# chemprop/chemprop

Measured on AMD Instinct MI355X. Metric: million directed-edge-updates/sec (depth=3, hidden=300), higher is better.
Workload: dtype f32 (exact 3-term f16 split of fp32 operands, fp32 accumulate); 1 GPU; qm9-shaped synthetic molecules, 512 mols/GPU/step, BondMessagePassing depth=3 hidden=300, forward (plan K0 + K1..K5); mols_per_gpu=512, directed_edges_per_gpu=9120, parallelism=dp1 (molecule shards, no data-path collective), launch=eager

## Files before the change

### chemprop_amd/_lib.py

```python
from __future__ import annotations

import ctypes as C
import os
import shutil
import subprocess
from typing import Optional

_HERE = os.path.dirname(os.path.abspath(__file__))
_ROOT = os.path.dirname(_HERE)
CSRC = os.path.join(_HERE, "csrc")
INCLUDE = os.path.join(_ROOT, "include")
LIB_PATH = os.environ.get("DMPNN_LIB") or os.path.join(_HERE, "libdmpnn_gfx950.so")
SOURCES = ["dmpnn_abi.hip", "dmpnn_prepare.hip", "dmpnn_segment.hip", "dmpnn_gemm.hip", "dmpnn_gemm_p1.hip",
           "dmpnn_gemm_p2.hip", "dmpnn_gemm_p3.hip", "dmpnn_gemm_p4.hip", "dmpnn_gemm_s1.hip", "dmpnn_rows16_drop.hip", "dmpnn_mega.hip", "dmpnn_mega16.hip", "dmpnn_mega16_lp.hip", "dmpnn_mega16_bwd.hip", "dmpnn_rows16.hip", "dmpnn_step16.hip", "dmpnn_bstep16.hip", "dmpnn_backward.hip", "dmpnn_molagg.hip", "dmpnn_collate.hip", "dmpnn_tiles_large.hip", "dmpnn_optim.hip", "dmpnn_wgrad16.hip", "dmpnn_head.hip", "dmpnn_vd.hip", "dmpnn_attn.hip", "dmpnn_inputgrad.hip", "dmpnn_predict.hip"]
HEADERS = ["dmpnn_common.hpp", "dmpnn_spill_impl.hpp", "dmpnn_gemm_impl.hpp", "dmpnn_mega_impl.hpp", "dmpnn_mega16_impl.hpp", "dmpnn_mega16_bwd_impl.hpp", "dmpnn_rows16_impl.hpp", "dmpnn_seg16.hpp", "dmpnn_step16_impl.hpp", "dmpnn_head_kernels.hpp"]
ABI_VERSION = 15
PLAN_NOFFSETS = 15

EXPORTS = [
    "dmpnn_version", "dmpnn_debug_timestamps", "dmpnn_last_error_string", "dmpnn_last_launch_count", "dmpnn_plan_bytes",
    "dmpnn_plan_layout", "dmpnn_prepare", "dmpnn_prepare_light", "dmpnn_prepare_tiles", "dmpnn_message_fwd", "dmpnn_aggregate_fwd",
    "dmpnn_linear_fwd", "dmpnn_linear16_wsplit_bytes", "dmpnn_linear16_ok", "dmpnn_linear16_fwd", "dmpnn_update_fwd", "dmpnn_forward", "dmpnn_forward_can_fuse", "dmpnn_forward_wsplit_bytes", "dmpnn_forward_keep_bits_bytes", "dmpnn_forward_spill_bytes", "dmpnn_backward_ws_bytes", "dmpnn_backward", "dmpnn_message_bwd", "dmpnn_atom_message_bwd",
    "dmpnn_aggregate_bwd", "dmpnn_linear_wgrad_ws_bytes", "dmpnn_linear_wgrad",
    "dmpnn_molagg_ws_bytes", "dmpnn_molagg_bounds", "dmpnn_molagg_fwd", "dmpnn_molagg_bwd", "dmpnn_gather_rows", "dmpnn_collate", "dmpnn_pack_tiles", "dmpnn_pack_tiles_blocked", "dmpnn_max_tiles",
    "dmpnn_prepare_tiles_from_table", "dmpnn_prepare_with_batch", "dmpnn_tile_plan_any_size", "dmpnn_split_row_floats", "dmpnn_forward_can_fuse16", "dmpnn_adam_step",
    "dmpnn_full_plan_keeps_tiles", "dmpnn_head_ws_bytes", "dmpnn_head", "dmpnn_train_step", "dmpnn_forward_tiles", "dmpnn_forward_route", "dmpnn_dropout_keep",
    "dmpnn_clip_grad", "dmpnn_clip_grad_ws_bytes", "dmpnn_train_route", "dmpnn_forward_h0_bytes", "dmpnn_tile_waves", "dmpnn_debug_lds_poison",
    "dmpnn_vd_ws_bytes", "dmpnn_vd_forward", "dmpnn_vd_backward", "dmpnn_linear16_dropout_fwd",
    "dmpnn_molagg_attn_ws_bytes", "dmpnn_molagg_attn_fwd", "dmpnn_molagg_attn_bwd",
    "dmpnn_backward_inputs", "dmpnn_backward_inputs_ws_bytes", "dmpnn_src_sum",
    "dmpnn_predict_head_ws_bytes", "dmpnn_predict_head_wsplit_bytes", "dmpnn_predict_head",
]

ACT = {"none": 0, "relu": 1, "leakyrelu": 2, "prelu": 3, "tanh": 4, "elu": 5, "selu": 6}
F_UNDIRECTED = 1
F_FUSED = 2
F_MEGA = 4
F_KEEP = 8
F_SPLIT16 = 16
F_WSPLIT_READY = 32
F_LOADER_TILES = 64
F_STORE16 = 128
F_ATOM = 1024
F_TILE_PLAN = 2048
F_UNDIRECTED_MASK = 4096
F_H0_RESIDUAL = 256
F_ROW_FINALIZE = 512
ROUTES = ("general", "general16", "fused", "fused16", "mega", "mega16")
PLAN_NOMEGA_MASK = 15
PLAN_NOFUSE_MASK = 7


class GemmArgs(C.Structure):
    _fields_ = [
        ("M", C.c_int64), ("N", C.c_int64), ("K1", C.c_int64), ("K2", C.c_int64),
        ("A1", C.c_void_p), ("lda1", C.c_int64), ("gather1", C.c_void_p), ("gather1_rows", C.c_int64),
        ("A2", C.c_void_p), ("lda2", C.c_int64),
        ("W", C.c_void_p), ("ldw", C.c_int64),
        ("bias", C.c_void_p),
        ("Cadd", C.c_void_p), ("ldcadd", C.c_int64),
        ("C", C.c_void_p), ("ldc", C.c_int64),
        ("Zpre", C.c_void_p), ("ldz", C.c_int64),
        ("act", C.c_int), ("act_slope", C.c_float), ("act_slope_ptr", C.c_void_p),
    ]


class FwdArgs(C.Structure):
    _fields_ = [
        ("plan", C.c_void_p), ("n_atoms", C.c_int64), ("n_edges", C.c_int64),
        ("d_v", C.c_int64), ("d_e", C.c_int64), ("d_h", C.c_int64), ("d_vd", C.c_int64),
        ("depth", C.c_int32), ("flags", C.c_uint32),
        ("act", C.c_int32), ("act_slope", C.c_float), ("act_slope_ptr", C.c_void_p),
        ("V", C.c_void_p), ("ldv", C.c_int64),
        ("E", C.c_void_p), ("lde", C.c_int64),
        ("V_d", C.c_void_p), ("ldvd", C.c_int64),
        ("W_i", C.c_void_p), ("b_i", C.c_void_p),
        ("W_h", C.c_void_p), ("b_h", C.c_void_p),
        ("W_o", C.c_void_p), ("b_o", C.c_void_p),
        ("W_d", C.c_void_p), ("b_d", C.c_void_p),
        ("ldh", C.c_int64), ("H0", C.c_void_p), ("Hs", C.c_void_p), ("n_hslots", C.c_int32),
        ("Ms", C.c_void_p), ("n_mslots", C.c_int32),
        ("Mv", C.c_void_p), ("Hv", C.c_void_p),
        ("out", C.c_void_p), ("ldout", C.c_int64),
        ("wsplit", C.c_void_p), ("wsplit_bytes", C.c_size_t),
        ("edge_index", C.c_void_p), ("rev_edge_index", C.c_void_p),
        ("n_tiles_launch", C.c_int64),
        ("spill_ws", C.c_void_p), ("spill_bytes", C.c_size_t),
        ("msplit", C.c_void_p), ("msplit_bytes", C.c_size_t),
        ("dropout_p", C.c_float), ("dropout_seed", C.c_uint64),
        ("keep_bits", C.c_void_p), ("keep_bits_bytes", C.c_size_t),
        ("h0_bytes", C.c_size_t),
    ]


class BwdArgs(C.Structure):
    _fields_ = [
        ("f", FwdArgs), ("gout", C.c_void_p), ("ldgout", C.c_int64),
        ("gW_i", C.c_void_p), ("gb_i", C.c_void_p), ("gW_h", C.c_void_p), ("gb_h", C.c_void_p),
        ("gW_o", C.c_void_p), ("gb_o", C.c_void_p), ("gW_d", C.c_void_p), ("gb_d", C.c_void_p),
        ("ws", C.c_void_p), ("ws_bytes", C.c_size_t),
        ("g_edge", C.c_void_p), ("ld_gedge", C.c_int64),
    ]


class BwdInputsArgs(C.Structure):
    _fields_ = [
        ("b", BwdArgs),
        ("gV", C.c_void_p), ("ldgv", C.c_int64),
        ("gE", C.c_void_p), ("ldge", C.c_int64),
        ("gV_d", C.c_void_p), ("ldgvd", C.c_int64),
    ]


MAX_FFN_LAYERS = 8
MAX_COMPONENTS = 8
DROP_SITE_VD = 0x8000
DROP_SITE_FFN = 0x10000
LOSS = {"mse": 0, "mae": 1, "bce": 2, "ce": 3, "mve": 4, "evidential": 5, "quantile": 6, "dirichlet": 7, "sid": 8, "wasserstein": 9, "mcc": 11}
SPECTRAL_ACT = {"softplus": 0, "exp": 1}
STEP_FORWARD, STEP_BACKWARD, STEP_UPDATE = 1, 2, 4


class HeadArgs(C.Structure):
    _fields_ = [
        ("n_atoms", C.c_int64), ("n_mols", C.c_int64), ("d_h", C.c_int64),
        ("batch", C.c_void_p),
        ("agg_mode", C.c_int32), ("agg_norm", C.c_float),
# ... 28 lines not shown
        ("keep_s", C.c_void_p), ("keep_Z", C.c_void_p),
        ("gout", C.c_void_p), ("ldgo", C.c_int64),
        ("gH", C.c_void_p), ("ldgh", C.c_int64),
        ("gW", C.c_void_p), ("gb", C.c_void_p),
        ("ws", C.c_void_p), ("ws_bytes", C.c_size_t),
    ]


MOLAGG_ATTENTIVE = 3
PREDICT_TRANSFORM = {"none": 0, "unscale": 1, "sigmoid": 2, "softmax": 3, "mve": 4, "evidential": 5, "quantile": 6}
PT_SPECTRAL = 8
PT_DIRICHLET_BINARY, PT_DIRICHLET_MULTICLASS = 10, 11
PREDICT_MAX_OUT = 64


class PredictArgs(C.Structure):
    _fields_ = [
        ("head", HeadArgs),
        ("transform", C.c_int32),
        ("out_mean", C.c_void_p), ("out_scale", C.c_void_p),
        ("preds", C.c_void_p),
        ("fingerprint", C.c_void_p), ("ld_fp", C.c_int64),
        ("wsplit", C.c_void_p), ("wsplit_bytes", C.c_size_t), ("wsplit_ready", C.c_int32),
    ]


class TrainRouteInfo(C.Structure):
    _fields_ = [("plan_kind", C.c_int32), ("route", C.c_int32), ("keep_rows", C.c_int32), ("keep_bits", C.c_int32), ("lean", C.c_int32)]


class StepComponent(C.Structure):
    _fields_ = [
        ("edge_index", C.c_void_p), ("rev_edge_index", C.c_void_p), ("batch", C.c_void_p), ("plan_bytes", C.c_size_t), ("plan_ready", C.c_int32),
        ("bwd", BwdArgs),
    ]


class VdArgs(C.Structure):
    _fields_ = [
        ("n_atoms", C.c_int64), ("d_h", C.c_int64), ("d_vd", C.c_int64),
        ("Hv", C.c_void_p), ("ldhv", C.c_int64),
        ("V_d", C.c_void_p), ("ldvd", C.c_int64),
        ("W_d", C.c_void_p), ("b_d", C.c_void_p),
        ("out", C.c_void_p), ("ldout", C.c_int64),
        ("gout", C.c_void_p), ("ldgout", C.c_int64),
        ("gHv", C.c_void_p), ("ldghv", C.c_int64),
        ("gW_d", C.c_void_p), ("gb_d", C.c_void_p),
        ("ws", C.c_void_p), ("ws_bytes", C.c_size_t),
        ("dropout_p", C.c_float), ("dropout_seed", C.c_uint64),
    ]


VD_MAX_WIDTH = 544


class StepArgs(C.Structure):
    _fields_ = [
        ("edge_index", C.c_void_p), ("rev_edge_index", C.c_void_p), ("batch", C.c_void_p), ("plan_bytes", C.c_size_t), ("plan_ready", C.c_int32),
        ("stages", C.c_int32),
        ("bwd", BwdArgs), ("head", HeadArgs),
        ("p", C.c_void_p), ("g", C.c_void_p), ("m", C.c_void_p), ("v", C.c_void_p), ("n_params", C.c_int64),
        ("lr", C.c_float), ("beta1", C.c_float), ("beta2", C.c_float), ("eps", C.c_float), ("weight_decay", C.c_float),
        ("bias_corr1", C.c_float), ("sqrt_bias_corr2", C.c_float), ("grad_scale", C.c_float), ("dev_scalars", C.c_void_p),
        ("clip_val", C.c_float), ("clip_mode", C.c_int32), ("clip_ws", C.c_void_p),
        ("n_extra", C.c_int32), ("extra", C.POINTER(StepComponent)),
        ("vd", C.POINTER(VdArgs)),
    ]


def sources() -> list[str]:
    return [os.path.join(CSRC, s) for s in SOURCES if os.path.isfile(os.path.join(CSRC, s))]


def _stale() -> bool:
    if os.environ.get("DMPNN_LIB"):
        return False
    if not os.path.isfile(LIB_PATH):
        return True
    t = os.path.getmtime(LIB_PATH)
    deps = sources() + [os.path.join(CSRC, h) for h in HEADERS] + [os.path.join(INCLUDE, "dmpnn.h")]
    return any(os.path.getmtime(d) > t for d in deps if os.path.isfile(d))


NO_SCRATCH = ("dmpnn_predict.hip",)


def _check_no_scratch(src: str, remarks: str, verbose: bool) -> None:
    import re

    fields = ("Function Name", "VGPRs", "LDS Size [bytes/block]", "ScratchSize [bytes/lane]")
    found = [dict()]
    for key, val in re.findall(r"remark:\s+(%s): (\S+)" % "|".join(re.escape(f) for f in fields), remarks):
        if key == "Function Name":
            found.append({})
        found[-1][key] = val
    kernels = [k for k in found if "Function Name" in k]
    if not kernels:
        raise RuntimeError(f"{src}: the compiler reported no kernel resource usage")
    for k in kernels:
        if verbose:
            print(f"{os.path.basename(src)}: {k['Function Name']} VGPRs {k.get('VGPRs')} LDS {k.get(fields[2])} B scratch {k.get(fields[3])} B/lane")
        if int(k.get(fields[3], "0")) != 0:
            raise RuntimeError(f"{src}: kernel {k['Function Name']} spills ({k[fields[3]]} bytes of scratch per lane)")


def build(force: bool = False, verbose: bool = False, defines=(), out: Optional[str] = None) -> str:
    lib_path = out or LIB_PATH
    if not force and not _stale() and out is None:
        return LIB_PATH
    hipcc = shutil.which("hipcc") or "/opt/rocm/bin/hipcc"
    if not os.path.isfile(hipcc):
        raise RuntimeError("hipcc not found: cannot build libdmpnn_gfx950.so")
    import concurrent.futures as cf
    import tempfile

    flags = ["--offload-arch=gfx950", "-O3", "-std=c++17", "-fPIC", f"-I{INCLUDE}", f"-I{CSRC}", *[f"-D{d}" for d in defines]]
    with tempfile.TemporaryDirectory(prefix="dmpnn_build_") as tmp:
        def cc(src):
            obj = os.path.join(tmp, os.path.basename(src) + ".o")
            no_scratch = os.path.basename(src) in NO_SCRATCH
            cmd = [hipcc, *flags, *(["-Rpass-analysis=kernel-resource-usage"] if no_scratch else []), "-c", src, "-o", obj]
            if verbose:
                print(" ".join(cmd))
            r = subprocess.run(cmd, capture_output=True, text=True)
            if r.returncode != 0:
                raise RuntimeError(f"hipcc failed on {src} ({r.returncode}):\n{r.stdout}\n{r.stderr}")
            if no_scratch:
                _check_no_scratch(src, r.stderr, verbose)
            return obj

        with cf.ThreadPoolExecutor(max_workers=8) as ex:
            objs = list(ex.map(cc, sources()))
        linked = os.path.join(os.path.dirname(objs[0]), "libdmpnn.so")
        cmd = [hipcc, "--offload-arch=gfx950", "-shared", "-fPIC", *objs, "-o", linked]
        if verbose:
            print(" ".join(cmd))
        r = subprocess.run(cmd, capture_output=True, text=True)
        if r.returncode != 0:
            raise RuntimeError(f"hipcc link failed ({r.returncode}):\n{r.stdout}\n{r.stderr}")
        shutil.copyfile(linked, lib_path + ".tmp")
        os.chmod(lib_path + ".tmp", 0o755)
    os.replace(lib_path + ".tmp", lib_path)
    _clean_unbundle_temporaries(lib_path)
    return lib_path


def _clean_unbundle_temporaries(lib_path: str) -> int:
    import glob

    n = 0
    for f in glob.glob(glob.escape(lib_path) + ".*"):
        tail = f[len(lib_path) + 1:]
        if tail.split(".", 1)[0].isdigit() and ("hipv4-" in tail or "host-" in tail):
            try:
                os.remove(f)
                n += 1
            except OSError:
                pass
    return n


_lib: Optional[C.CDLL] = None


def load() -> C.CDLL:
    global _lib
    if _lib is not None:
        return _lib
    import torch

    if _stale() and (shutil.which("hipcc") or os.path.isfile("/opt/rocm/bin/hipcc")):
        build()
    if not os.path.isfile(LIB_PATH):
        raise RuntimeError(
            f"{LIB_PATH} is missing: run `python -c 'import __graft_entry__ as g; g.build()'` "
            "(the MI355X engine has no CPU / eager fallback)")
    lib = C.CDLL(LIB_PATH)
    lib.dmpnn_version.restype = C.c_int
    lib.dmpnn_last_error_string.restype = C.c_char_p
    lib.dmpnn_last_launch_count.restype = C.c_int
    lib.dmpnn_plan_bytes.restype = C.c_size_t
    lib.dmpnn_plan_bytes.argtypes = [C.c_int64, C.c_int64]
    lib.dmpnn_plan_layout.argtypes = [C.c_int64, C.c_int64, C.POINTER(C.c_int64)]
    lib.dmpnn_forward_can_fuse.argtypes = [C.POINTER(FwdArgs)]
    lib.dmpnn_prepare.argtypes = [C.c_void_p, C.c_void_p, C.c_int64, C.c_int64, C.c_void_p, C.c_size_t, C.c_void_p]
    lib.dmpnn_prepare_light.argtypes = lib.dmpnn_prepare.argtypes
    lib.dmpnn_prepare_tiles.argtypes = [C.c_void_p, C.c_void_p, C.c_void_p, C.c_int64, C.c_int64, C.c_void_p, C.c_size_t, C.c_void_p]
    lib.dmpnn_message_fwd.argtypes = [C.c_void_p, C.c_int64, C.c_int64, C.c_int64, C.c_void_p, C.c_int64,
                                      C.c_void_p, C.c_int64, C.c_int, C.c_float, C.c_void_p, C.c_uint, C.c_void_p]
    lib.dmpnn_aggregate_fwd.argtypes = [C.c_void_p, C.c_int64, C.c_int64, C.c_int64, C.c_void_p, C.c_int64,
                                        C.c_void_p, C.c_int64, C.c_int, C.c_float, C.c_void_p, C.c_void_p]
    lib.dmpnn_linear_fwd.argtypes = [C.POINTER(GemmArgs), C.c_void_p]
    lib.dmpnn_update_fwd.argtypes = [C.c_void_p, C.c_int64, C.c_int64, C.c_int64, C.c_void_p, C.c_int64, C.c_void_p, C.c_int64,
                                     C.c_void_p, C.c_void_p, C.c_void_p, C.c_int64, C.c_void_p, C.c_int64, C.c_void_p,
                                     C.c_int64, C.c_int, C.c_float, C.c_void_p, C.c_void_p]
    lib.dmpnn_forward.argtypes = [C.POINTER(FwdArgs), C.c_void_p]
    lib.dmpnn_backward_ws_bytes.argtypes = [C.POINTER(FwdArgs)]
    lib.dmpnn_backward.argtypes = [C.POINTER(BwdArgs), C.c_void_p]
    lib.dmpnn_backward_inputs_ws_bytes.argtypes = [C.POINTER(FwdArgs)]
    lib.dmpnn_backward_inputs.argtypes = [C.POINTER(BwdInputsArgs), C.c_void_p]
    lib.dmpnn_src_sum.argtypes = [C.c_void_p, C.c_int64, C.c_int64, C.c_int64, C.c_void_p, C.c_int64, C.c_void_p, C.c_int64, C.c_void_p]
    lib.dmpnn_message_bwd.argtypes = [C.c_void_p, C.c_int64, C.c_int64, C.c_int64, C.c_void_p, C.c_int64,
                                      C.c_void_p, C.c_int64, C.c_void_p]
    lib.dmpnn_aggregate_bwd.argtypes = lib.dmpnn_message_bwd.argtypes
    lib.dmpnn_atom_message_bwd.argtypes = lib.dmpnn_message_bwd.argtypes
    lib.dmpnn_linear_wgrad_ws_bytes.argtypes = [C.c_int64, C.c_int64, C.c_int64, C.c_int]
    lib.dmpnn_linear_wgrad.argtypes = [C.POINTER(GemmArgs), C.c_void_p, C.c_int64, C.c_void_p, C.c_int64,
                                       C.c_void_p, C.c_void_p, C.c_size_t, C.c_void_p]
    size_t_fns = ("dmpnn_plan_bytes", "dmpnn_backward_ws_bytes", "dmpnn_linear_wgrad_ws_bytes", "dmpnn_forward_wsplit_bytes", "dmpnn_forward_spill_bytes",
                  "dmpnn_forward_keep_bits_bytes",
                  "dmpnn_molagg_ws_bytes", "dmpnn_linear16_wsplit_bytes", "dmpnn_head_ws_bytes", "dmpnn_clip_grad_ws_bytes", "dmpnn_forward_h0_bytes", "dmpnn_vd_ws_bytes",
                  "dmpnn_molagg_attn_ws_bytes", "dmpnn_backward_inputs_ws_bytes", "dmpnn_predict_head_ws_bytes", "dmpnn_predict_head_wsplit_bytes")
    lib.dmpnn_linear16_wsplit_bytes.argtypes = [C.c_int64, C.c_int64]
    lib.dmpnn_linear16_ok.argtypes = [C.POINTER(GemmArgs)]
    lib.dmpnn_linear16_fwd.argtypes = [C.POINTER(GemmArgs), C.c_void_p, C.c_size_t, C.c_int, C.c_void_p]
    lib.dmpnn_linear16_dropout_fwd.argtypes = [C.POINTER(GemmArgs), C.c_void_p, C.c_size_t, C.c_int, C.c_float, C.c_uint64, C.c_int32, C.c_void_p]
    lib.dmpnn_gather_rows.argtypes = [C.c_void_p, C.c_int64, C.c_int64, C.c_void_p, C.c_int64, C.c_int64, C.c_void_p, C.c_int64,
                                      C.c_void_p]
    lib.dmpnn_pack_tiles.argtypes = [C.c_void_p, C.c_void_p, C.c_int64, C.c_void_p, C.c_void_p, C.c_int64]
    lib.dmpnn_pack_tiles.restype = C.c_int64
    lib.dmpnn_pack_tiles_blocked.argtypes = [C.c_void_p, C.c_void_p, C.c_int64, C.c_void_p, C.c_void_p, C.c_int64]
    lib.dmpnn_pack_tiles_blocked.restype = C.c_int64
    lib.dmpnn_max_tiles.argtypes = [C.c_int64, C.c_int64]
    lib.dmpnn_prepare_with_batch.argtypes = [C.c_void_p, C.c_void_p, C.c_void_p, C.c_int64, C.c_int64, C.c_void_p, C.c_size_t, C.c_void_p]
    lib.dmpnn_prepare_with_batch.restype = C.c_int
    lib.dmpnn_tile_plan_any_size.argtypes = [C.c_int64, C.c_int64]
    lib.dmpnn_max_tiles.restype = C.c_int64
    lib.dmpnn_prepare_tiles_from_table.argtypes = [C.c_void_p, C.c_void_p, C.c_int64, C.c_int64, C.c_int64, C.c_void_p, C.c_size_t,
                                                   C.c_void_p]
    lib.dmpnn_collate.argtypes = [C.c_void_p, C.c_void_p, C.c_int64, C.c_void_p, C.c_void_p, C.c_void_p, C.c_int64, C.c_int64,
                                  C.c_void_p, C.c_void_p, C.c_void_p, C.c_void_p]
    lib.dmpnn_molagg_ws_bytes.argtypes = [C.c_int64]
    lib.dmpnn_molagg_bounds.argtypes = [C.c_void_p, C.c_int64, C.c_int64, C.c_void_p, C.c_size_t, C.c_void_p]
    lib.dmpnn_molagg_fwd.argtypes = [C.c_void_p, C.c_int64, C.c_int64, C.c_int64, C.c_int64, C.c_void_p, C.c_int, C.c_float,
                                     C.c_void_p, C.c_int64, C.c_void_p]
    lib.dmpnn_molagg_bwd.argtypes = [C.c_void_p, C.c_int64, C.c_void_p, C.c_int64, C.c_int64, C.c_int64, C.c_void_p, C.c_int,
                                     C.c_float, C.c_void_p, C.c_int64, C.c_void_p]
    lib.dmpnn_forward_wsplit_bytes.argtypes = [C.POINTER(FwdArgs)]
    lib.dmpnn_forward_keep_bits_bytes.argtypes = [C.POINTER(FwdArgs)]
    lib.dmpnn_forward_spill_bytes.argtypes = [C.POINTER(FwdArgs)]
    lib.dmpnn_forward_h0_bytes.argtypes = [C.POINTER(FwdArgs)]
    lib.dmpnn_forward_can_fuse16.argtypes = [C.POINTER(FwdArgs)]
    lib.dmpnn_adam_step.argtypes = [C.c_void_p, C.c_void_p, C.c_void_p, C.c_void_p, C.c_int64, C.c_float, C.c_float, C.c_float, C.c_float,
                                    C.c_float, C.c_float, C.c_float, C.c_float, C.c_void_p, C.c_void_p]
    lib.dmpnn_train_route.argtypes = [C.POINTER(FwdArgs), C.c_int64, C.c_int32, C.c_int32, C.c_int32, C.c_int32, C.c_int32, C.POINTER(TrainRouteInfo)]
    lib.dmpnn_clip_grad.argtypes = [C.c_void_p, C.c_int64, C.c_float, C.c_int32, C.c_float, C.c_void_p, C.c_void_p]
    lib.dmpnn_dropout_keep.argtypes = [C.c_uint64, C.c_int32, C.c_int64, C.c_int64, C.c_float]
    lib.dmpnn_forward_route.argtypes = [C.POINTER(FwdArgs), C.c_int, C.c_int, C.c_int, C.c_int]
    lib.dmpnn_tile_waves.restype = C.c_int
    lib.dmpnn_tile_waves.argtypes = [C.c_int64, C.c_int64, C.c_int64, C.c_int64]
    lib.dmpnn_forward_tiles.argtypes = [C.POINTER(FwdArgs), C.c_void_p, C.c_void_p, C.c_void_p, C.c_int64, C.c_size_t, C.c_void_p]
    lib.dmpnn_full_plan_keeps_tiles.argtypes = [C.c_int64, C.c_int64]
    lib.dmpnn_head_ws_bytes.argtypes = [C.POINTER(HeadArgs)]
    lib.dmpnn_head.argtypes = [C.POINTER(HeadArgs), C.c_void_p, C.c_int64, C.c_void_p]
    lib.dmpnn_train_step.argtypes = [C.POINTER(StepArgs), C.c_void_p]
    lib.dmpnn_vd_ws_bytes.argtypes = [C.POINTER(VdArgs)]
    lib.dmpnn_vd_forward.argtypes = [C.POINTER(VdArgs), C.c_void_p]
    lib.dmpnn_vd_backward.argtypes = [C.POINTER(VdArgs), C.c_void_p]
    lib.dmpnn_molagg_attn_ws_bytes.argtypes = [C.POINTER(MolAggAttnArgs)]
    lib.dmpnn_molagg_attn_fwd.argtypes = [C.POINTER(MolAggAttnArgs), C.c_void_p]
    lib.dmpnn_molagg_attn_bwd.argtypes = [C.POINTER(MolAggAttnArgs), C.c_void_p]
    lib.dmpnn_predict_head_ws_bytes.argtypes = [C.POINTER(PredictArgs)]
    lib.dmpnn_predict_head_wsplit_bytes.argtypes = [C.POINTER(PredictArgs)]
    lib.dmpnn_predict_head.argtypes = [C.POINTER(PredictArgs), C.c_void_p, C.c_int64, C.c_void_p]
    lib.dmpnn_split_row_floats.argtypes = [C.c_int64]
    lib.dmpnn_split_row_floats.restype = C.c_int64
    lib.dmpnn_debug_timestamps.argtypes = [C.c_void_p]
    for name in size_t_fns:
        getattr(lib, name).restype = C.c_size_t
    for name in EXPORTS:
        if name != "dmpnn_last_error_string" and name not in size_t_fns and name not in ("dmpnn_pack_tiles", "dmpnn_pack_tiles_blocked", "dmpnn_max_tiles", "dmpnn_split_row_floats"):
            getattr(lib, name).restype = C.c_int
    if lib.dmpnn_version() != ABI_VERSION:
        raise RuntimeError(f"libdmpnn ABI version {lib.dmpnn_version()} != {ABI_VERSION} (stale build?)")
    _lib = lib
    return lib


_ENV_DATA = getattr(os.environ, "_data", None)
_ENV_KEYS: dict = {}


def opt(name: str, default: str) -> str:
    if _ENV_DATA is None or os.name != "posix":
        return os.environ.get(name, default)
    k = _ENV_KEYS.get(name)
    if k is None:
        k = _ENV_KEYS[name] = name.encode()
    v = _ENV_DATA.get(k)
    return default if v is None else v.decode()


class DmpnnError(RuntimeError):
    pass


def check(rc: int, what: str) -> None:
    if rc != 0:
        msg = load().dmpnn_last_error_string().decode(errors="replace")
        raise DmpnnError(f"{what} failed (code {rc}): {msg}")
```

### chemprop_amd/csrc/dmpnn_abi.hip

```cpp
#include <stdarg.h>
#include <stdlib.h>
#include <string.h>

#include "dmpnn_common.hpp"
#include "dmpnn_mega16_impl.hpp"

namespace dmpnn {

static thread_local char g_err[512] = "";
static thread_local int g_launches = 0;

void set_error(const char* fmt, ...) {
    va_list ap;
    va_start(ap, fmt);
    vsnprintf(g_err, sizeof(g_err), fmt, ap);
    va_end(ap);
}
void reset_launch_count() { g_launches = 0; }
static __global__ __launch_bounds__(1024) void k_debug_lds_poison(unsigned pat, unsigned* sink) {
    extern __shared__ unsigned lds_words[];
    constexpr int n = (160 * 1024 - 64) / 4;
    for (int i = threadIdx.x; i < n; i += 1024) lds_words[i] = pat;
    __syncthreads();
    if (sink && lds_words[(threadIdx.x * 7) % n] == 0x12345u) sink[0] = 1;
// ... 211 lines not shown
        if (Mv && n_atoms > 0) {
            for (int64_t v = 0; v < n_atoms; ++v)
                if (hipMemsetAsync(Mv + v * ld_mv, 0, (size_t)d_h * sizeof(float), static_cast<hipStream_t>(stream)) != hipSuccess) {
                    set_error("update_fwd: memset failed");
                    return DMPNN_EHIP;
                }
        }
        return DMPNN_OK;
    }
    const int* plan_i = static_cast<const int*>(plan);
    const PlanLayout L = plan_layout(n_atoms, n_edges);
    dmpnn_gemm_args g;
    memset(&g, 0, sizeof(g));
    g.M = n_edges; g.N = d_h; g.K1 = d_h;
    g.A1 = M; g.lda1 = ld_m;
    g.W = W_h; g.ldw = d_h; g.bias = b_h;
    g.Cadd = H0; g.ldcadd = ld_h0;
    g.C = H_out; g.ldc = ld_hout;
    g.act = act; g.act_slope = act_slope; g.act_slope_ptr = act_slope_ptr;
    GemmExtra x;
    memset(&x, 0, sizeof(x));
    x.seg = true;
    x.tile_row = plan_i + L.tile_row; x.tile_atom = plan_i + L.tile_atom; x.n_tiles = (int)L.max_tiles;
    x.row_ptr = plan_i + L.row_ptr; x.revp = plan_i + L.revp;
    x.Mout = M_next; x.ldm = ld_mnext; x.Sout = Mv; x.lds = ld_mv;
    return launch_linear_ex(g, x, static_cast<hipStream_t>(stream));
}

static size_t steps16_wsplit_bytes(const dmpnn_fwd_args& a) {
    const int64_t h = a.d_h;
    const int64_t de_i = (a.flags & DMPNN_F_ATOM) ? 0 : a.d_e, de_h = (a.flags & DMPNN_F_ATOM) ? a.d_e : 0;
    size_t n = linear16_wsplit_bytes(h, a.d_v + de_i) + linear16_wsplit_bytes(h, h + de_h) + linear16_wsplit_bytes(h, a.d_v + h);
    n += linear16_wsplit_bytes(h + a.d_vd, h + a.d_vd) * ((a.W_d && a.d_vd > 0) ? 1 : 0);
    n += linear16_wsplit_bytes(h, h) + linear16_wsplit_bytes(h, a.d_v);
    return n;
}

size_t dmpnn_forward_wsplit_bytes(const dmpnn_fwd_args* a) {
    if (!a || a->d_h <= 0 || a->d_v <= 0 || a->d_e < 0) return 0;
    return (a->flags & DMPNN_F_MEGA) ? mega16_wsplit_bytes(*a) : steps16_wsplit_bytes(*a);
}

static bool keep_bits_apply(const dmpnn_fwd_args& a) {
    const unsigned need = DMPNN_F_TILE_PLAN | DMPNN_F_KEEP | DMPNN_F_MEGA | DMPNN_F_SPLIT16 | DMPNN_F_FUSED;
    return (a.flags & need) == need && (a.act == DMPNN_ACT_NONE || act_is_relu_class(a.act)) &&
           !(a.dropout_p > 0.f) && !a.W_d && a.n_atoms > 0 && a.n_edges > 0;
}
size_t dmpnn_forward_keep_bits_bytes(const dmpnn_fwd_args* a) {
    if (!a) return 0;
    if ((a->flags & (DMPNN_F_FUSED | DMPNN_F_SPLIT16)) == (DMPNN_F_FUSED | DMPNN_F_SPLIT16) && !(a->flags & DMPNN_F_MEGA)) return fused16_lean_bits_bytes(*a);
    if (!keep_bits_apply(*a)) return 0;
    return (size_t)a->depth * (size_t)plan_layout(a->n_atoms, a->n_edges).max_mtiles * 256u * 8u;
}

size_t dmpnn_forward_h0_bytes(const dmpnn_fwd_args* a) { return a ? fused16_h0q_bytes(*a) : 0; }

size_t dmpnn_forward_spill_bytes(const dmpnn_fwd_args* a) {
    if (!a || a->n_atoms < 0 || a->n_edges < 0 || a->ldh <= 0) return 0;
    return (size_t)(3 * a->n_edges + a->n_atoms) * (size_t)a->ldh * sizeof(float);
}

static bool al_ptr(const void* p, int bytes) { return (reinterpret_cast<uintptr_t>(p) & (uintptr_t)(bytes - 1)) == 0; }

int dmpnn_forward_can_fuse(const dmpnn_fwd_args* a) {
    if (!a) return 0;
    const int64_t h = a->d_h, dv = a->d_v, de = a->d_e;
    if (a->flags & DMPNN_F_UNDIRECTED) return 0;
    if (h <= 0 || h % 4 != 0 || h > 320 || a->ldh % 4 != 0) return 0;
    if (dv % 2 != 0 || de % 2 != 0 || a->ldv % 2 != 0 || a->lde % 2 != 0) return 0;
    if (!al_ptr(a->V, 8) || !al_ptr(a->E, 8) || !al_ptr(a->W_i, 8) || !al_ptr(a->W_h, 16)) return 0;
    if (!al_ptr(a->H0, 16) || !al_ptr(a->Ms, 16) || !al_ptr(a->Mv, 16) || (a->Hs && !al_ptr(a->Hs, 16))) return 0;
    if (a->n_atoms * a->ldv * 4 > 0x7FFFFFFF || a->n_edges * a->lde * 4 > 0x7FFFFFFF) return 0;
    return mega_shapes_ok(*a) ? 2 : 1;
}

static const int64_t kSteps16MinEdges = 20000, kFused16MinEdges = 2048;

int dmpnn_tile_waves(int64_t n_atoms, int64_t n_edges, int64_t d_h, int64_t n_tiles) {
    dmpnn_fwd_args t;
    memset(&t, 0, sizeof(t));
    t.n_atoms = n_atoms; t.n_edges = n_edges; t.d_h = d_h;
    return tile_waves(t, n_tiles > 0 ? (int)n_tiles : (int)plan_layout(n_atoms, n_edges).max_mtiles);
}

int dmpnn_forward_route(const dmpnn_fwd_args* a, int keep, int max_level, int plan_kind, int arith) {
    if (!a || max_level < 0 || plan_kind < 0 || plan_kind > 2 || arith < 0 || arith > 1) return -1;
    const bool undirected = (a->flags & DMPNN_F_UNDIRECTED) != 0;
    int level = undirected ? 0 : dmpnn_forward_can_fuse(a);
    if (level > max_level) level = max_level;
    if (plan_kind == 2) return (level == 2 && arith == 0 && !(keep && a->W_d)) ? DMPNN_ROUTE_MEGA16 : -1;
    if (plan_kind == 1 && keep) return -1;
    const int64_t nE = a->n_edges, h = a->d_h;
    if (!keep && !undirected && arith == 0 && nE >= kFused16MinEdges && (level == 1 || (level == 0 && h > 320 && max_level >= 1))) {
        dmpnn_fwd_args t = *a;
        t.flags &= ~(unsigned)(DMPNN_F_KEEP | DMPNN_F_STORE16);
        if (fused16_shapes_ok(t)) return DMPNN_ROUTE_FUSED16;
    }
    if (keep && level == 1 && arith == 0 && nE >= kSteps16MinEdges && plan_kind == 0) {
        dmpnn_fwd_args t = *a;
        t.flags = (t.flags | DMPNN_F_FUSED | DMPNN_F_SPLIT16) & ~(unsigned)(DMPNN_F_MEGA | DMPNN_F_STORE16);
        if (fused16_lean_shapes(t)) return DMPNN_ROUTE_FUSED16;
    }
    if (level == 1 && arith == 0 && nE >= kSteps16MinEdges && plan_kind != 1) level = 0;
    if (level == 2) return arith == 0 ? DMPNN_ROUTE_MEGA16 : DMPNN_ROUTE_MEGA;
    if (level == 1) return DMPNN_ROUTE_FUSED;
    if (plan_kind == 1) return -1;
    return (arith == 0 && (h > 320 || nE >= kSteps16MinEdges)) ? DMPNN_ROUTE_GENERAL16 : DMPNN_ROUTE_GENERAL;
}

int dmpnn_train_route(const dmpnn_fwd_args* a, int64_t n_mols, int32_t have, int32_t oversize, int32_t max_level, int32_t arith,
                      int32_t keep_rows, dmpnn_train_route_info* out) {
    DMPNN_CHECK_ARG(a && out && max_level >= 0 && (arith == 0 || arith == 1) && keep_rows >= -1 && keep_rows <= 1, "train_route: bad arguments");
    memset(out, 0, sizeof(*out));
    const int64_t nV = a->n_atoms, nE = a->n_edges, h = a->d_h;
    const bool undirected = (a->flags & DMPNN_F_UNDIRECTED) != 0, atom = (a->flags & DMPNN_F_ATOM) != 0;
    const bool relu_class = act_is_relu_class(a->act);
    const bool builtin = a->act == DMPNN_ACT_NONE || relu_class || act_is_smooth(a->act);
    bool tiles = !undirected && !a->W_d && builtin && max_level >= 2 && arith == 0 && nE > 0 && nV > 0 && oversize != 1;
    if (a->dropout_p > 0.f && !relu_class) tiles = false;
    if (!(h > 0 && h % 4 == 0 && h <= 320 && a->d_v % 2 == 0 && a->d_e % 2 == 0)) tiles = false;
    if (atom && !(a->d_e >= 2 && a->d_e <= 16) ) tiles = false;
    const bool small = small_plan_fits(nV, nE), table = (have & 2) != 0, large = (have & 1) != 0 && tiles_large_fits(nV, nE);
    if (!(small || table || large)) tiles = false;
    if (!(n_mols > 0 && nE <= 30 * n_mols && (table || large || small))) tiles = false;
    out->plan_kind = tiles ? 2 : 0;
    int cap = max_level;
    if (oversize == 1 && cap > 1) cap = 1;
    dmpnn_fwd_args t = *a;
    if (table || large) t.flags |= DMPNN_F_LOADER_TILES;
    out->route = dmpnn_forward_route(&t, 1, cap, out->plan_kind, arith);
    if (out->route < 0 && out->plan_kind == 2) {
        out->plan_kind = 0;
        out->route = dmpnn_forward_route(&t, 1, cap, 0, arith);
    }
    const int64_t n_steps = a->depth > 1 ? a->depth - 1 : 0;
    const bool rows = keep_rows == 1 || (keep_rows < 0 && nE * n_steps >= DMPNN_KEEP_ROWS_MIN);
    out->keep_rows = (!atom && n_steps > 0 && mega16_rows_width_ok(h) && rows) ? 1 : 0;
    if (out->route == DMPNN_ROUTE_MEGA16) {
        out->keep_bits = (out->plan_kind == 2 && (relu_class || a->act == DMPNN_ACT_NONE) && !(a->dropout_p > 0.f)) ? 1 : 0;
    } else if (out->route == DMPNN_ROUTE_FUSED16) {
        dmpnn_fwd_args l = *a;
        l.flags = (l.flags | DMPNN_F_FUSED | DMPNN_F_SPLIT16) & ~(unsigned)(DMPNN_F_MEGA | DMPNN_F_STORE16);
        out->lean = fused16_lean_shapes(l) ? 1 : 0;
        out->keep_bits = out->lean;
    }
    return DMPNN_OK;
}

int dmpnn_forward_tiles(const dmpnn_fwd_args* a, const int64_t* batch, const int* tile_row, const int* tile_atom, int64_t n_tiles,
                        size_t plan_bytes, void* stream) {
    DMPNN_CHECK_ARG(a != nullptr && a->plan != nullptr, "forward_tiles: null args / plan");
    void* plan = const_cast<void*>(a->plan);
    bool did_split = false;
    if (batch && tile_row && tile_atom && n_tiles > 0) {
        const dmpnn::PlanLayout L = dmpnn::plan_layout(a->n_atoms, a->n_edges);
        const bool ok = a->n_atoms > 0 && a->n_edges > 0 && a->n_atoms < (1ll << 31) && a->n_edges < (1ll << 31) &&
                        plan_bytes >= (size_t)L.words * sizeof(int) && n_tiles <= L.max_mtiles;
        if (ok) DMPNN_TRY(launch_tiles_checked_split(a->edge_index, batch, tile_row, tile_atom, n_tiles, a->n_atoms, a->n_edges, static_cast<int*>(plan),
                                                     static_cast<hipStream_t>(stream), a, &did_split));
        if (!did_split)
            DMPNN_TRY(prepare_tiles_and_bounds(a->edge_index, a->rev_edge_index, batch, a->n_atoms, a->n_edges, plan, plan_bytes, nullptr, 0, stream, nullptr, a, &did_split));
    } else if (tile_row && tile_atom && n_tiles > 0) {
        const dmpnn::PlanLayout L = dmpnn::plan_layout(a->n_atoms, a->n_edges);
        const bool ok = a->n_atoms >= 0 && a->n_edges >= 0 && a->n_atoms < (1ll << 31) && a->n_edges < (1ll << 31) &&
                        plan_bytes >= (size_t)L.words * sizeof(int) && n_tiles <= L.max_mtiles;
        if (ok) DMPNN_TRY(launch_tiles_from_table_split(tile_row, tile_atom, n_tiles, a->n_atoms, a->n_edges, static_cast<int*>(plan),
// ... 338 lines not shown
```

### chemprop_amd/csrc/dmpnn_common.hpp

```cpp
#pragma once

#include <hip/hip_runtime.h>
#include <stdint.h>
#include <stdio.h>
#include <string.h>

#include "dmpnn.h"

namespace dmpnn {

namespace mega16 { struct SplitArgs; }

void set_error(const char* fmt, ...);
void count_launch(const char* name);
void reset_launch_count();

#define DMPNN_CHECK_ARG(cond, ...)                 \
    do {                                           \
        if (!(cond)) {                             \
            ::dmpnn::set_error(__VA_ARGS__);       \
            return DMPNN_EINVAL;                   \
        }                                          \
    } while (0)

// ... 171 lines not shown
        matom[t] = a;
    }
    if (n_tiles == 0 && (nE > 0 || nV > 0)) bad = 1;
    if (bad) atomicOr(&bad_s, 1);
    __syncthreads();
    if (threadIdx.x < DMPNN_HDR_WORDS) {
        int v = 0;
        const int h = threadIdx.x;
        if (h == DMPNN_HDR_FLAGS) v = (bad_s ? PLAN_NO_PIECE_TILES : 0) | PLAN_TILES_ONLY | extra_flags;
        if (h == DMPNN_HDR_NMTILES) v = bad_s ? 0 : n_tiles;
        if (h == DMPNN_HDR_NSPILL) v = bad_s ? 0 : spill_s;
        if (h == DMPNN_HDR_LIGHT) v = 2;
        if (h == DMPNN_HDR_NATOMS) v = nV;
        if (h == DMPNN_HDR_NEDGES) v = nE;
        if (h == DMPNN_HDR_TILE_STRIDE) v = kFusedBM;
        plan[h] = v;
    }
}

int launch_tiles_from_table_split(const int* tile_row, const int* tile_atom, int64_t n_tiles, int64_t nV, int64_t nE, int* plan, hipStream_t s,
                                  const dmpnn_fwd_args* split_for, bool* did_split);
int launch_tiles_checked_split(const int64_t* edge_index, const int64_t* batch, const int* tile_row, const int* tile_atom, int64_t n_tiles,
                               int64_t nV, int64_t nE, int* plan, hipStream_t s, const dmpnn_fwd_args* split_for, bool* did_split);
int launch_prepare_tiles_batch(const int64_t* edge_index, const int64_t* batch, int64_t nV, int64_t nE, int* plan, hipStream_t s,
                               int* mol_bounds = nullptr, int64_t n_mols = 0, const dmpnn_fwd_args* split_for = nullptr, bool* did_split = nullptr);
bool mega16_split_args(const dmpnn_fwd_args& a, mega16::SplitArgs* sp);
size_t fused16_h0q_bytes(const dmpnn_fwd_args& a);
bool mega16_keeps_rows(const dmpnn_fwd_args& a);
bool mega16_rows_width_ok(int64_t d_h);
int prepare_tiles_and_bounds(const int64_t* edge_index, const int64_t* rev, const int64_t* batch, int64_t nV, int64_t nE, void* plan,
                             size_t plan_bytes, int* mol_bounds, int64_t n_mols, void* stream, bool* wrote_bounds,
                             const dmpnn_fwd_args* split_for = nullptr, bool* did_split = nullptr);
int molagg_fwd_rows(const float* H, int64_t ldh, int64_t n_atoms, int64_t d_h, int64_t n_mols, const void* ws, int mode,
                    float norm, float* out, int64_t ldo, int64_t rows, void* stream);
int molagg_bwd_rows(const float* gout, int64_t ldg, const int64_t* batch, int64_t n_atoms, int64_t d_h, int64_t n_mols,
                    const void* ws, int mode, float norm, float* gH, int64_t ldgh, int64_t rows, void* stream);
int attn_fwd_impl(const dmpnn_molagg_attn_args* a, int* id_bounds, int64_t* id_batch, void* stream);
int attn_bwd_impl(const dmpnn_molagg_attn_args* a, void* stream);
bool tiles_large_fits(int64_t nV, int64_t nE);
int launch_prepare_tiles_large(const int64_t* edge_index, const int64_t* batch, int64_t nV, int64_t nE, int* plan, hipStream_t s);
constexpr int kSmallPlanMaxAtoms = 6144, kSmallPlanMaxEdges = 10240;
inline size_t small_plan_lds_bytes(int64_t nV, int64_t nE) {
    return ((size_t)(3 * (nV + 2)) * 4 + (size_t)(5 * nE + 2) * 2 + 31) & ~size_t(15);
}
inline bool small_plan_fits(int64_t nV, int64_t nE) {
    return nV <= kSmallPlanMaxAtoms && nE <= kSmallPlanMaxEdges && small_plan_lds_bytes(nV, nE) <= 160 * 1024 - 2048;
}
int launch_message(const PlanView& pv, int64_t nV, int64_t nE, int64_t h, const float* Hin,
                   int64_t ld_in, float* M, int64_t ld_m, int act, float slope,
                   const float* slope_ptr, unsigned flags, hipStream_t s);
int launch_aggregate(const PlanView& pv, int64_t nV, int64_t nE, int64_t h, const float* Hin,
                     int64_t ld_in, float* Mv, int64_t ld_mv, int act, float slope,
                     const float* slope_ptr, hipStream_t s);
int launch_linear(const dmpnn_gemm_args& a, hipStream_t s);

struct GemmExtra {
    const int* gather2; int64_t gather2_rows;
    const int* tile_row; int n_tiles;
    bool seg;
    const int* tile_atom; const int* row_ptr; const int* revp;
    float* Mout; int64_t ldm;
    float* Sout; int64_t lds;
    const int* poison_flags; int poison_mask;
};
int launch_linear_ex(const dmpnn_gemm_args& a, const GemmExtra& x, hipStream_t s);
bool mega_shapes_ok(const dmpnn_fwd_args& a);
int launch_mega_forward(const dmpnn_fwd_args& a, float* out, int64_t ldout, hipStream_t s);
size_t mega16_wsplit_bytes(const dmpnn_fwd_args& a);
size_t mega16_fwd_wsplit_bytes(const dmpnn_fwd_args& a);
struct SplitWView { const unsigned char* p; const float* inv_scale; int nc; };
size_t linear16_wsplit_bytes(int64_t N, int64_t K);
int split_weights_view(const float* W, int64_t ldw, int64_t N, int64_t K, int tr, void* ws, SplitWView* out, hipStream_t s);
SplitWView split_weights_view_of(void* ws, int64_t N, int64_t K);
struct SplitWJob { const float* W; int64_t ldw, N, K; int tr; void* ws; };
int split_weights_views(const SplitWJob* jobs, int n, SplitWView* out, hipStream_t s);
bool split_weights_args(const SplitWJob* jobs, int n, SplitWView* out, mega16::SplitArgs* sp);
int launch_split_args(const mega16::SplitArgs& sp, hipStream_t s);
bool linear16_ok(const dmpnn_gemm_args& a);
struct RowsDrop { float p; uint64_t seed; int site; };
int launch_linear16_view(const dmpnn_gemm_args& a, const SplitWView& W, const int* poison_flags, int poison_mask, hipStream_t s,
                         const RowsDrop* drop = nullptr);
int launch_mega16_forward(const dmpnn_fwd_args& a, float* out, int64_t ldout, hipStream_t s);
int tile_waves(const dmpnn_fwd_args& a, int n_tiles);
bool fused16_shapes_ok(const dmpnn_fwd_args& a);
bool fused16_lean_shapes(const dmpnn_fwd_args& a, bool on_demand = false);
size_t fused16_lean_bits_bytes(const dmpnn_fwd_args& a);
bool fused16_lean(const dmpnn_fwd_args& a);
int64_t split_row_floats(int64_t d_h);

struct WSplitJob {
    int64_t M; int C;
    const float* A1; int64_t lda1; const int* g1; int K1;
    const float* A2; int64_t lda2; const int* g2; int K2;
    int ones;
    unsigned char* out; float* scales;
    int n_ct, n_chunks, wg0;
    const long long* g1_64; int64_t g1_rows;
};
struct WSplitArgs { WSplitJob job[8]; int n_jobs; };
struct WProdArgs {
    const unsigned char* Z; const float* sZ; const unsigned char* A; const float* sA;
    int n_nt, n_kt, n_chunks, chunks_per_split, splits;
    int N, Kt; float* slab; int ldk; int64_t slab_stride;
};
struct WProdPlan { int n_nt, n_kt, n_chunks, chunks_per_split, splits, ldk; int64_t slab_stride; };
constexpr int kWProdMaxJobs = 8;
struct WProdJobs { WProdArgs job[4]; int wg0[5]; int n_jobs; };
struct WProdRPlan { int n_kg, splits, rows_per_split, ldk; int64_t slab_stride; };
WProdRPlan plan_wgrad16r(int64_t M, int N, int K, int rows_per_split = 0);
void wgrad16r_plan_launch(const int64_t* M, const int* K, int n, int reserve, int* rows_out);
constexpr int kWProdRMaxJobs = 16;
struct WProdRJob { const unsigned char* Z; int tsz; const unsigned char* A; int tsa; int64_t M; int N, K; float* slab; WProdRPlan plan; float* slab_b; };
int launch_wgrad16r(const WProdRJob* jobs, int n, hipStream_t s);
struct SRJob { const float* A1; int64_t lda1; int K1; const int* g1; const long long* g1_64; int64_t g1_rows;
               const float* A2; int64_t lda2; int K2; const int* g2; int64_t M; unsigned char* out; int ts; };
int launch_rows2sr(const SRJob* jobs, int n, hipStream_t s);
size_t wsplit16_bytes(int64_t M, int64_t C);
struct AggRide {
    float* Hm; int ld; const int64_t* batch; int* table; int n_mols; int mode; float norm;
    bool taken;
};
extern thread_local AggRide g_agg_ride;
struct ExtraWgrad {
    const float* Z; int64_t ldz; const float* A; int64_t lda; int64_t M; int N, K, ones;
    float* gW; int64_t ldgw; float* gb; float* ws;
};
size_t extra_wgrad_ws_floats(int64_t M, int N, int Kt);
struct InputGrads { float* gV; int64_t ldgv; float* gE; int64_t ldge; float* gV_d; int64_t ldgvd; float* ws; };
size_t input_grads_ws_floats(const dmpnn_fwd_args& f);
int launch_src_sum(const PlanView& pv, int64_t nV, int64_t nE, int64_t h, const float* G, int64_t ldg, float* S, int64_t lds, hipStream_t s);
int input_grads(const dmpnn_fwd_args& f, const InputGrads& ig, const float* gout, int64_t ldgout, const float* GO, const float* G0, float* S,
                bool use16, hipStream_t s);
int backward_impl(const dmpnn_bwd_args* b, void* stream, const ExtraWgrad* extra, bool* extra_done, const InputGrads* ig = nullptr);
void wsplit16_job(WSplitJob* j, int64_t M, int C, const float* A1, int64_t lda1, const int* g1, int K1, const float* A2, int64_t lda2,
                  const int* g2, int K2, int ones, void* ws);
int launch_wsplit16(WSplitArgs& a, hipStream_t s);
bool wgrad16_operand_ok(const float* A1, int64_t lda1, int K1, const float* A2, int64_t lda2, int K2);
WProdPlan plan_wgrad16(int64_t M, int N, int Kt);
void wgrad16_add(WProdJobs* jobs, const WSplitJob& Z, const WSplitJob& A, const WProdPlan& p, int N, int Kt, float* slab);
int launch_wgrad16(const WProdJobs& jobs, hipStream_t s);
int launch_fused16_forward(const dmpnn_fwd_args& a, const SplitWView* w16, float* out, int64_t ldout, hipStream_t s,
                           const mega16::SplitArgs* pending = nullptr);
int launch_bstep16(const dmpnn_fwd_args& f, int site, const float* Tin, const float* gMv, const SplitWView* W, float* Tout,
                   unsigned char* Zrows, hipStream_t s);
size_t mega16_bwd_wsplit_bytes(int64_t h);
struct Mega16BwdRows { unsigned char* gZ; unsigned char* gH0; unsigned char* gZO; int tsr; };
int launch_mega16_backward(const dmpnn_fwd_args& f, const float* gHO, int64_t ldg, const float* HO, int64_t ldho, float* gZO,
                           float* gZs, float* gH0, void* wsplit, float* sp_gM, float* sp_Ta, hipStream_t s, const float* g_edge = nullptr, int64_t ld_gedge = 0,
                           const Mega16BwdRows* rows = nullptr);

int vd_check_args(const dmpnn_vd_args* a, bool bwd);
int vd_forward_impl(const dmpnn_vd_args* a, void* stream);
int vd_backward_impl(const dmpnn_vd_args* a, void* stream, bool split_ready);

struct PredictTail {
    const float* A; int64_t lda; int K;
    const float* W; const float* b; int n_out;
    int64_t B;
    float* raw;
    float* preds; int transform, t, nc; const float* mean; const float* scale;
    float* fp; int64_t ld_fp; const float* Z; int64_t ldz; int fp_w;
    int spectral_act;
};
int launch_predict_tail(const PredictTail& q, hipStream_t s);

inline bool aligned16(const void* p) { return (reinterpret_cast<uintptr_t>(p) & 15u) == 0; }
// ... 13 lines not shown
```

### chemprop_amd/csrc/dmpnn_mega16.hip

```cpp
#include <algorithm>
#include <cstdlib>

#include "dmpnn_mega16_impl.hpp"

namespace dmpnn {
namespace mega16 {
DMPNN_DEFINE_MEGA16(1, true, true)
DMPNN_DEFINE_MEGA16(1, true, false)
DMPNN_DEFINE_MEGA16(1, false, true)
DMPNN_DEFINE_MEGA16(1, false, false)
DMPNN_DEFINE_MEGA16(2, true, true)
DMPNN_DEFINE_MEGA16(2, true, false)
DMPNN_DEFINE_MEGA16(2, false, true)
DMPNN_DEFINE_MEGA16(2, false, false)
DMPNN_DEFINE_MEGA16(5, true, true)
DMPNN_DEFINE_MEGA16(5, true, false)
DMPNN_DEFINE_MEGA16(5, false, true)
DMPNN_DEFINE_MEGA16(5, false, false)
DMPNN_DEFINE_MEGA16_NW(5, true, true, 8)
DMPNN_DEFINE_MEGA16_NW(5, true, false, 8)
DMPNN_DEFINE_MEGA16_NW(5, false, true, 8)
DMPNN_DEFINE_MEGA16_NW(5, false, false, 8)
#define DMPNN_DECLARE_MEGA16_LP(WN, SA, NW) template <> int launch_mega16<WN, SA, false, NW, true>(const Mega16K& g, int n_tiles, hipStream_t s);
DMPNN_DECLARE_MEGA16_LP(1, true, 4) DMPNN_DECLARE_MEGA16_LP(1, false, 4) DMPNN_DECLARE_MEGA16_LP(2, true, 4) DMPNN_DECLARE_MEGA16_LP(2, false, 4)
DMPNN_DECLARE_MEGA16_LP(5, true, 4) DMPNN_DECLARE_MEGA16_LP(5, false, 4) DMPNN_DECLARE_MEGA16_LP(5, true, 8) DMPNN_DECLARE_MEGA16_LP(5, false, 8)
#undef DMPNN_DECLARE_MEGA16_LP
}

thread_local long long* g_debug_stamps = nullptr;
thread_local AggRide g_agg_ride = {nullptr, 0, nullptr, nullptr, 0, 0, 0.f, false};

namespace {
inline size_t al256(size_t x) { return (x + 255) & ~size_t(255); }
struct WsLayout {
    size_t wi, wh, wom, wov, sc_i, sc_h, sc_o, whe, sc_e, total;
    int nc_i, nc_h, nc_v;
};
WsLayout ws_layout(const dmpnn_fwd_args& a) {
    WsLayout L;
    const size_t N = (size_t)a.d_h;
    const bool atom = (a.flags & DMPNN_F_ATOM) != 0;
    L.nc_i = (int)((a.d_v + (atom ? 0 : a.d_e) + 31) / 32); L.nc_h = (int)((a.d_h + 31) / 32); L.nc_v = (int)((a.d_v + 31) / 32);
    size_t o = 0;
    const size_t NT = (N + 15) / 16;
    L.wi = o; o += al256(NT * L.nc_i * 2048);
    L.wh = o; o += al256(NT * L.nc_h * 2048);
    L.wom = o; o += al256(NT * L.nc_h * 2048);
    L.wov = o; o += al256(NT * L.nc_v * 2048);
    L.sc_i = o; o += al256(N * 4);
    L.sc_h = o; o += al256(N * 4);
    L.sc_o = o; o += al256(N * 4);
    L.whe = o; o += atom ? al256(NT * 1 * 2048) : 0;
    L.sc_e = o; o += atom ? al256(N * 4) : 0;
    L.total = o;
    return L;
}
}

size_t mega16_wsplit_bytes(const dmpnn_fwd_args& a) {
    return ws_layout(a).total + ((a.flags & DMPNN_F_KEEP) ? mega16_bwd_wsplit_bytes(a.d_h) : 0);
}
size_t mega16_fwd_wsplit_bytes(const dmpnn_fwd_args& a) { return ws_layout(a).total; }

bool mega16_split_args(const dmpnn_fwd_args& a, mega16::SplitArgs* spp) {
    const WsLayout W = ws_layout(a);
    if (!a.wsplit || a.wsplit_bytes < W.total) return false;
    unsigned char* ws = static_cast<unsigned char*>(a.wsplit);
    const int N = (int)a.d_h, dv = (int)a.d_v, de = (int)a.d_e;
    mega16::SplitArgs& sp = *spp;
    memset(&sp, 0, sizeof(sp));
    sp.N = N; sp.n_jobs = 4;
    const bool atom = (a.flags & DMPNN_F_ATOM) != 0;
    const int ki = atom ? dv : dv + de, ldwh = atom ? N + de : N;
    sp.job[0] = mega16::SplitJob{a.W_i, ki, 0, ki, 0, ki, ws + W.wi, W.nc_i, reinterpret_cast<float*>(ws + W.sc_i)};
    sp.job[1] = mega16::SplitJob{a.W_h, ldwh, 0, N, 0, N, ws + W.wh, W.nc_h, reinterpret_cast<float*>(ws + W.sc_h)};
    sp.job[2] = mega16::SplitJob{a.W_o, dv + N, dv, N, 0, dv + N, ws + W.wom, W.nc_h, reinterpret_cast<float*>(ws + W.sc_o)};
    sp.job[3] = mega16::SplitJob{a.W_o, dv + N, 0, dv, 0, dv + N, ws + W.wov, W.nc_v, nullptr};
    if ((a.flags & DMPNN_F_KEEP) && a.wsplit_bytes >= W.total + mega16_bwd_wsplit_bytes(N)) {
        const size_t NT = (size_t)(N + 15) / 16, nch = (size_t)(N + 31) / 32;
        const size_t one = al256(NT * nch * 2048) + al256((size_t)N * 4);
        unsigned char* wb = ws + W.total;
        sp.job[4] = mega16::SplitJob{a.W_o + dv, dv + N, 0, N, 0, N, wb, (int)nch, reinterpret_cast<float*>(wb + al256(NT * nch * 2048)), 1};
        sp.job[5] = mega16::SplitJob{a.W_h, ldwh, 0, N, 0, N, wb + one, (int)nch, reinterpret_cast<float*>(wb + one + al256(NT * nch * 2048)), 1};
        sp.n_jobs = 6;
    }
    if (atom) {
        sp.job[sp.n_jobs] = mega16::SplitJob{a.W_h, ldwh, N, de, N, de, ws + W.whe, 1, reinterpret_cast<float*>(ws + W.sc_e)};
        ++sp.n_jobs;
    }
    return true;
}

bool mega16_rows_width_ok(int64_t d_h) {
    const int64_t bn = d_h <= 64 ? 64 : (d_h <= 128 ? 128 : 320);
    return d_h > 0 && d_h <= 320 && split_row_floats(d_h) * 4 == bn * 4 + 16;
}
bool mega16_keeps_rows(const dmpnn_fwd_args& a) {
    const unsigned need = DMPNN_F_FUSED | DMPNN_F_MEGA | DMPNN_F_SPLIT16 | DMPNN_F_KEEP;
    if ((a.flags & need) != need || (a.flags & DMPNN_F_ATOM) || a.depth < 2 || a.n_edges <= 0 || !mega16_rows_width_ok(a.d_h)) return false;
    const size_t bytes = (size_t)(a.depth - 1) * (size_t)a.n_edges * (size_t)(split_row_floats(a.d_h) * 4);
    return a.msplit && aligned16(a.msplit) && a.msplit_bytes >= bytes;
}

int tile_waves(const dmpnn_fwd_args& a, int n_tiles) {
    static const int forced = [] { const char* e = getenv("DMPNN_TILE_WAVES"); return e ? atoi(e) : 0; }();
    if (forced == 4 || forced == 8) return forced;
    if (a.d_h <= 128 || a.d_h > 320) return 4;
    static const int n_cu = [] {
        int dev = 0, n = 0;
        if (hipGetDevice(&dev) != hipSuccess || hipDeviceGetAttribute(&n, hipDeviceAttributeMultiprocessorCount, dev) != hipSuccess || n <= 0) n = 256;
        return n;
    }();
    if (n_tiles <= n_cu) return 8;
    const int64_t est = std::max<int64_t>((a.n_edges + 39) / 40, (a.n_atoms + 19) / 20);
    return est + est / 16 <= n_cu ? 8 : 4;
}

int launch_mega16_forward(const dmpnn_fwd_args& a, float* out, int64_t ldout, hipStream_t s) {
    const int64_t nV = a.n_atoms, nE = a.n_edges;
    const WsLayout W = ws_layout(a);
    if (!a.wsplit || a.wsplit_bytes < W.total) {
        set_error("forward(split16): wsplit workspace missing or too small (%zu < %zu bytes)", a.wsplit_bytes, W.total);
        return DMPNN_ENOSPC;
    }
    unsigned char* ws = static_cast<unsigned char*>(a.wsplit);
    const int N = (int)a.d_h, dv = (int)a.d_v, de = (int)a.d_e;
    if (!(a.flags & DMPNN_F_WSPLIT_READY)) {
        mega16::SplitArgs sp;
        if (!mega16_split_args(a, &sp)) { set_error("forward(split16): wsplit workspace missing or too small"); return DMPNN_ENOSPC; }
        hipLaunchKernelGGL(mega16::k_split_weights, dim3((unsigned)(((N + 15) / 16) * 4 * sp.n_jobs)), dim3(256), 0, s, sp);
        DMPNN_CHECK_LAUNCH("k_split_weights");
    }

    const PlanLayout L = plan_layout(nV, nE);
    const int* plan_i = static_cast<const int*>(a.plan);
    mega16::Mega16K G;
    memset(&G, 0, sizeof(G));
    mega::MegaK& g = G.m;
    g.mtile_row = plan_i + L.mtile_row; g.mtile_atom = plan_i + L.mtile_atom; g.row_ptr = plan_i + L.row_ptr;
    g.srcp = plan_i + L.srcp; g.perm = plan_i + L.perm; g.revp = plan_i + L.revp;
    g.flags = plan_i + DMPNN_HDR_FLAGS; g.poison_mask = kPlanNoMega;
    g.nV = (int)nV; g.nE = (int)nE; g.d_v = dv; g.d_e = (a.flags & DMPNN_F_ATOM) ? 0 : de; g.h = N; g.depth = a.depth;
    g.V = a.V; g.ldv = (int)a.ldv; g.E = a.E ? a.E : a.V; g.lde = (int)a.lde;
    g.v_bytes = (unsigned)(nV * a.ldv * 4); g.e_bytes = a.E ? (unsigned)(nE * a.lde * 4) : 0u;
    g.W_i = a.W_i; g.b_i = a.b_i; g.W_h = a.W_h; g.b_h = a.b_h; g.W_o = a.W_o; g.b_o = a.b_o;
    g.act = a.act; g.slope = a.act_slope; g.slope_ptr = a.act_slope_ptr;
    g.out = out; g.ldout = (int)ldout;
    g.ldh = (int)a.ldh; g.slot = (long long)nE * a.ldh;
    if (a.flags & DMPNN_F_KEEP) { g.H0 = a.H0; g.Hs = a.Hs; g.Ms = a.Ms; g.Mv = a.Mv; }
    if ((a.flags & DMPNN_F_KEEP) && a.keep_bits) {
        G.keep_bits = static_cast<unsigned long long*>(a.keep_bits);
        G.bits_slot = (long long)L.max_mtiles * 256;
    }
    g.spill = (a.spill_ws && a.spill_bytes >= dmpnn_forward_spill_bytes(&a) && aligned16(a.spill_ws)) ? a.spill_ws : nullptr;
    G.Wi = mega16::SplitW{ws + W.wi, reinterpret_cast<const float*>(ws + W.sc_i), W.nc_i};
    G.Wh = mega16::SplitW{ws + W.wh, reinterpret_cast<const float*>(ws + W.sc_h), W.nc_h};
    G.WoM = mega16::SplitW{ws + W.wom, reinterpret_cast<const float*>(ws + W.sc_o), W.nc_h};
    G.WoV = mega16::SplitW{ws + W.wov, reinterpret_cast<const float*>(ws + W.sc_o), W.nc_v};
    if (a.flags & DMPNN_F_ATOM) {
        G.WhE = mega16::SplitW{ws + W.whe, reinterpret_cast<const float*>(ws + W.sc_e), 1};
        G.atom_de = de;
        if ((a.flags & DMPNN_F_KEEP) && a.depth > 1 && nE > 0) {
            G.atom_me = static_cast<float*>(a.msplit);
            G.me_slot = (long long)nE * mega16::kAtomK;
        }
    }
    if (mega16_keeps_rows(a)) {
        G.Mrows = static_cast<unsigned char*>(a.msplit);
        G.tsr = (int)(split_row_floats(a.d_h) * 4);
        G.mrow_slot = (long long)nE * G.tsr;
    }
    g.dbg = g_debug_stamps;
    if ((a.flags & DMPNN_F_KEEP) && g_agg_ride.Hm && g_agg_ride.n_mols > 0 && out == a.out && N % 4 == 0) {
        G.agg_Hm = g_agg_ride.Hm; G.agg_ld = g_agg_ride.ld; G.agg_batch = reinterpret_cast<const long long*>(g_agg_ride.batch);
        G.agg_bounds = g_agg_ride.table; G.agg_done = g_agg_ride.table + 2 * g_agg_ride.n_mols + 4; G.agg_n_mols = g_agg_ride.n_mols;
        G.agg_mode = g_agg_ride.mode; G.agg_norm = g_agg_ride.norm;
        g_agg_ride.taken = true;
    }
    if (a.dropout_p > 0.f && a.dropout_p < 1.f) {
        g.drop_thr = drop_threshold(a.dropout_p); g.drop_scale = 1.f / (1.f - a.dropout_p);
        g.seed_lo = (unsigned)(a.dropout_seed & 0xFFFFFFFFull); g.seed_hi = (unsigned)(a.dropout_seed >> 32);
    }
    g.edge_index = reinterpret_cast<const long long*>(a.edge_index);
    g.rev64 = reinterpret_cast<const long long*>(a.rev_edge_index);
    const int n_tiles = (a.n_tiles_launch > 0 && a.n_tiles_launch < L.max_mtiles) ? (int)a.n_tiles_launch : (int)L.max_mtiles;
    const bool sa = !act_is_smooth(a.act), kp = (a.flags & DMPNN_F_KEEP) != 0;
    const int wn = a.d_h <= 64 ? 1 : (a.d_h <= 128 ? 2 : 5);
    if (a.flags & DMPNN_F_STORE16) {
        if (wn == 1) return sa ? mega16::launch_mega16<1, true, false, 4, true>(G, n_tiles, s) : mega16::launch_mega16<1, false, false, 4, true>(G, n_tiles, s);
        if (wn == 2) return sa ? mega16::launch_mega16<2, true, false, 4, true>(G, n_tiles, s) : mega16::launch_mega16<2, false, false, 4, true>(G, n_tiles, s);
        if (tile_waves(a, n_tiles) == 8)
            return sa ? mega16::launch_mega16<5, true, false, 8, true>(G, n_tiles, s) : mega16::launch_mega16<5, false, false, 8, true>(G, n_tiles, s);
        return sa ? mega16::launch_mega16<5, true, false, 4, true>(G, n_tiles, s) : mega16::launch_mega16<5, false, false, 4, true>(G, n_tiles, s);
    }
#define DMPNN_PICK(WN) (sa ? (kp ? mega16::launch_mega16<WN, true, true>(G, n_tiles, s) : mega16::launch_mega16<WN, true, false>(G, n_tiles, s)) \
                           : (kp ? mega16::launch_mega16<WN, false, true>(G, n_tiles, s) : mega16::launch_mega16<WN, false, false>(G, n_tiles, s)))
    if (wn == 1) return DMPNN_PICK(1);
    if (wn == 2) return DMPNN_PICK(2);
    if (tile_waves(a, n_tiles) == 8)
        return sa ? (kp ? mega16::launch_mega16<5, true, true, 8>(G, n_tiles, s) : mega16::launch_mega16<5, true, false, 8>(G, n_tiles, s))
                  : (kp ? mega16::launch_mega16<5, false, true, 8>(G, n_tiles, s) : mega16::launch_mega16<5, false, false, 8>(G, n_tiles, s));
    return DMPNN_PICK(5);
#undef DMPNN_PICK
}

}
```

### chemprop_amd/csrc/dmpnn_mega16_impl.hpp

```cpp
#pragma once

#include <type_traits>

#include "dmpnn_mega_impl.hpp"

namespace dmpnn {
namespace mega16 {

using gemm::BK;
using gemm::f32x4;
using gemm::kOOB;
using gemm::kThreads;
using gemm::rsrc_t;
using gemm::u32x4;
using gemm::u32x2;
using mega::RT_A;
using mega::RT_E;

typedef _Float16 h8 __attribute__((ext_vector_type(8)));
typedef _Float16 h4 __attribute__((ext_vector_type(4)));
typedef _Float16 h2 __attribute__((ext_vector_type(2)));


struct SplitW {
// ... 87 lines not shown
        const float s = live ? scale_for(mx) : 0.f;
        if (lane == 0 && J.inv_scale && live) J.inv_scale[n] = 1.f / s;
        if (k0 < J.nc * 32) {
            h8 hv, lv;
#pragma unroll
            for (int q = 0; q < 8; ++q) {
                const float x = (k0 + q < J.K && live) ? v[q] * s : 0.f;
                const _Float16 hi = (_Float16)x;
                const _Float16 lo = (_Float16)(x - (float)hi);
                hv[q] = hi; lv[q] = lo;
            }
            const int c = k0 >> 5, lg = (k0 & 31) >> 3;
            const long long base = (((long long)T * J.nc + c) * 2) * 512 + (lg * 16 + li) * 8;
            *reinterpret_cast<h8*>(out + base) = hv;
            *reinterpret_cast<h8*>(out + base + 512) = lv;
        }
        return;
    }
    float mx = 0.f;
    for (int k = lane; k < J.scale_K; k += 64) mx = fmaxf(mx, fabsf(row[(J.scale_col0 + k) * ks]));
    for (int off = 32; off > 0; off >>= 1) mx = fmaxf(mx, __shfl_xor(mx, off));
    const float s = live ? scale_for(mx) : 0.f;
    if (lane == 0 && J.inv_scale && live) J.inv_scale[n] = 1.f / s;
    for (int k = lane; k < J.nc * 32; k += 64) {
        const float x = (k < J.K && live) ? row[(J.col0 + k) * ks] * s : 0.f;
        const _Float16 hi = (_Float16)x;
        const _Float16 lo = (_Float16)(x - (float)hi);
        const int c = k >> 5, kk = k & 31, lg = kk >> 3, j = kk & 7;
        const long long base = (((long long)T * J.nc + c) * 2) * 512 + (lg * 16 + li) * 8 + j;
        out[base] = hi;
        out[base + 512] = lo;
    }
}
static __global__ __launch_bounds__(256) void k_split_weights(SplitArgs a) {
    split_weights_wave(a, blockIdx.x * 4 + (threadIdx.x >> 6), threadIdx.x & 63);
}

__device__ __forceinline__ void rows_to_sr(const float* src, long long ld, long long row0, int nrows, int N, unsigned char* dst, int ts,
                                           int wave, int lane, int n_waves) {
    for (int r = wave; r < nrows; r += n_waves) {
        const float* x = src + (row0 + r) * ld;
        float v[8];
        float mx = 0.f;
#pragma unroll
        for (int j = 0; j < 8; ++j) {
            const int c = lane + 64 * j;
            v[j] = c < N ? x[c] : 0.f;
            mx = fmaxf(mx, fabsf(v[j]));
        }
        for (int off = 32; off > 0; off >>= 1) mx = fmaxf(mx, __shfl_xor(mx, off));
        const float sc = scale_for(mx);
        unsigned char* o = dst + (row0 + r) * ts;
#pragma unroll
        for (int j = 0; j < 8; ++j) {
            const int c = lane + 64 * j;
            if (c < N) {
                const float y = v[j] * sc;
                const _Float16 hi = (_Float16)y;
                *reinterpret_cast<_Float16*>(o + (c >> 5) * 128 + (c & 31) * 2) = hi;
                *reinterpret_cast<_Float16*>(o + (c >> 5) * 128 + 64 + (c & 31) * 2) = (_Float16)(y - (float)hi);
            }
        }
        if (lane == 0) *reinterpret_cast<float4*>(o + (ts - 16)) = make_float4(sc, mx > 0.f ? 0.f : 1.f, 0.f, 0.f);
    }
}

#if !defined(DMPNN_TILE8_BRING)
#define DMPNN_TILE8_BRING 1
#endif
template <int WN>
constexpr size_t tile_region_bytes() {
    constexpr size_t ts = 64 * WN * 4 + 16, tsg = 4 * 128 + 16;
    return (size_t)kMegaBM * (ts > tsg ? ts : tsg);
}
constexpr int kAtomK = 16;
constexpr size_t kAtomLds = (size_t)(kMegaBM + kMegaBA) * kAtomK * sizeof(float);
template <int WN>
constexpr size_t lds_bytes() {
    return tile_region_bytes<WN>() + (size_t)(3 * kMegaBM + kMegaBA + 24) * sizeof(int) + 10 * 64 * 16;
}
template <int WN>
constexpr size_t lds_bytes_atom() { return lds_bytes<WN>() + kAtomLds; }

template <int WN, bool SA, bool KEEP, int NW = 4, bool LP = false>
__global__ __launch_bounds__(64 * NW, 2) void k_mpnn_tile16(Mega16K G) {
    static_assert(!(LP && KEEP), "the hi-halves-alone form is inference only");
    static_assert(NW == 4 || (NW == 8 && WN == 5), "the 8-wave form splits 20 column tiles 3+3+3+3+2+2+2+2");
    const mega::MegaK& g = G.m;
    constexpr int KT = 64 * NW;
    constexpr int JR = 16 / NW;
    constexpr int BM = kMegaBM, BA = kMegaBA, BN = 64 * WN, LDC = BN + 4, QN = BN / 4;
    constexpr int TS = BN * 4 + 16;
    constexpr int ITEMS = (BM * QN + KT - 1) / KT;
    extern __shared__ __attribute__((aligned(16))) unsigned char lds[];
    unsigned char* T16 = lds;
    static_assert(LDC * 4 == TS, "the fp32 tile and the split A tile have the same footprint");
    constexpr int META_OFF = (int)tile_region_bytes<WN>();
    float* T = reinterpret_cast<float*>(lds);
    int* revl = reinterpret_cast<int*>(lds + META_OFF);
    int* aor = revl + BM;
    int* asrc = aor + BM;
    int* rp = asrc + BM;
    unsigned* maxbits = reinterpret_cast<unsigned*>(rp + BA + 1);
    h8* cfrag = reinterpret_cast<h8*>(lds + META_OFF + (((3 * BM + BA + 1 + 8) * 4 + 15) / 16) * 16);

    using T_ = std::true_type;
    using F_ = std::false_type;
    int tid = threadIdx.x, lane = tid & 63, wave = tid >> 6;
    int li = lane & 15, lg = lane >> 4;
    int kq = tid & 7;
    auto launder = [&]() {
        asm volatile("" : "+v"(tid));
        lane = tid & 63; wave = tid >> 6; li = lane & 15; lg = lane >> 4; kq = tid & 7;
    };
#if !defined(DMPNN_NO_KERNARG_WARM)
    warm_kernargs<(int)sizeof(Mega16K)>();
#endif
    int n_stamp = 0;
    auto stamp = [&]() {
        if (g.dbg && blockIdx.x == 0 && threadIdx.x == 0 && n_stamp < 32) g.dbg[n_stamp] = (long long)__builtin_readcyclecounter();
        ++n_stamp;
    };
    stamp();
    const int t = blockIdx.x;
    int rs = g.mtile_row[t], re = g.mtile_row[t + 1];
    int va = g.mtile_atom[t], vb = g.mtile_atom[t + 1];
    int hdr_light = g.flags[DMPNN_HDR_LIGHT], hdr_flags = g.flags[0], hdr_tiles = g.flags[DMPNN_HDR_NMTILES];
    int chk = g.flags[DMPNN_HDR_WORDS + (lane & (kPlanCheckWords - 1))];
    asm volatile("" : "+v"(rs), "+v"(re), "+v"(va), "+v"(vb), "+v"(hdr_light), "+v"(hdr_flags), "+v"(hdr_tiles), "+v"(chk));
    rs = __builtin_amdgcn_readfirstlane(rs); re = __builtin_amdgcn_readfirstlane(re);
    va = __builtin_amdgcn_readfirstlane(va); vb = __builtin_amdgcn_readfirstlane(vb);
    hdr_light = __builtin_amdgcn_readfirstlane(hdr_light); hdr_flags = __builtin_amdgcn_readfirstlane(hdr_flags);
    hdr_tiles = __builtin_amdgcn_readfirstlane(hdr_tiles);
    const int nrows = re - rs, na = vb - va;
    const int N = g.h, qn = N >> 2;
    const bool lean = hdr_light == 2;
    const bool poison = (hdr_flags & (lean ? kPlanNoMegaLean : g.poison_mask)) != 0 || (lean && g.nE > 0 && (!g.edge_index || !g.rev64)) ||
                        hdr_tiles > (int)gridDim.x || ((hdr_flags & PLAN_CHECK_WORDS) != 0 && __ballot(chk != 0) != 0ull);
    if (poison) {
        const float nanv = __int_as_float(0x7fc00000);
        const long long total = (long long)g.nV * N;
        for (long long i = (long long)blockIdx.x * KT + tid; i < total; i += (long long)gridDim.x * KT)
            g.out[(i / N) * g.ldout + (i % N)] = nanv;
        return;
    }
    if (na <= 0 || nrows < 0 || va < 0 || vb > g.nV || rs < 0 || re > g.nE) return;
    if (nrows > BM || na > BA) {
        if (NW > 4 && threadIdx.x >= kThreads) return;
        const mega::MegaK& gs = spill::fresh_kernargs<Mega16K>()->m;
        if ((KEEP && gs.drop_thr) || G.atom_de) {
            const float nanv = __int_as_float(0x7fc00000);
            for (int i = tid; i < na * N; i += kThreads) gs.out[(long long)(va + i / N) * gs.ldout + (i % N)] = nanv;
            if constexpr (KEEP) {
                if (gs.Hs)
                    for (int i = tid; i < nrows * N; i += kThreads)
                        for (int sl = 0; sl < gs.depth - 1; ++sl) gs.Hs[(long long)sl * gs.slot + (long long)(rs + i / N) * gs.ldh + (i % N)] = nanv;
            }
            return;
        }
        spill::forward(mega::spill_view(gs, gs.flags[DMPNN_HDR_LIGHT] == 2, rs, nrows, va, na, gs.slope_ptr ? *gs.slope_ptr : gs.slope),
                       reinterpret_cast<float*>(lds));
        if constexpr (KEEP) {
            const Mega16K& Gs = *spill::fresh_kernargs<Mega16K>();
            if (Gs.Mrows && gs.Ms) {
                __threadfence_block();
                __syncthreads();
                for (int sl = 0; sl < gs.depth - 1; ++sl)
                    rows_to_sr(gs.Ms + (long long)sl * gs.slot, gs.ldh, rs, nrows, gs.h, Gs.Mrows + (long long)sl * Gs.mrow_slot, Gs.tsr,
                               (int)(threadIdx.x >> 6), (int)(threadIdx.x & 63), kThreads / 64);
            }
        }
        return;
    }
    const float slope = g.slope_ptr ? *g.slope_ptr : g.slope;
    const float neg_slope = g.act == DMPNN_ACT_NONE ? 1.f : (g.act == DMPNN_ACT_RELU ? 0.f : slope);
    constexpr bool simple_act = SA;

    int revl_v = 0, rp_v = 0, aor_v = 0, asrc_v = 0;
    bool row_bad = false;
    unsigned ro1[JR * RT_E], ro2[JR * RT_E];
    {
        int i1[JR * RT_E], i2[JR * RT_E];
        if (lean && nrows > 0) {
            const int e = rs + (tid < nrows ? tid : 0);
            const long long es = g.edge_index[e], ed = g.edge_index[(long long)g.nE + e], er = g.rev64[e];
            const long long r_l = er - rs, d_l = ed - va, s_l = es - va;
            row_bad = tid < nrows && (r_l < 0 || r_l >= nrows || d_l < 0 || d_l >= na || s_l < 0 || s_l >= na);
            revl_v = (tid < nrows && !row_bad) ? (int)r_l : 0;
            aor_v = (tid < nrows && !row_bad) ? (int)d_l : 0;
            asrc_v = (tid < nrows && !row_bad) ? (int)s_l : 0;
#pragma unroll
            for (int j = 0; j < JR * RT_E; ++j) {
                const int r = wave + NW * j;
                const long long sj = g.edge_index[r < nrows ? rs + r : rs];
                i1[j] = (sj >= 0 && sj < g.nV) ? (int)sj : 0;
                i2[j] = rs + r;
            }
        } else if (lean) {
#pragma unroll
            for (int j = 0; j < JR * RT_E; ++j) { i1[j] = 0; i2[j] = 0; }
        } else {
            revl_v = tid < nrows ? g.revp[rs + tid] - rs : 0;
            rp_v = g.row_ptr[va + (tid <= na ? tid : na)] - rs;
#pragma unroll
            for (int j = 0; j < JR * RT_E; ++j) {
                const int r = wave + NW * j;
                i1[j] = g.srcp[r < nrows ? rs + r : 0];
                i2[j] = g.perm[r < nrows ? rs + r : 0];
            }
        }
#pragma unroll
        for (int j = 0; j < JR * RT_E; ++j) {
            const bool ok = wave + NW * j < nrows;
            ro1[j] = ok ? (unsigned)i1[j] * (unsigned)g.ldv * 4u : kOOB;
            ro2[j] = ok ? (unsigned)i2[j] * (unsigned)g.lde * 4u : kOOB;
        }
    }
    const rsrc_t rVg = gemm::make_rsrc(g.V, g.v_bytes), rEg = gemm::make_rsrc(g.E, g.e_bytes);
    u32x2 a_grp[JR * RT_E];
    {
        const int k = lane * 2;
        const unsigned k1o = k < g.d_v ? (unsigned)k * 4u : kOOB;
        const unsigned k2o = (k >= g.d_v && k < g.d_v + g.d_e) ? (unsigned)(k - g.d_v) * 4u : kOOB;
#pragma unroll
        for (int j = 0; j < JR * RT_E; ++j)
            a_grp[j] = __builtin_amdgcn_raw_buffer_load_b64(rVg, gemm::join_off(ro1[j], k1o), 0, 0) |
                       __builtin_amdgcn_raw_buffer_load_b64(rEg, gemm::join_off(ro2[j], k2o), 0, 0);
    }
    unsigned pf_word[4] = {0u, 0u, 0u, 0u};
#if defined(DMPNN_META_STAMPS)
    stamp();
#endif
    if (tid < BM) { revl[tid] = revl_v; asrc[tid] = asrc_v; if (lean) aor[tid] = aor_v; }
    if (tid <= BA) rp[tid] = rp_v;
    if (tid < 8) maxbits[tid] = 0u;
    __syncthreads();
#if defined(DMPNN_META_STAMPS)
    stamp();
#endif
    if (row_bad) atomicOr(&maxbits[5], 1u);
    if (!lean && tid < na)
        for (int r = rp[tid]; r < rp[tid + 1]; ++r) aor[r] = tid;
    __syncthreads();
#if defined(DMPNN_META_STAMPS)
    stamp();
#endif
    int ar[12];
    {
        const int4 q0 = *reinterpret_cast<const int4*>(aor + lg * 4), q1 = *reinterpret_cast<const int4*>(aor + 16 + lg * 4),
                   q2 = *reinterpret_cast<const int4*>(aor + 32 + lg * 4);
        const int qa[12] = {q0.x, q0.y, q0.z, q0.w, q1.x, q1.y, q1.z, q1.w, q2.x, q2.y, q2.z, q2.w};
#pragma unroll
        for (int i = 0; i < 12; ++i) ar[i] = ((i >> 2) * 16 + lg * 4 + (i & 3)) < nrows ? qa[i] : -2;
    }
    for (int f = wave; f < 10; f += NW) {
        const bool agg = f >= 6;
        const int ff = agg ? f - 6 : f, jt = ff >> 1, ks = ff & 1;
        const int j = jt * 16 + li;
        int a_t = -1, rv = -1;
        if (agg) {
            a_t = j < na ? j : -1;
        } else if (j < nrows) {
            rv = revl[j];
            a_t = lean ? asrc[j] : aor[rv];
        }
        if (G.atom_de) rv = -1;
        unsigned hb[8];
#pragma unroll
        for (int sl = 0; sl < 8; ++sl) {
            const int row = ks == 0 ? (sl < 4 ? lg * 4 + sl : 16 + lg * 4 + (sl - 4)) : (sl < 4 ? 32 + lg * 4 + sl : -2);
            const int av = ks == 0 ? ar[sl] : (sl < 4 ? ar[8 + sl] : -2);
            const bool in = av == a_t, isrev = row == rv;
            hb[sl] = in ? (isrev ? 0u : 0x3C00u) : (isrev ? 0xBC00u : 0u);
        }
        const u32x4 pk = {hb[0] | (hb[1] << 16), hb[2] | (hb[3] << 16), hb[4] | (hb[5] << 16), hb[6] | (hb[7] << 16)};
        cfrag[f * 64 + lane] = __builtin_bit_cast(h8, pk);
    }
    __syncthreads();

    auto wave_max = [&](float v) -> float {
        int u = (int)__float_as_uint(v);
        u = max(u, __builtin_amdgcn_update_dpp(0, u, 0xB1, 0xf, 0xf, true));
        u = max(u, __builtin_amdgcn_update_dpp(0, u, 0x4E, 0xf, 0xf, true));
        u = max(u, __builtin_amdgcn_update_dpp(0, u, 0x141, 0xf, 0xf, true));
        u = max(u, __builtin_amdgcn_update_dpp(0, u, 0x140, 0xf, 0xf, true));
        const int m = max(max(__builtin_amdgcn_readlane(u, 0), __builtin_amdgcn_readlane(u, 16)),
                          max(__builtin_amdgcn_readlane(u, 32), __builtin_amdgcn_readlane(u, 48)));
        return __uint_as_float((unsigned)m);
    };
    int scale_phase = 0;
    float tile_mx = 0.f;
    auto tile_scale = [&](float local_max) -> float {
        const int slot = scale_phase & 3;
        local_max = wave_max(local_max);
        if (lane == 0) atomicMax(&maxbits[slot], __float_as_uint(local_max));
        __syncthreads();
        const float mx = __uint_as_float(maxbits[slot]);
        tile_mx = mx;
        if (tid == 0) maxbits[(slot + 2) & 3] = 0u;
        ++scale_phase;
        return scale_for(mx);
    };

    auto body = [&](auto wl_c) __attribute__((always_inline)) {
    constexpr int WL = decltype(wl_c)::value;
    auto ct0 = [&]() -> int { return (NW == 8 && WL == 2) ? 2 * wave + 4 : WL * wave; };
    auto load_bfrags = [&](rsrc_t rW, const unsigned (&offB)[WL], int c, h8 (&bh)[WL], h8 (&bl)[WL]) {
#pragma unroll
        for (int ct = 0; ct < WL; ++ct) {
            const u32x4 vh = __builtin_amdgcn_raw_buffer_load_b128(rW, offB[ct] + (unsigned)c * 2048u, 0, 0);
            bh[ct] = __builtin_bit_cast(h8, vh);
            if constexpr (!LP) {
                const u32x4 vl = __builtin_amdgcn_raw_buffer_load_b128(rW, offB[ct] + (unsigned)c * 2048u + 1024u, 0, 0);
                bl[ct] = __builtin_bit_cast(h8, vl);
            }
        }
    };
    auto bfrag_offsets = [&](const SplitW& W, unsigned (&offB)[WL]) {
        launder();
#pragma unroll
        for (int ct = 0; ct < WL; ++ct)
            offB[ct] = (unsigned)(ct0() + ct) * (unsigned)(W.nc * 2048) + (unsigned)lane * 16u;
    };
    unsigned char* rows_pending = nullptr;
    int rows_pending_n = 0;
    auto flush_rows = [&]() {
        if constexpr (KEEP) {
            if (rows_pending) {
                constexpr int PPR = TS / 16;
                for (int it = tid; it < rows_pending_n * PPR; it += KT) {
                    const int r = it / PPR, pc = it - r * PPR;
                    *reinterpret_cast<u32x4*>(rows_pending + (long long)r * TS + pc * 16) = *reinterpret_cast<const u32x4*>(T16 + r * TS + pc * 16);
                }
                rows_pending = nullptr;
            }
        }
    };
    auto contract = [&](auto rt_c, f32x4 (&acc)[decltype(rt_c)::value][WL], const unsigned char* Ab, int astride, int n_chunks,
                        int wc0, const SplitW& W) {
        constexpr int RT = decltype(rt_c)::value;
        const rsrc_t rW = gemm::make_rsrc(W.p, (unsigned)(((N + 15) / 16) * W.nc * 2048));
        unsigned offB[WL];
        bfrag_offsets(W, offB);
#pragma unroll
        for (int ct = 0; ct < WL; ++ct) offB[ct] += (unsigned)wc0 * 2048u;
        auto read_afrags = [&](int c, h8 (&ah)[RT], h8 (&al)[RT]) {
#pragma unroll
            for (int rt = 0; rt < RT; ++rt) {
                const unsigned char* p = Ab + (rt * 16 + li) * astride + c * 128 + lg * 16;
                ah[rt] = *reinterpret_cast<const h8*>(p);
                if constexpr (!LP) al[rt] = *reinterpret_cast<const h8*>(p + 64);
            }
        };
        h8 a0h[RT], a0l[RT], a1h[RT], a1l[RT];
        if constexpr (NW == 8 && DMPNN_TILE8_BRING == 2) {
            h8 b0h[WL], b0l[WL], b1h[WL], b1l[WL];
            load_bfrags(rW, offB, 0, b0h, b0l);
            {
                const bool two = n_chunks > 1;
#pragma unroll
                for (int ct = 0; ct < WL; ++ct) {
                    b1h[ct] = __builtin_bit_cast(h8, __builtin_amdgcn_raw_buffer_load_b128(rW, two ? offB[ct] + 2048u : kOOB, 0, 0));
                    if constexpr (!LP) b1l[ct] = __builtin_bit_cast(h8, __builtin_amdgcn_raw_buffer_load_b128(rW, two ? offB[ct] + 3072u : kOOB, 0, 0));
                }
            }
            __syncthreads();
            flush_rows();
            launder();
            read_afrags(0, a0h, a0l);
            auto chunk2 = [&](int c, h8 (&ah)[RT], h8 (&al)[RT], h8 (&nah)[RT], h8 (&nal)[RT], h8 (&bh)[WL], h8 (&bl)[WL]) {
                const bool more2 = c + 2 < n_chunks;
#pragma unroll
                for (int ct = 0; ct < WL; ++ct) {
#pragma unroll
                    for (int rt = 0; rt < RT; ++rt) acc[rt][ct] = __builtin_amdgcn_mfma_f32_16x16x32_f16(ah[rt], bh[ct], acc[rt][ct], 0, 0, 0);
                    if constexpr (!LP) {
#pragma unroll
                        for (int rt = 0; rt < RT; ++rt) acc[rt][ct] = __builtin_amdgcn_mfma_f32_16x16x32_f16(ah[rt], bl[ct], acc[rt][ct], 0, 0, 0);
#pragma unroll
                        for (int rt = 0; rt < RT; ++rt) acc[rt][ct] = __builtin_amdgcn_mfma_f32_16x16x32_f16(al[rt], bh[ct], acc[rt][ct], 0, 0, 0);
                    }
                    __builtin_amdgcn_sched_barrier(0);
                    const unsigned o = more2 ? offB[ct] + (unsigned)(c + 2) * 2048u : kOOB;
                    bh[ct] = __builtin_bit_cast(h8, __builtin_amdgcn_raw_buffer_load_b128(rW, o, 0, 0));
                    if constexpr (!LP) bl[ct] = __builtin_bit_cast(h8, __builtin_amdgcn_raw_buffer_load_b128(rW, more2 ? o + 1024u : kOOB, 0, 0));
                    if (ct == (WL > 1 ? WL - 2 : 0)) read_afrags(c + 1 < n_chunks ? c + 1 : c, nah, nal);
                    __builtin_amdgcn_sched_barrier(0);
                }
            };
            int c = 0;
#pragma nounroll
            for (; c + 1 < n_chunks; c += 2) {
                chunk2(c, a0h, a0l, a1h, a1l, b0h, b0l);
                chunk2(c + 1, a1h, a1l, a0h, a0l, b1h, b1l);
            }
            if (c < n_chunks) chunk2(c, a0h, a0l, a1h, a1l, b0h, b0l);
            return;
        }
        h8 bh[WL], bl[WL];
        load_bfrags(rW, offB, 0, bh, bl);
        __syncthreads();
        flush_rows();
        launder();
        read_afrags(0, a0h, a0l);
        auto chunk = [&](int c, h8 (&ah)[RT], h8 (&al)[RT], h8 (&nah)[RT], h8 (&nal)[RT]) {
            const bool more = c + 1 < n_chunks;
#pragma unroll
            for (int ct = 0; ct < WL; ++ct) {
#pragma unroll
                for (int rt = 0; rt < RT; ++rt) acc[rt][ct] = __builtin_amdgcn_mfma_f32_16x16x32_f16(ah[rt], bh[ct], acc[rt][ct], 0, 0, 0);
                if constexpr (!LP) {
#pragma unroll
                    for (int rt = 0; rt < RT; ++rt) acc[rt][ct] = __builtin_amdgcn_mfma_f32_16x16x32_f16(ah[rt], bl[ct], acc[rt][ct], 0, 0, 0);
#pragma unroll
                    for (int rt = 0; rt < RT; ++rt) acc[rt][ct] = __builtin_amdgcn_mfma_f32_16x16x32_f16(al[rt], bh[ct], acc[rt][ct], 0, 0, 0);
                }
                __builtin_amdgcn_sched_barrier(0);
                const unsigned o = more ? offB[ct] + (unsigned)(c + 1) * 2048u : kOOB;
                bh[ct] = __builtin_bit_cast(h8, __builtin_amdgcn_raw_buffer_load_b128(rW, o, 0, 0));
                if constexpr (!LP) bl[ct] = __builtin_bit_cast(h8, __builtin_amdgcn_raw_buffer_load_b128(rW, more ? o + 1024u : kOOB, 0, 0));
                if (ct == (WL > 1 ? WL - 2 : 0)) read_afrags(more ? c + 1 : c, nah, nal);
                __builtin_amdgcn_sched_barrier(0);
            }
        };
#pragma nounroll
        for (int c = 0; c < n_chunks; c += 2) {
            chunk(c, a0h, a0l, a1h, a1l);
            if (c + 1 < n_chunks) chunk(c + 1, a1h, a1l, a0h, a0l);
        }
    };

    constexpr int TSG = 4 * 128 + 16;
    unsigned char* Ag = lds;
    auto ga_load = [&](auto rt_c, auto has_a2_c, int grp, int K1, int K2, rsrc_t rA1, rsrc_t rA2,
                       const unsigned (&ro1)[JR * decltype(rt_c)::value], const unsigned (&ro2)[JR * decltype(rt_c)::value],
                       u32x2 (&v)[JR * decltype(rt_c)::value]) {
        constexpr int J = JR * decltype(rt_c)::value;
        constexpr bool HAS_A2 = decltype(has_a2_c)::value;
        const int k = grp * 128 + lane * 2;
        const unsigned k1o = k < K1 ? (unsigned)k * 4u : kOOB;
        const unsigned k2o = (k >= K1 && k < K1 + K2) ? (unsigned)(k - K1) * 4u : kOOB;
#pragma unroll
        for (int j = 0; j < J; ++j) {
            v[j] = __builtin_amdgcn_raw_buffer_load_b64(rA1, gemm::join_off(ro1[j], k1o), 0, 0);
            if constexpr (HAS_A2) v[j] = v[j] | __builtin_amdgcn_raw_buffer_load_b64(rA2, gemm::join_off(ro2[j], k2o), 0, 0);
        }
    };
    auto ga_stage = [&](auto rt_c, f32x4 (&acc)[decltype(rt_c)::value][WL], const u32x2 (&v)[JR * decltype(rt_c)::value], float s_prev) -> float {
        constexpr int RT = decltype(rt_c)::value, J = JR * RT;
        float mx = 0.f;
#pragma unroll
        for (int j = 0; j < J; ++j) mx = fmaxf(mx, fmaxf(fabsf(__uint_as_float(v[j].x)), fabsf(__uint_as_float(v[j].y))));
        const float s = tile_scale(mx);
        if (s_prev != 0.f && s_prev != s) {
            const float f = s / s_prev;
#pragma unroll
            for (int rt = 0; rt < RT; ++rt)
#pragma unroll
                for (int ct = 0; ct < WL; ++ct)
#pragma unroll
                    for (int r = 0; r < 4; ++r) acc[rt][ct][r] *= f;
        }
        launder();
#pragma unroll
        for (int j = 0; j < J; ++j) {
            unsigned hi, lo;
            split2(__uint_as_float(v[j].x), __uint_as_float(v[j].y), s, hi, lo);
            unsigned char* p = Ag + (wave + NW * j) * TSG + (lane >> 4) * 128 + (lane & 15) * 4;
            *reinterpret_cast<unsigned*>(p) = hi;
            if constexpr (!LP) *reinterpret_cast<unsigned*>(p + 64) = lo;
        }
        return s;
    };
    auto zero_acc = [&](auto rt_c, f32x4 (&acc)[decltype(rt_c)::value][WL]) {
        constexpr int RT = decltype(rt_c)::value;
#pragma unroll
        for (int rt = 0; rt < RT; ++rt)
#pragma unroll
            for (int ct = 0; ct < WL; ++ct) acc[rt][ct] = f32x4{0.f, 0.f, 0.f, 0.f};
    };
    struct ColConst { float isw[WL], bv[WL]; };
    auto col_consts = [&](const float* inv_sW, const float* bias) -> ColConst {
        ColConst cc;
        launder();
        const float* bp = bias ? bias : inv_sW;
#pragma unroll
        for (int ct = 0; ct < WL; ++ct) {
            const int col = (ct0() + ct) * 16 + li;
            const bool okc = col < N;
            cc.isw[ct] = inv_sW[okc ? col : 0];
            const float braw = bp[okc ? col : 0];
            cc.bv[ct] = (okc && bias) ? braw : 0.f;
        }
        return cc;
    };
    auto unscale = [&](auto rt_c, f32x4 (&acc)[decltype(rt_c)::value][WL], float inv_sA, const ColConst& cc) {
        constexpr int RT = decltype(rt_c)::value;
#pragma unroll
        for (int ct = 0; ct < WL; ++ct) {
            const float isw = cc.isw[ct] * inv_sA;
#pragma unroll
            for (int rt = 0; rt < RT; ++rt)
#pragma unroll
                for (int r = 0; r < 4; ++r) acc[rt][ct][r] = acc[rt][ct][r] * isw + cc.bv[ct];
        }
    };
    auto act_frags = [&](auto rt_c, auto use_res_c, f32x4 (&z)[decltype(rt_c)::value][WL], const f32x4 (&res)[decltype(rt_c)::value][WL]) {
        constexpr int RT = decltype(rt_c)::value;
        constexpr bool USE_RES = decltype(use_res_c)::value;
        if constexpr (simple_act) {
#if !defined(DMPNN_RELU_SELECT)
            if (neg_slope == 0.f) {
#pragma unroll
                for (int rt = 0; rt < RT; ++rt)
#pragma unroll
                    for (int ct = 0; ct < WL; ++ct)
#pragma unroll
                        for (int r = 0; r < 4; ++r) {
                            const float v = USE_RES ? res[rt][ct][r] + z[rt][ct][r] : z[rt][ct][r];
                            z[rt][ct][r] = __builtin_elementwise_maximum(v, 0.f);
                        }
                return;
            }
#endif
#pragma unroll
            for (int rt = 0; rt < RT; ++rt)
#pragma unroll
                for (int ct = 0; ct < WL; ++ct)
#pragma unroll
                    for (int r = 0; r < 4; ++r) {
                        const float v = USE_RES ? res[rt][ct][r] + z[rt][ct][r] : z[rt][ct][r];
                        z[rt][ct][r] = (v > 0.f ? v : neg_slope * v) + 0.f;
// ... 260 lines not shown
        __syncthreads();
        launder();
        if constexpr (KEEP) {
            if (G.atom_me) {
                for (int i = tid; i < nrows * kAtomK; i += KT) {
                    const int r = i / kAtomK, k = i - r * kAtomK;
                    const float v = SE[(lean ? asrc[r] : aor[revl[r]]) * kAtomK + k];
                    for (int sl = 0; sl < T_steps - 1; ++sl) G.atom_me[(long long)sl * G.me_slot + (long long)(rs + r) * kAtomK + k] = v;
                }
            }
        }
        float xv[RT_E][8];
        float mx = 0.f;
#pragma unroll
        for (int rt = 0; rt < RT_E; ++rt) {
            const int row = rt * 16 + li;
            const int a_s = row < nrows ? (lean ? asrc[row] : aor[revl[row]]) : -1;
#pragma unroll
            for (int j = 0; j < 8; ++j) {
                const int k = lg * 8 + j;
                xv[rt][j] = (a_s >= 0 && k < kAtomK) ? SE[a_s * kAtomK + (k < kAtomK ? k : 0)] : 0.f;
                mx = fmaxf(mx, fabsf(xv[rt][j]));
            }
        }
        const float sE = tile_scale(mx);
        h8 eh[RT_E], el[RT_E];
#pragma unroll
        for (int rt = 0; rt < RT_E; ++rt)
#pragma unroll
            for (int j = 0; j < 8; ++j) {
                const float x = xv[rt][j] * sE;
                const _Float16 hi = (_Float16)x;
                eh[rt][j] = hi; el[rt][j] = (_Float16)(x - (float)hi);
            }
        unsigned offE[WL];
        bfrag_offsets(G.WhE, offE);
        h8 wh[WL], wl[WL];
        load_bfrags(gemm::make_rsrc(G.WhE.p, (unsigned)(((N + 15) / 16) * G.WhE.nc * 2048)), offE, 0, wh, wl);
        const ColConst ce = col_consts(G.WhE.inv_scale, nullptr);
#pragma unroll
        for (int ct = 0; ct < WL; ++ct)
#pragma unroll
            for (int rt = 0; rt < RT_E; ++rt) {
                f32x4 z = f32x4{0.f, 0.f, 0.f, 0.f};
                z = __builtin_amdgcn_mfma_f32_16x16x32_f16(eh[rt], wh[ct], z, 0, 0, 0);
                z = __builtin_amdgcn_mfma_f32_16x16x32_f16(eh[rt], wl[ct], z, 0, 0, 0);
                z = __builtin_amdgcn_mfma_f32_16x16x32_f16(el[rt], wh[ct], z, 0, 0, 0);
                const float isw = ce.isw[ct] / sE;
#pragma unroll
                for (int r = 0; r < 4; ++r) h0[rt][ct][r] += z[r] * isw;
            }
    }

    for (int step = 1; step < T_steps; ++step) {
        f32x4 acc[RT_E][WL];
        zero_acc(RE{}, acc);
        const ColConst cc = col_consts(G.Wh.inv_scale, g.b_h);
        contract(RE{}, acc, T16, TS, (N + BK - 1) / BK, 0, G.Wh);
        stamp();
        unscale(RE{}, acc, rcp_pow2_exact(sA), cc);
        act_frags(RE{}, T_{}, acc, h0);
        dropout_frags(RE{}, acc, (unsigned)(step - 1), rs, true);
        stamp();
        if (KEEP && G.keep_bits) {
            store_bits(RE{}, acc, step);
        } else if (KEEP && g.Hs) {
            __syncthreads();
            frag_to_tile(RE{}, acc);
            __syncthreads();
            tile_to_global(g.Hs + (long long)(step - 1) * g.slot, rs, g.ldh, nrows);
        }
        const bool last = step == T_steps - 1;
        sA = segment_mfma(acc, last, last ? g.Mv : ((g.Ms && !G.Mrows) ? g.Ms + (long long)step * g.slot : nullptr), g.ldh,
                          (last || !G.Mrows) ? nullptr : G.Mrows + (long long)step * G.mrow_slot);
        stamp();
    }

    {
        f32x4 acc[RT_A][WL];
        zero_acc(RA{}, acc);
        const ColConst cc = col_consts(G.WoM.inv_scale, g.b_o);
        const rsrc_t rV = gemm::make_rsrc(g.V + (long long)va * g.ldv, (unsigned)(na * g.ldv) * 4u);
        const rsrc_t rnull = gemm::make_rsrc(g.W_o, 0);
        unsigned rov[JR * RT_A];
#pragma unroll
        for (int j = 0; j < JR * RT_A; ++j) rov[j] = wave + NW * j < na ? (unsigned)(wave + NW * j) * (unsigned)g.ldv * 4u : kOOB;
        u32x2 v_grp[JR * RT_A];
        ga_load(RA{}, F_{}, 0, g.d_v, 0, rV, rnull, rov, rov, v_grp);
        contract(RA{}, acc, T16, TS, (N + BK - 1) / BK, 0, G.WoM);
        stamp();
        float sV = sA;
        for (int grp = 0; grp * 4 < G.WoV.nc; ++grp) {
            if (grp > 0) ga_load(RA{}, F_{}, grp, g.d_v, 0, rV, rnull, rov, rov, v_grp);
            sV = ga_stage(RA{}, acc, v_grp, sV);
            if (grp == 0) stamp();
            const int ncg = G.WoV.nc - grp * 4 < 4 ? G.WoV.nc - grp * 4 : 4;
            contract(RA{}, acc, Ag, TSG, ncg, grp * 4, G.WoV);
        }
        stamp();
        unscale(RA{}, acc, rcp_pow2_exact(sV), cc);
        act_frags(RA{}, F_{}, acc, acc);
        dropout_frags(RA{}, acc, (unsigned)(T_steps - 1), va, false);
        if (maxbits[5]) {
#pragma unroll
            for (int rt = 0; rt < RT_A; ++rt)
#pragma unroll
                for (int ct = 0; ct < WL; ++ct) acc[rt][ct] = f32x4{__int_as_float(0x7fc00000), __int_as_float(0x7fc00000), __int_as_float(0x7fc00000), __int_as_float(0x7fc00000)};
        }
        if ((pf_word[0] ^ pf_word[1] ^ pf_word[2] ^ pf_word[3]) == 0x7fdead01u) maxbits[7] = 1u;
        __syncthreads();
        frag_to_tile(RA{}, acc);
        __syncthreads();
        tile_to_global(g.out, va, g.ldout, na);
        stamp();
        if constexpr (KEEP) {
            if (G.agg_Hm) {
                const long long m0 = G.agg_batch[va], m1 = G.agg_batch[vb - 1];
                if (m0 >= 0 && m1 < G.agg_n_mols && m1 - m0 < BA) {
                    const int nm = (int)(m1 - m0) + 1;
                    for (int it = tid; it < nm * QN; it += KT) {
                        const int ml = it / QN, q = it - ml * QN;
                        if (q >= qn) continue;
                        const long long m = m0 + ml;
                        const int f = G.agg_bounds[m] - va, e = G.agg_bounds[G.agg_n_mols + m] - va;
                        if (f < 0 || e > na || e <= f) continue;
                        float4 sacc = *reinterpret_cast<const float4*>(T + f * LDC + 4 * q);
                        for (int a = f + 1; a < e; ++a) {
                            const float4 x = *reinterpret_cast<const float4*>(T + a * LDC + 4 * q);
                            sacc.x += x.x; sacc.y += x.y; sacc.z += x.z; sacc.w += x.w;
                        }
                        if (G.agg_mode == DMPNN_MOLAGG_MEAN) { const float n = (float)(e - f); sacc.x /= n; sacc.y /= n; sacc.z /= n; sacc.w /= n; }
                        if (G.agg_mode == DMPNN_MOLAGG_NORM) { sacc.x /= G.agg_norm; sacc.y /= G.agg_norm; sacc.z /= G.agg_norm; sacc.w /= G.agg_norm; }
                        *reinterpret_cast<float4*>(G.agg_Hm + m * G.agg_ld + 4 * q) = sacc;
                        if (q == 0) G.agg_done[m] = 1;
                    }
                }
            }
        }
    }
    };
    if constexpr (NW == 4) {
        body(std::integral_constant<int, WN>{});
    } else {
        if (__builtin_amdgcn_readfirstlane((int)(threadIdx.x >> 6)) < 4) body(std::integral_constant<int, 3>{});
        else body(std::integral_constant<int, 2>{});
    }
}

template <int WN, bool SA, bool KEEP, int NW = 4, bool LP = false>
int launch_mega16(const Mega16K& g, int n_tiles, hipStream_t s);

#define DMPNN_DEFINE_MEGA16(WN, SA, KEEP) DMPNN_DEFINE_MEGA16_NW(WN, SA, KEEP, 4)
#define DMPNN_DEFINE_MEGA16_NW(WN, SA, KEEP, NW) DMPNN_DEFINE_MEGA16_LP(WN, SA, KEEP, NW, false)
#define DMPNN_DEFINE_MEGA16_LP(WN, SA, KEEP, NW, LP)                                                       \
    template <>                                                                                            \
    int launch_mega16<WN, SA, KEEP, NW, LP>(const Mega16K& g, int n_tiles, hipStream_t s) {                \
        const size_t lds = g.atom_de ? lds_bytes_atom<WN>() : lds_bytes<WN>();                             \
        static bool attr_set = false;                                                                      \
        if (!attr_set) {                                                                                   \
            hipError_t e = hipFuncSetAttribute(reinterpret_cast<const void*>(&k_mpnn_tile16<WN, SA, KEEP, NW, LP>),      \
                                               hipFuncAttributeMaxDynamicSharedMemorySize, (int)lds_bytes_atom<WN>()); \
            if (e != hipSuccess) {                                                                         \
                set_error("hipFuncSetAttribute(k_mpnn_tile16<%d>, %zu B LDS): %s", WN, lds, hipGetErrorString(e)); \
                return DMPNN_EHIP;                                                                         \
            }                                                                                              \
            attr_set = true;                                                                               \
        }                                                                                                  \
        hipLaunchKernelGGL((k_mpnn_tile16<WN, SA, KEEP, NW, LP>), dim3((unsigned)n_tiles), dim3(64 * NW), lds, s, g);   \
        DMPNN_CHECK_LAUNCH("k_mpnn_tile16");                                                               \
        return DMPNN_OK;                                                                                   \
    }

}
}
```

### chemprop_amd/engine.py

```python
from __future__ import annotations

import ctypes as C
import os
from typing import NamedTuple, Optional

import torch
from torch import Tensor

from . import _lib
from ._lib import (ACT, F_FUSED, F_H0_RESIDUAL, F_KEEP, F_LOADER_TILES, F_MEGA, F_ROW_FINALIZE, F_SPLIT16, F_STORE16, F_TILE_PLAN, F_UNDIRECTED, F_WSPLIT_READY,
                   PLAN_NOFUSE_MASK, PLAN_NOMEGA_MASK, FwdArgs, GemmArgs)


STEPS16_MIN_EDGES = 20000
FUSED16_MIN_EDGES = 2048


def small_plan_fits(n_atoms: int, n_edges: int) -> bool:
    lds = ((3 * (n_atoms + 2)) * 4 + (5 * n_edges + 2) * 2 + 31) & ~15
    return n_atoms <= 6144 and n_edges <= 10240 and lds <= 160 * 1024 - 2048


_raw_stream = getattr(torch._C, "_cuda_getCurrentRawStream", None)


_plan_bytes_cache: dict = {}


def plan_bytes(n_atoms: int, n_edges: int) -> int:
    k = (n_atoms, n_edges)
    v = _plan_bytes_cache.get(k)
    if v is None:
        if len(_plan_bytes_cache) > 4096:
            _plan_bytes_cache.clear()
        v = _plan_bytes_cache[k] = int(_lib.load().dmpnn_plan_bytes(n_atoms, n_edges))
    return v


def _stream_ptr(device) -> int:
    if _raw_stream is not None:
        idx = device.index
        return _raw_stream(torch.cuda.current_device() if idx is None else idx)
    return torch.cuda.current_stream(device).cuda_stream


class _OnDevice:

    __slots__ = ("ctx",)

    def __init__(self, dev):
        idx = dev.index
        self.ctx = None if (idx is None or idx == torch.cuda.current_device()) else torch.cuda.device(dev)

    def __enter__(self):
        if self.ctx is not None:
            self.ctx.__enter__()

    def __exit__(self, *a):
        if self.ctx is not None:
            self.ctx.__exit__(*a)


def _require_device(t: Tensor, name: str) -> None:
    if t.device.type != "cuda":
        raise RuntimeError(
            f"chemprop_amd: `{name}` lives on {t.device}; the MI355X engine runs HIP kernels only "
            "(no CPU fallback) — move the batch and the module to a GPU device first")


def _f32c(t: Tensor, name: str) -> Tensor:
    _require_device(t, name)
    if t.dtype != torch.float32:
        t = t.float()
    if t.dim() == 2 and t.stride(1) == 1 and t.stride(0) >= t.shape[1]:
        return t
    if t.dim() == 2 and t.shape[0] <= 1:
        return torch.empty(t.shape, dtype=t.dtype, device=t.device).copy_(t)
    return t.contiguous()


def _dense32(t: Optional[Tensor], name: str) -> Optional[Tensor]:
    if t is None:
        return None
    _require_device(t, name)
    return (t if t.dtype == torch.float32 else t.float()).contiguous()


def _ptr(t: Optional[Tensor]) -> Optional[int]:
    return None if t is None else t.data_ptr()


class GraphPlan:

    __slots__ = ("buf", "n_atoms", "n_edges", "device", "light", "tiles_only", "edge_index", "rev_edge_index", "loader_tiles",
                 "any_size", "oversize", "pending", "_job", "host_tiles")

    def __init__(self, edge_index: Tensor, rev_edge_index: Tensor, n_atoms: int, light=False, batch: Optional[Tensor] = None,
                 tiles: Optional[tuple] = None, launch: bool = True):
        _require_device(edge_index, "edge_index")
        lib = _lib.load()
        dev = edge_index.device
        n_edges = int(edge_index.shape[1])
        ei = edge_index if edge_index.dtype == torch.int64 else edge_index.long()
        ei = ei.contiguous()
        rev = rev_edge_index if rev_edge_index.dtype == torch.int64 else rev_edge_index.long()
        rev = rev.contiguous()
        nbytes = plan_bytes(n_atoms, n_edges)
        self.buf = torch.empty(nbytes // 4, dtype=torch.int32, device=dev)
        self.n_atoms, self.n_edges, self.device = int(n_atoms), n_edges, dev
        self.oversize = None
        small = small_plan_fits(n_atoms, n_edges)
        self.loader_tiles = 0
        if light == "tiles" and tiles is not None:
            tr, ta, nt = tiles
            if (tr.dtype == torch.int32 and ta.dtype == torch.int32 and tr.device == dev and ta.device == dev
                    and tr.is_contiguous() and ta.is_contiguous() and tr.numel() > nt and ta.numel() > nt and nt > 0):
                self.loader_tiles = int(nt)
        bt = batch if (batch is not None and batch.dtype == torch.int64 and batch.device == dev
                       and batch.numel() == n_atoms and batch.is_contiguous()) else None
        big = (light == "tiles" and not small and not self.loader_tiles and bt is not None and n_atoms > 0
               and bool(lib.dmpnn_tile_plan_any_size(n_atoms, n_edges)))
        self.tiles_only = light == "tiles" and (small or self.loader_tiles > 0 or big)
        self.light = bool(light) and (small or self.loader_tiles > 0 or big)
        full_tiles = (not light and not small and bt is not None and n_atoms > 0 and n_edges > 0
                      and bool(lib.dmpnn_full_plan_keeps_tiles(n_atoms, n_edges)))
        self.any_size = (self.tiles_only and not small) or full_tiles
        self.edge_index, self.rev_edge_index = ei, rev
        self.pending, self._job = None, None
        self.host_tiles = None
        if launch == "defer":
            if self.tiles_only and small and not self.loader_tiles and bt is not None:
                self.pending = bt
                self._job = (tiles, bt, full_tiles, nbytes)
                return
            launch = True
        if not launch:
            if light and not self.tiles_only:
                raise RuntimeError("GraphPlan(launch=False) is the plan of a training step: full, or the tile plan (light='tiles')")
            self.loader_tiles = 0
            return
        self._job = (tiles, bt, full_tiles, nbytes)
        self._launch()

    def ensure_launched(self) -> None:
        if self.pending is not None:
            self.pending = None
            self._launch()

    def _launch(self) -> None:
        lib = _lib.load()
        tiles, bt, full_tiles, nbytes = self._job
        self._job = None
        dev, ei, rev, n_atoms, n_edges = self.device, self.edge_index, self.rev_edge_index, self.n_atoms, self.n_edges
        with _OnDevice(dev):
            if self.loader_tiles:
                _lib.check(lib.dmpnn_prepare_tiles_from_table(tiles[0].data_ptr(), tiles[1].data_ptr(), self.loader_tiles, n_atoms,
                                                              n_edges, self.buf.data_ptr(), nbytes, _stream_ptr(dev)),
                           "dmpnn_prepare_tiles_from_table")
            elif self.tiles_only:
                _lib.check(lib.dmpnn_prepare_tiles(ei.data_ptr(), rev.data_ptr(), bt.data_ptr() if bt is not None else None,
                                                   n_atoms, n_edges, self.buf.data_ptr(), nbytes, _stream_ptr(dev)),
                           "dmpnn_prepare_tiles")
            elif full_tiles:
                _lib.check(lib.dmpnn_prepare_with_batch(ei.data_ptr(), rev.data_ptr(), bt.data_ptr(), n_atoms, n_edges,
                                                        self.buf.data_ptr(), nbytes, _stream_ptr(dev)), "dmpnn_prepare_with_batch")
            else:
                prep = lib.dmpnn_prepare_light if self.light else lib.dmpnn_prepare
                _lib.check(prep(ei.data_ptr(), rev.data_ptr(), n_atoms, n_edges,
                                self.buf.data_ptr(), nbytes, _stream_ptr(dev)), "dmpnn_prepare")

    @classmethod
    def from_bmg(cls, bmg, light=False, use_batch: bool = True, launch=True) -> "GraphPlan":
        return cls(bmg.edge_index, bmg.rev_edge_index, int(bmg.V.shape[0]), light=light,
                   batch=getattr(bmg, "batch", None) if use_batch else None,
                   tiles=getattr(bmg, "tiles", None) if light == "tiles" else None, launch=launch)

    def arrays(self) -> dict:
        self.ensure_launched()
        off = self._offsets()
        b = self.buf.cpu()
        E, V, T = self.n_edges, self.n_atoms, int(off[11])
        cut = lambda o, n: b[o:o + n]
        return dict(hdr=b[:16], src=cut(off[0], E), dst=cut(off[1], E), rev=cut(off[2], E),
                    row_ptr=cut(off[3], V + 1), perm=cut(off[4], E), inv=cut(off[5], E), srcp=cut(off[6], E),
                    dstp=cut(off[7], E), revp=cut(off[8], E), tile_row=cut(off[9], T + 2),
                    tile_atom=cut(off[10], T + 2), mtile_row=cut(off[12], int(off[14]) + 2),
                    mtile_atom=cut(off[13], int(off[14]) + 2))

    def header(self) -> list:
        self.ensure_launched()
        return self.buf[:16].tolist()

    def flags(self) -> int:
# ... 227 lines not shown
    g.act, g.act_slope, g.act_slope_ptr = act_code(act), float(slope), _ptr(slope_t)
    lib = _lib.load()
    with _OnDevice(A1.device):
        if mfma == "split16":
            if not lib.dmpnn_linear16_ok(C.byref(g)):
                raise RuntimeError("linear(split16): shapes / alignments not taken by the split kernel")
            nb = int(lib.dmpnn_linear16_wsplit_bytes(N, K1 + K2))
            ws = torch.empty(nb, dtype=torch.uint8, device=A1.device)
            _lib.check(lib.dmpnn_linear16_fwd(C.byref(g), ws.data_ptr(), nb, 0, _stream_ptr(A1.device)), "dmpnn_linear16_fwd")
        else:
            _lib.check(lib.dmpnn_linear_fwd(C.byref(g), _stream_ptr(A1.device)), "dmpnn_linear_fwd")
    return C_


def update_fused(plan: GraphPlan, M: Tensor, H0: Tensor, W_h: Tensor, b_h: Optional[Tensor] = None,
                 act: str = "relu", slope: float = 0.0, slope_t: Optional[Tensor] = None, want_H: bool = False,
                 want_M: bool = True, want_Mv: bool = False, H_out: Optional[Tensor] = None,
                 M_next: Optional[Tensor] = None, Mv: Optional[Tensor] = None):
    M, H0, W_h = _f32c(M, "M"), _f32c(H0, "H0"), _f32c(W_h, "W_h").contiguous()
    dev, (nE, h) = M.device, M.shape
    if want_H and H_out is None:
        H_out = torch.empty_like(M)
    if want_M and M_next is None:
        M_next = torch.empty_like(M)
    if want_Mv and Mv is None:
        Mv = torch.empty(plan.n_atoms, h, dtype=torch.float32, device=dev)
    ld = lambda t: t.stride(0) if t is not None else 0
    with _OnDevice(dev):
        _lib.check(_lib.load().dmpnn_update_fwd(
            plan.buf.data_ptr(), plan.n_atoms, plan.n_edges, h, M.data_ptr(), M.stride(0), H0.data_ptr(), H0.stride(0),
            W_h.data_ptr(), _ptr(b_h), _ptr(H_out), ld(H_out), _ptr(M_next), ld(M_next), _ptr(Mv), ld(Mv),
            act_code(act), float(slope), _ptr(slope_t), _stream_ptr(dev)), "dmpnn_update_fwd")
    return H_out, M_next, Mv


class ForwardState:

    __slots__ = ("plan", "H0", "Hs", "Ms", "Mv", "Hv", "ldh", "n_hslots", "n_mslots", "out", "args", "refs", "dims",
                 "fused", "route")


class _Route(NamedTuple):
    demand: Optional[str]
    use_mega: bool
    use_fused: bool
    use_fused16: bool
    want16: bool
    asked_general: bool
    mf: str


class _Workspace(NamedTuple):
    edge_ws: Optional[Tensor]
    atom_ws: Optional[Tensor]
    split_ms: Optional[Tensor] = None
    bits: Optional[Tensor] = None
    n_hslots: int = 0
    n_mslots: int = 0
    h0_bytes: int = 0
    spill: Optional[Tensor] = None


def _forward_args(plan: GraphPlan, V, E, W_i, W_h, W_o, b_o, b_i, b_h, W_d, b_d, V_d, depth: int, act: str, slope: float, slope_t,
                  undirected: bool, form: int, atom: bool, out: Optional[Tensor]) -> tuple:
    V = _f32c(V, "V")
    E = _f32c(E, "E")
    dev = V.device
    nV, nE = plan.n_atoms, plan.n_edges
    if V.shape[0] != nV or E.shape[0] != nE:
        raise RuntimeError(f"forward: plan is for V={nV}, E={nE} but got V={V.shape[0]}, E={E.shape[0]}")
    d_v, d_e, d_h = int(V.shape[1]), int(E.shape[1]), int(W_h.shape[0])
    if atom and (int(W_i.shape[1]) != d_v or int(W_h.shape[1]) != d_h + d_e):
        raise RuntimeError("forward(atom): W_i must be [d_h, d_v] and W_h [d_h, d_h + d_e] (base.py:278-289)")
    d_vd = int(V_d.shape[1]) if (W_d is not None and V_d is not None) else 0

    a = FwdArgs()
    a.plan, a.n_atoms, a.n_edges = plan.buf.data_ptr(), nV, nE
    a.edge_index, a.rev_edge_index = plan.edge_index.data_ptr(), plan.rev_edge_index.data_ptr()
    a.d_v, a.d_e, a.d_h, a.d_vd = d_v, d_e, d_h, d_vd
    a.depth, a.flags = int(depth), (F_UNDIRECTED if undirected else 0) | (int(form) & (F_H0_RESIDUAL | F_ROW_FINALIZE))
    if getattr(plan, "loader_tiles", 0) or getattr(plan, "any_size", False):
        a.flags |= F_LOADER_TILES
        a.n_tiles_launch = plan.loader_tiles
    a.act, a.act_slope, a.act_slope_ptr = act_code(act), float(slope), _ptr(slope_t)
    a.V, a.ldv = V.data_ptr(), V.stride(0)
    a.E, a.lde = E.data_ptr(), E.stride(0)
    if d_vd:
        V_d = _f32c(V_d, "V_d")
        a.V_d, a.ldvd = V_d.data_ptr(), V_d.stride(0)
    W_i, W_h, W_o, b_o = _dense32(W_i, "W_i"), _dense32(W_h, "W_h"), _dense32(W_o, "W_o"), _dense32(b_o, "b_o")
    b_i, b_h = _dense32(b_i, "b_i"), _dense32(b_h, "b_h")
    a.W_i, a.b_i, a.W_h, a.b_h, a.W_o, a.b_o = W_i.data_ptr(), _ptr(b_i), W_h.data_ptr(), _ptr(b_h), W_o.data_ptr(), b_o.data_ptr()
    if d_vd:
        W_d, b_d = _dense32(W_d, "W_d"), _dense32(b_d, "b_d")
        a.W_d, a.b_d = _ptr(W_d), _ptr(b_d)
    a.ldh = (d_h + 3) // 4 * 4
    if out is None:
        out = torch.empty(nV, d_h + d_vd, dtype=torch.float32, device=dev)
    elif (out.dtype != torch.float32 or out.device != dev or tuple(out.shape) != (nV, d_h + d_vd) or out.stride(1) != 1
          or out.stride(0) % 4 or out.data_ptr() % 16):
        raise ValueError(f"forward: out must be fp32 [{nV}, {d_h + d_vd}] on {dev}, unit column stride, 16-byte aligned rows")
    a.out, a.ldout = out.data_ptr(), out.stride(0)
    a.H0 = a.Ms = a.Mv = plan.buf.data_ptr()
    dims = dict(d_v=d_v, d_e=d_e, d_h=d_h, d_vd=d_vd, has_bi=b_i is not None, has_bh=b_h is not None, atom=bool(atom))
    return a, out, (V, E, V_d, W_i, W_h, W_o, b_o, b_i, b_h, W_d, b_d), dims


def _forward_route(lib, a, plan: GraphPlan, keep: bool, fused: Optional[bool], route: Optional[str], max_level: int, mfma: Optional[str],
                   undirected: bool) -> _Route:
    if fused is False:
        route = "general"
    asked_general = route == "general"
    if _lib.opt("DMPNN_GENERAL", "0") == "1":
        route = "general"
    mf = mfma or _lib.opt("DMPNN_MFMA", "split16")
    light, tiles_only = bool(getattr(plan, "light", False)), bool(getattr(plan, "tiles_only", False))
    if route is None and fused is None and mfma is None:
        cap = min(int(max_level), 1) if _lib.opt("DMPNN_MEGA", "1") == "0" else int(max_level)
        rc = int(lib.dmpnn_forward_route(C.byref(a), 1 if keep else 0, cap, 2 if tiles_only else (1 if light else 0), 1 if mf == "f32" else 0))
        if rc < 0:
            raise RuntimeError("forward: " + ("a tile plan (light='tiles') only serves the whole-forward tile kernel on the f16 pipe" if tiles_only else
                                              "a light GraphPlan only serves inference forwards of the fused routes (build the plan with "
                                              "light=False for the general route or for training)"))
        name = _lib.ROUTES[rc]
        use_mega, use_fused16 = name.startswith("mega"), name == "fused16"
        return _Route(route, use_mega, use_mega or use_fused16 or name == "fused", use_fused16, name.endswith("16"), asked_general, mf)
    level = 0 if (route == "general" or undirected) else int(lib.dmpnn_forward_can_fuse(C.byref(a)))
    if route == "fused" or _lib.opt("DMPNN_MEGA", "1") == "0":
        level = min(level, 1)
    if route is None:
        level = min(level, int(max_level))
    if (fused is True or route in ("fused", "mega")) and level < (2 if route == "mega" else 1):
        raise RuntimeError(f"forward: route {route or 'fused'!r} requested but the shapes do not allow it "
                           "(fused: d_h % 4 == 0, d_h <= 320, even d_v / d_e, directed; mega: additionally a batch within the "
                           "single-workgroup plan, or a plan with molecule tiles)")
    use_fused16 = (route == "fused16" and not undirected and not tiles_only and mf == "split16" and not (keep and light) and fuse16_shapes(a))
    if route == "fused16" and not use_fused16:
        raise RuntimeError("forward: route 'fused16' requested but not available (directed, d_h % 4 == 0, d_h <= 640, "
                           "even d_v / d_e, a full or light plan — training: a full plan)")
    if use_fused16:
        level = 1
    use_fused, use_mega = level >= 1, level >= 2
    if light and (not use_fused or (keep and not (tiles_only and use_mega and not a.d_vd))):
        raise RuntimeError("forward: a light GraphPlan only serves inference forwards of the fused routes "
                           "(build the plan with light=False for the general route or for training; the tile plan also "
                           "serves a training forward of the tile kernel without W_d)")
    if tiles_only and (not use_mega or mf == "f32"):
        raise RuntimeError("forward: a tile plan (light='tiles') only serves the whole-forward tile kernel on the f16 pipe")
    want16 = mf != "f32" and (use_mega or use_fused16 or (not use_fused and (mfma == "split16" or (mfma is None and mf == "split16" and (
        a.d_h > 320 or a.n_edges >= STEPS16_MIN_EDGES)))))
    return _Route(route, use_mega, use_fused, use_fused16, want16, asked_general, mf)


def _forward_homes(lib, a, r: _Route, V: Tensor, act: str, mfma: Optional[str], keep: bool, keep_bits: bool, atom: bool,
                   dropout: Optional[tuple], undirected: bool, undirected_dropout: bool) -> None:
    d_v, d_e, d_h, d_vd = a.d_v, a.d_e, a.d_h, a.d_vd
    if atom:
        tile_home = r.use_mega and r.want16 and (not keep or (d_e % 2 == 0 and d_v % 2 == 0 and d_h % 2 == 0))
        rows_home = r.asked_general and not r.use_fused and not undirected
        if not ((tile_home or rows_home) and not d_vd and 1 <= d_e <= 16):
            raise RouteUnavailable("atom messages inside the kernels: the tile kernel, 1 <= d_e <= 16, no W_d (training: even d_v / d_e / d_h) "
                                   "— or, on demand (route='general'), the per-step general route: directed, 1 <= d_e <= 16, no W_d")
        a.flags |= _lib.F_ATOM
    if dropout is None or not float(dropout[0]) > 0.0:
        return
    relu_class = act in ("relu", "leakyrelu")
# ... 331 lines not shown
```

### chemprop_amd/nn.py

```python
from __future__ import annotations

import copy
import ctypes as _ctypes
import os
from typing import Optional

import torch
from torch import Tensor, nn

from . import _lib, engine
from .autograd import input_grad_plan, input_grad_wanted, mp_forward
from .data import BatchMolGraph as _OwnBatch

DEFAULT_ATOM_FDIM, DEFAULT_BOND_FDIM = 72, 14
DEFAULT_HIDDEN_DIM = 300


class InvalidShapeError(ValueError):

    def __init__(self, var_name, received, expected):
        super().__init__(f"arg '{var_name}' has incorrect shape! got: `{tuple(received)}`. "
                         f"expected: `{tuple(expected)}`")


# ... 61 lines not shown
                 d_h: int = DEFAULT_HIDDEN_DIM, bias: bool = False, depth: int = 3, dropout: float = 0.0,
                 activation="relu", undirected: bool = False, d_vd: Optional[int] = None,
                 V_d_transform: Optional[nn.Module] = None, graph_transform: Optional[nn.Module] = None):
        super().__init__()
        self.hparams = _HParams(d_v=d_v, d_e=d_e, d_h=d_h, bias=bias, depth=depth, dropout=dropout,
                                activation=activation, undirected=undirected, d_vd=d_vd,
                                V_d_transform=V_d_transform, graph_transform=graph_transform,
                                cls=self.__class__)
        self.W_i = nn.Linear(d_v + d_e, d_h, bias)
        self.W_h = nn.Linear(d_h, d_h, bias)
        self.W_o = nn.Linear(d_v + d_h, d_h)
        self.W_d = nn.Linear(d_h + d_vd, d_h + d_vd) if d_vd else None
        self.depth = depth
        self.undirected = undirected
        self.dropout = nn.Dropout(dropout)
        self.tau = get_activation_function(activation)
        self.V_d_transform = V_d_transform if V_d_transform is not None else nn.Identity()
        self.graph_transform = graph_transform if graph_transform is not None else nn.Identity()

    @property
    def output_dim(self) -> int:
        return self.W_d.out_features if self.W_d is not None else self.W_o.out_features

    def forward(self, bmg, V_d: Optional[Tensor] = None) -> Tensor:
        return bond_message_passing_forward(self, bmg, V_d)


def _training_plan_kind(mp, bmg, atom: bool = False, vd_outside: bool = False):
    if _lib.opt("DMPNN_GENERAL", "0") == "1" or _lib.opt("DMPNN_TRAIN_PLAN", "tiles") == "full":
        return False
    act = classify_activation(mp.tau)[0]
    if act == "custom" or (mp.training and mp.dropout.p > 0 and type(mp.dropout) is not nn.Dropout):
        return False
    mode = _lib.opt("DMPNN_VALIDATE", "first")
    if mode == "always" or (mode != "never" and getattr(mp, "_dmpnn_batches_checked", 0) < _VALIDATE_FIRST_N):
        return False
    if not (mp.W_i.weight.requires_grad or mp.W_h.weight.requires_grad):
        return False
    d_h, d_in = mp.W_h.weight.shape[0], mp.W_i.weight.shape[1]
    d_v = mp.W_o.weight.shape[1] - d_h
    d_e = int(bmg.E.shape[1]) if atom else d_in - d_v
    batch = getattr(bmg, "batch", None)
    info = engine.train_route(int(bmg.V.shape[0]), int(bmg.E.shape[0]), d_v, d_e, d_h, mp.depth, act,
                              len(bmg) if hasattr(bmg, "__len__") else 0, undirected=bool(mp.undirected), has_vd=mp.W_d is not None and not vd_outside,
                              dropout_p=float(mp.dropout.p) if mp.training else 0.0, atom=atom,
                              have_batch=batch is not None and batch.dtype == torch.int64 and batch.is_contiguous(),
                              have_table=getattr(bmg, "tiles", None) is not None, oversize=getattr(bmg, "oversize", None),
                              max_level=1 if getattr(mp, "_dmpnn_no_mega", False) else 2)
    return "tiles" if info.plan_kind == 2 else False


_ENV_KEYS = ("DMPNN_GENERAL", "DMPNN_MEGA", "DMPNN_MFMA", "DMPNN_VALIDATE", "DMPNN_STORE")


class _Replay:

    __slots__ = ("args", "tensors", "ptrs", "tau", "training", "env", "dev", "d_v", "d_e", "d_h", "wsplit", "depth", "block", "flags",
                 "ldh", "spill")


def _param(mp, lin: str, name: str):
    m = mp._modules.get(lin)
    return None if m is None else m._parameters.get(name)


def _make_replay(mp, plan, st) -> None:
    mp.__dict__.pop("_dmpnn_replay", None)
    if st is None or st.route not in ("mega16", "mega16/f16-operands") or not plan.tiles_only or mp.W_d is not None:
        return
    r = _Replay()
    r.args = bytes(st.args)
    r.tensors = tuple(_param(mp, l, n) for l, n in (("W_i", "weight"), ("W_h", "weight"), ("W_o", "weight"), ("W_i", "bias"),
                                                      ("W_h", "bias"), ("W_o", "bias")))
    r.ptrs = tuple(0 if t is None else t.data_ptr() for t in r.tensors)
    r.tau, r.training, r.depth = mp._modules.get("tau"), mp.training, mp.depth
    r.env = tuple(_lib.opt(k, "") for k in _ENV_KEYS)
    r.dev = plan.device
    r.d_v, r.d_e, r.d_h = st.dims["d_v"], st.dims["d_e"], st.dims["d_h"]
    r.wsplit = st.refs[-1]
    if r.wsplit is None or any(t is not None and (t.dtype != torch.float32 or not t.is_contiguous()) for t in r.tensors):
        return
    blk = r.block = _lib.FwdArgs.from_buffer_copy(r.args)
    blk.ldv, blk.lde, blk.ldout = r.d_v, r.d_e, r.d_h
    r.flags = int(blk.flags) & ~_lib.F_WSPLIT_READY & ~_lib.F_LOADER_TILES
    r.ldh, r.spill = int(blk.ldh), None
    mp.__dict__["_dmpnn_replay"] = r


def _replay_forward(mp, r: "_Replay", bmg):
    mods = mp._modules
    if (mp.training != r.training or mods.get("tau") is not r.tau or mp.depth != r.depth or mp.undirected
            or type(mods.get("graph_transform")) is not nn.Identity or mods.get("W_d") is not None):
        return None
    ts = r.tensors
    if (_param(mp, "W_i", "weight") is not ts[0] or _param(mp, "W_h", "weight") is not ts[1] or _param(mp, "W_o", "weight") is not ts[2]
            or _param(mp, "W_i", "bias") is not ts[3] or _param(mp, "W_h", "bias") is not ts[4] or _param(mp, "W_o", "bias") is not ts[5]):
        return None
    for t, ptr in zip(ts, r.ptrs):
        if t is not None and (t.data_ptr() != ptr or t.device != r.dev):
            return None
    if tuple(_lib.opt(k, "") for k in _ENV_KEYS) != r.env:
        return None
    V, E, ei, rev, batch = bmg.V, bmg.E, bmg.edge_index, bmg.rev_edge_index, getattr(bmg, "batch", None)
    dev = r.dev
    if V.device != dev or batch is None or V.dim() != 2 or E.dim() != 2 or V.shape[1] != r.d_v or E.shape[1] != r.d_e:
        return None
    if (type(bmg) is not _OwnBatch or bmg.oversize is None) and (
            V.dtype != torch.float32 or E.dtype != torch.float32 or not V.is_contiguous() or not E.is_contiguous() or ei.dtype != torch.int64
            or rev.dtype != torch.int64 or not ei.is_contiguous() or not rev.is_contiguous() or ei.device != dev
            or batch.dtype != torch.int64 or not batch.is_contiguous() or batch.device != dev):
        return None
    nV, nE = V.shape[0], E.shape[0]
    n_mols = len(bmg) if hasattr(bmg, "__len__") else 0
    oversize = getattr(bmg, "oversize", None)
    if oversize is True:
        return None
    tiles = getattr(bmg, "tiles", None)
    if tiles is not None and (tiles[0].device != dev or tiles[2] <= 0):
        tiles = None
    own = getattr(bmg, "plan_table", None) if tiles is None else None
    if own is not None and own[0].device != dev:
        own = None
    small = engine.small_plan_fits(nV, nE)
    lib = _lib.load()
    if (n_mols <= 0 or nE > 30 * n_mols or nE == 0 or (tiles is None and not small and not lib.dmpnn_tile_plan_any_size(nV, nE))
            or batch.numel() != nV
            or ei.shape[1] != nE or rev.numel() != nE or getattr(mp, "_dmpnn_no_mega", False)):
        return None
    nbytes = engine.plan_bytes(nV, nE)
    buf = torch.empty(nbytes // 4, dtype=torch.int32, device=dev)
    out = torch.empty(nV, r.d_h, dtype=torch.float32, device=dev)
    a = r.block
    pb = buf.data_ptr()
    a.plan, a.n_atoms, a.n_edges = pb, nV, nE
    a.V, a.E = V.data_ptr(), E.data_ptr()
    a.out = out.data_ptr()
    a.Mv = a.Hv = pb
    a.edge_index, a.rev_edge_index = ei.data_ptr(), rev.data_ptr()
    if oversize is None:
        need = (3 * nE + nV) * r.ldh
        sp = r.spill
        if sp is None or sp.numel() < need:
            sp = r.spill = torch.empty(need + need // 4, dtype=torch.float32, device=dev)
        a.spill_ws, a.spill_bytes = sp.data_ptr(), need * 4
    else:
        a.spill_ws, a.spill_bytes = None, 0
    cur = torch.cuda.current_device()
    ctx = None if dev.index is None or dev.index == cur else torch.cuda.device(dev)
    if ctx is not None:
        ctx.__enter__()
    try:
        stream = engine._raw_stream(dev.index if dev.index is not None else cur) if engine._raw_stream is not None else engine._stream_ptr(dev)
        if tiles is not None:
            a.flags = r.flags | _lib.F_LOADER_TILES
            a.n_tiles_launch = tiles[2]
            rc = lib.dmpnn_forward_tiles(_ctypes.byref(a), None, tiles[0].data_ptr(), tiles[1].data_ptr(), tiles[2], nbytes, stream)
        elif own is not None:
            a.flags = r.flags if small else (r.flags | _lib.F_LOADER_TILES)
            a.n_tiles_launch = own[2]
            rc = lib.dmpnn_forward_tiles(_ctypes.byref(a), batch.data_ptr(), own[0].data_ptr(), own[1].data_ptr(), own[2], nbytes, stream)
        else:
            a.flags = r.flags if small else (r.flags | _lib.F_LOADER_TILES)
            a.n_tiles_launch = n_mols
            rc = lib.dmpnn_forward_tiles(_ctypes.byref(a), batch.data_ptr(), None, None, 0, nbytes, stream)
    finally:
        if ctx is not None:
            ctx.__exit__(None, None, None)
    if rc:
        _lib.check(rc, "dmpnn_forward_tiles")
    if oversize is None:
        _spill_monitor(mp, buf, dev)
    from .agg import note_batch

    note_batch(batch, n_mols)
    return out


class _Monitor:
    __slots__ = ("host", "event", "pending", "calls", "observed", "with_spill")


def _spill_monitor(mp, plan_buf: Tensor, dev) -> None:
    if torch.cuda.is_current_stream_capturing():
        return
    m = mp.__dict__.get("_dmpnn_mon")
    if m is None:
        m = _Monitor()
        m.host = torch.zeros(16, dtype=torch.int32).pin_memory()
        m.event = torch.cuda.Event()
        m.pending, m.calls, m.observed, m.with_spill = False, 0, 0, 0
        mp.__dict__["_dmpnn_mon"] = m
    if m.pending and m.event.query():
        m.pending = False
        _note_spills(mp, m, int(m.host[8]))
    m.calls += 1
    if not m.pending and (m.calls % 8 == 0 if m.calls <= 64 else m.calls % 64 == 0) and not torch.cuda.is_current_stream_capturing():
        m.host.copy_(plan_buf[:16], non_blocking=True)
        m.event.record(torch.cuda.current_stream(dev))
        m.pending = True


def _note_spills(mp, m, n_spill: int) -> None:
    m.observed += 1
    if n_spill > 0:
        m.with_spill += 1
    if m.with_spill >= 2 and 4 * m.with_spill >= m.observed:
        object.__setattr__(mp, "_dmpnn_no_mega", True)


def bond_message_passing_forward(mp, bmg, V_d: Optional[Tensor] = None) -> Tensor:
    if torch.compiler.is_compiling() or torch.compiler.is_exporting():
        from .export import traced_forward

        return traced_forward(mp, bmg, V_d)
    if V_d is None and not torch.is_grad_enabled():
        r = mp.__dict__.get("_dmpnn_replay")
        if r is not None:
            out = _replay_forward(mp, r, bmg)
            if out is not None:
                return out
    bmg = mp.graph_transform(bmg)
    engine._require_device(bmg.V, "bmg.V")
    if mp.W_i.weight.device != bmg.V.device:
        raise RuntimeError(f"module is on {mp.W_i.weight.device} but the batch is on {bmg.V.device}")
    n_atoms = int(bmg.V.shape[0])
    if V_d is not None:
        V_d = mp.V_d_transform(V_d)
        d_vd = (mp.W_d.in_features - mp.W_o.out_features) if mp.W_d is not None else None
        if mp.W_d is None or V_d.dim() != 2 or V_d.shape[0] != n_atoms or V_d.shape[1] != d_vd:
            raise InvalidShapeError("V_d", V_d.shape, [n_atoms, d_vd if d_vd is not None else 0])
    n_mols = len(bmg) if hasattr(bmg, "__len__") else 0
    loader_tiles = getattr(bmg, "tiles", None) is not None or (
        getattr(bmg, "batch", None) is not None and not engine.small_plan_fits(int(bmg.V.shape[0]), int(bmg.E.shape[0]))
        and bool(_lib.load().dmpnn_tile_plan_any_size(int(bmg.V.shape[0]), int(bmg.E.shape[0]))))
    oversize = getattr(bmg, "oversize", None)
    if oversize is None and mp.training and mp.dropout.p > 0 and torch.is_grad_enabled():
        oversize = batch_oversize(bmg, n_mols)
    if oversize is True:
        loader_tiles = False
    light = _light_plan_ok(mp)
    if light and oversize is not True and _tile_plan_ok(mp, int(bmg.V.shape[0]), int(bmg.E.shape[0]), n_mols, loader_tiles):
        light = "tiles"
    if not light and torch.is_grad_enabled() and V_d is None:
        light = _training_plan_kind(mp, bmg) if oversize is not True else False
    in_grad = input_grad_wanted(bmg.V, bmg.E, V_d)
    light, cap = input_grad_plan(in_grad, light, 2)
    plan = engine.GraphPlan.from_bmg(bmg, light=light, launch="defer" if light == "tiles" else True)
    own = getattr(bmg, "plan_table", None)
    if own is not None and plan.pending is not None and not torch.is_grad_enabled() and own[0].device == plan.device:
        plan.host_tiles = own
    if n_mols and getattr(bmg, "batch", None) is not None:
        from .agg import note_batch

        note_batch(bmg.batch, n_mols)
    mp.__dict__.pop("_dmpnn_last", None)
    plan.oversize = oversize
    level = _route(mp, plan, n_mols, getattr(bmg, "batch", None))
    if oversize is True:
        level = min(level, 1)
    level = min(level, cap)
    out = mp_forward(mp, plan, bmg.V, bmg.E, V_d, max_level=level)
    last = mp.__dict__.pop("_dmpnn_last", None)
    mp.__dict__["_dmpnn_route"] = getattr(last, "route", None)
    plan.ensure_launched()
    if oversize is None and plan.tiles_only and last is not None and last.route in ("mega16", "mega16/f16-operands"):
        _spill_monitor(mp, plan.buf, plan.device)
    if light == "tiles" and V_d is None and not torch.is_grad_enabled() and _lib.opt("DMPNN_REPLAY", "1") != "0":
        _make_replay(mp, plan, last)
    return out


_VALIDATE_FIRST_N = 2


def batch_oversize(bmg, n_mols: int = 0):
    o = getattr(bmg, "oversize", None)
    if o is not None:
        return bool(o)
    batch = getattr(bmg, "batch", None)
    if batch is None or batch.dtype != torch.int64 or batch.numel() != int(bmg.V.shape[0]):
        return None
    from .data import TILE_MAX_ATOMS, TILE_MAX_EDGES

    if batch.numel() == 0:
        return False
    n_mols = int(n_mols) if n_mols else 0
    na = torch.bincount(batch, minlength=n_mols)
    bad = na.max() > TILE_MAX_ATOMS
    if int(bmg.E.shape[0]) > 0:
        ne = torch.bincount(batch[bmg.edge_index[1]], minlength=n_mols)
        bad = bad | (ne.max() > TILE_MAX_EDGES)
    return bool(bad.item())


def _light_plan_ok(mp) -> bool:
    if torch.is_grad_enabled() and any(p.requires_grad for p in mp.parameters()):
        return False
    if mp.undirected or (mp.training and mp.dropout.p > 0) or classify_activation(mp.tau)[0] == "custom":
        return False
    if _lib.opt("DMPNN_GENERAL", "0") == "1":
        return False
    if _lib.opt("DMPNN_VALIDATE", "first") != "never" and getattr(mp, "_dmpnn_batches_checked", 0) < _VALIDATE_FIRST_N:
        return False
    d_h, d_in = mp.W_h.weight.shape[0], mp.W_i.weight.shape[1]
    d_v = mp.W_o.weight.shape[1] - d_h
    return d_h % 4 == 0 and d_h <= 320 and d_v % 2 == 0 and (d_in - d_v) % 2 == 0


def _tile_plan_ok(mp, n_atoms: int, n_edges: int, n_mols: int, loader_tiles: bool = False) -> bool:
    if _lib.opt("DMPNN_MEGA", "1") == "0" or _lib.opt("DMPNN_MFMA", "split16") == "f32":
        return False
    if getattr(mp, "_dmpnn_no_mega", False):
        return False
    if _lib.opt("DMPNN_VALIDATE", "first") == "always":
        return False
    return n_mols > 0 and n_edges <= 30 * n_mols and (loader_tiles or engine.small_plan_fits(n_atoms, n_edges))


def _route(mp, plan, n_mols: int = 0, batch=None) -> int:
    mode = _lib.opt("DMPNN_VALIDATE", "first")
    seen = getattr(mp, "_dmpnn_batches_checked", 0)
    no_mega = getattr(mp, "_dmpnn_no_mega", False)
    if n_mols > 0 and plan.n_edges > 30 * n_mols:
        no_mega = True
    if mode == "always" or (mode == "first" and seen < _VALIDATE_FIRST_N):
        object.__setattr__(mp, "_dmpnn_batches_checked", seen + 1)
        hdr = plan.header()
        flags = hdr[0]
        if flags & 7:
            return 0
        if hdr[8] > 0 and getattr(plan, "oversize", None) is None:
            no_mega = True
            object.__setattr__(mp, "_dmpnn_no_mega", True)
        if flags & 8:
            if engine.small_plan_fits(plan.n_atoms, plan.n_edges) or (getattr(plan, "any_size", False) and not plan.tiles_only):
                object.__setattr__(mp, "_dmpnn_no_mega", True)
            elif batch is not None and not no_mega and _lib.load().dmpnn_tile_plan_any_size(plan.n_atoms, plan.n_edges):
                tp = engine.GraphPlan(plan.edge_index, plan.rev_edge_index, plan.n_atoms, light="tiles", batch=batch)
                if tp.tiles_only and tp.flags() & 8:
# ... 162 lines not shown
```

### include/dmpnn.h

```cpp
#ifndef DMPNN_H
#define DMPNN_H

#include <stddef.h>
#include <stdint.h>

#ifdef __cplusplus
extern "C" {
#endif

#define DMPNN_ABI_VERSION 15

enum dmpnn_status {
    DMPNN_OK = 0,
    DMPNN_EINVAL = -1,
    DMPNN_EHIP = -2,
    DMPNN_ENOSPC = -3
};

enum dmpnn_activation {
    DMPNN_ACT_NONE = 0,
    DMPNN_ACT_RELU = 1,
    DMPNN_ACT_LEAKYRELU = 2,
    DMPNN_ACT_PRELU = 3,
    DMPNN_ACT_TANH = 4,
    DMPNN_ACT_ELU = 5,
    DMPNN_ACT_SELU = 6
};

enum dmpnn_flags {
    DMPNN_F_UNDIRECTED = 1u << 0,
    DMPNN_F_UNDIRECTED_MASK = 1u << 12,
    DMPNN_F_FUSED = 1u << 1,
    DMPNN_F_MEGA = 1u << 2,
    DMPNN_F_KEEP = 1u << 3,
    DMPNN_F_SPLIT16 = 1u << 4,
    DMPNN_F_WSPLIT_READY = 1u << 5,
    DMPNN_F_LOADER_TILES = 1u << 6,
    DMPNN_F_H0_RESIDUAL = 1u << 8,
    DMPNN_F_ROW_FINALIZE = 1u << 9,
    DMPNN_F_ATOM = 1u << 10,
    DMPNN_F_TILE_PLAN = 1u << 11,
    DMPNN_F_STORE16 = 1u << 7
};

size_t dmpnn_plan_bytes(int64_t n_atoms, int64_t n_edges);

int dmpnn_prepare(const int64_t* edge_index,
                  const int64_t* rev_edge_index,
                  int64_t n_atoms, int64_t n_edges, void* plan, size_t plan_bytes, void* stream);
int dmpnn_prepare_light(const int64_t* edge_index, const int64_t* rev_edge_index, int64_t n_atoms, int64_t n_edges,
                        void* plan, size_t plan_bytes, void* stream);

int dmpnn_prepare_tiles(const int64_t* edge_index, const int64_t* rev_edge_index, const int64_t* batch, int64_t n_atoms,
                        int64_t n_edges, void* plan, size_t plan_bytes, void* stream);
int dmpnn_tile_plan_any_size(int64_t n_atoms, int64_t n_edges);

int dmpnn_prepare_with_batch(const int64_t* edge_index, const int64_t* rev_edge_index, const int64_t* batch, int64_t n_atoms,
                             int64_t n_edges, void* plan, size_t plan_bytes, void* stream);
int dmpnn_full_plan_keeps_tiles(int64_t n_atoms, int64_t n_edges);

enum dmpnn_plan_hdr {
    DMPNN_HDR_FLAGS = 0,
    DMPNN_HDR_MAXDEG = 1,
    DMPNN_HDR_NATOMS = 2,
    DMPNN_HDR_NEDGES = 3,
    DMPNN_HDR_NTILES = 4,
    DMPNN_HDR_TILE_STRIDE = 5,
    DMPNN_HDR_NMTILES = 6,
    DMPNN_HDR_LIGHT = 7,
    DMPNN_HDR_NSPILL = 8,
    DMPNN_HDR_WORDS = 16
};
#define DMPNN_PLAN_NOFFSETS 15
int dmpnn_plan_layout(int64_t n_atoms, int64_t n_edges, int64_t offsets_out[DMPNN_PLAN_NOFFSETS]);


int dmpnn_message_fwd(const void* plan, int64_t n_atoms, int64_t n_edges, int64_t d_h,
                      const float* Hin, int64_t ld_in, float* M, int64_t ld_m,
                      int act_on_load, float act_slope, const float* act_slope_ptr,
                      unsigned flags, void* stream);

int dmpnn_aggregate_fwd(const void* plan, int64_t n_atoms, int64_t n_edges, int64_t d_h,
                        const float* Hin, int64_t ld_in, float* Mv, int64_t ld_mv,
                        int act_on_load, float act_slope, const float* act_slope_ptr, void* stream);

typedef struct dmpnn_gemm_args {
    int64_t M, N, K1, K2;
    const float* A1; int64_t lda1; const int32_t* gather1;
    int64_t gather1_rows;
    const float* A2; int64_t lda2;
    const float* W;  int64_t ldw;
    const float* bias;
    const float* Cadd; int64_t ldcadd;
    float* C; int64_t ldc;
    float* Zpre; int64_t ldz;
    int act; float act_slope; const float* act_slope_ptr;
} dmpnn_gemm_args;
int dmpnn_linear_fwd(const dmpnn_gemm_args* a, void* stream);
size_t dmpnn_linear16_wsplit_bytes(int64_t N, int64_t K);
int dmpnn_linear16_ok(const dmpnn_gemm_args* a);
int dmpnn_linear16_fwd(const dmpnn_gemm_args* a, void* wsplit, size_t wsplit_bytes, int wsplit_ready, void* stream);
int dmpnn_linear16_dropout_fwd(const dmpnn_gemm_args* a, void* wsplit, size_t wsplit_bytes, int wsplit_ready, float p, uint64_t seed,
                               int32_t site, void* stream);

int dmpnn_update_fwd(const void* plan, int64_t n_atoms, int64_t n_edges, int64_t d_h,
                     const float* M, int64_t ld_m, const float* H0, int64_t ld_h0,
                     const float* W_h, const float* b_h,
                     float* H_out, int64_t ld_hout, float* M_next, int64_t ld_mnext,
                     float* Mv, int64_t ld_mv,
                     int act, float act_slope, const float* act_slope_ptr, void* stream);

typedef struct dmpnn_fwd_args {
    const void* plan; int64_t n_atoms, n_edges;
    int64_t d_v, d_e, d_h, d_vd; int32_t depth; uint32_t flags;
    int32_t act; float act_slope; const float* act_slope_ptr;
    const float* V; int64_t ldv;
    const float* E; int64_t lde;
    const float* V_d; int64_t ldvd;
    const float* W_i; const float* b_i;
    const float* W_h; const float* b_h;
    const float* W_o; const float* b_o;
    const float* W_d; const float* b_d;
    int64_t ldh; float* H0; float* Hs; int32_t n_hslots; float* Ms; int32_t n_mslots;
    float* Mv; float* Hv;
    float* out; int64_t ldout;
    void* wsplit; size_t wsplit_bytes;
    const int64_t* edge_index; const int64_t* rev_edge_index;
    int64_t n_tiles_launch;
    float* spill_ws; size_t spill_bytes;
    void* msplit; size_t msplit_bytes;
    float dropout_p; uint64_t dropout_seed;
    void* keep_bits; size_t keep_bits_bytes;
    size_t h0_bytes;
} dmpnn_fwd_args;
size_t dmpnn_forward_wsplit_bytes(const dmpnn_fwd_args* a);
size_t dmpnn_forward_keep_bits_bytes(const dmpnn_fwd_args* a);
size_t dmpnn_forward_h0_bytes(const dmpnn_fwd_args* a);
int64_t dmpnn_split_row_floats(int64_t d_h);
int dmpnn_forward_can_fuse16(const dmpnn_fwd_args* a);
size_t dmpnn_forward_spill_bytes(const dmpnn_fwd_args* a);
int dmpnn_forward(const dmpnn_fwd_args* a, void* stream);
int dmpnn_forward_tiles(const dmpnn_fwd_args* a, const int64_t* batch, const int* tile_row, const int* tile_atom, int64_t n_tiles,
                        size_t plan_bytes, void* stream);
int dmpnn_forward_can_fuse(const dmpnn_fwd_args* a);
enum dmpnn_route { DMPNN_ROUTE_GENERAL = 0, DMPNN_ROUTE_GENERAL16 = 1, DMPNN_ROUTE_FUSED = 2, DMPNN_ROUTE_FUSED16 = 3,
                   DMPNN_ROUTE_MEGA = 4, DMPNN_ROUTE_MEGA16 = 5 };
int dmpnn_forward_route(const dmpnn_fwd_args* a, int keep, int max_level, int plan_kind, int arith);
int dmpnn_tile_waves(int64_t n_atoms, int64_t n_edges, int64_t d_h, int64_t n_tiles);

#define DMPNN_KEEP_ROWS_MIN 4096
typedef struct dmpnn_train_route_info {
    int32_t plan_kind;
    int32_t route;
    int32_t keep_rows;
    int32_t keep_bits;
    int32_t lean;
} dmpnn_train_route_info;
int dmpnn_train_route(const dmpnn_fwd_args* a, int64_t n_mols, int32_t have, int32_t oversize, int32_t max_level, int32_t arith,
                      int32_t keep_rows, dmpnn_train_route_info* out);

typedef struct dmpnn_bwd_args {
    dmpnn_fwd_args f;
    const float* gout; int64_t ldgout;
    float* gW_i; float* gb_i; float* gW_h; float* gb_h;
    float* gW_o; float* gb_o; float* gW_d; float* gb_d;
    float* ws; size_t ws_bytes;
    const float* g_edge; int64_t ld_gedge;
} dmpnn_bwd_args;
size_t dmpnn_backward_ws_bytes(const dmpnn_fwd_args* f);
int dmpnn_backward(const dmpnn_bwd_args* a, void* stream);

typedef struct dmpnn_bwd_inputs_args {
    dmpnn_bwd_args b;
    float* gV;   int64_t ldgv;
    float* gE;   int64_t ldge;
    float* gV_d; int64_t ldgvd;
} dmpnn_bwd_inputs_args;
size_t dmpnn_backward_inputs_ws_bytes(const dmpnn_fwd_args* f);
int dmpnn_backward_inputs(const dmpnn_bwd_inputs_args* a, void* stream);
int dmpnn_src_sum(const void* plan, int64_t n_atoms, int64_t n_edges, int64_t d_h, const float* G, int64_t ldg, float* S, int64_t lds,
                  void* stream);

int dmpnn_message_bwd(const void* plan, int64_t n_atoms, int64_t n_edges, int64_t d_h,
                      const float* gM, int64_t ld_gm, float* gH, int64_t ld_gh, void* stream);
int dmpnn_atom_message_bwd(const void* plan, int64_t n_atoms, int64_t n_edges, int64_t d_h,
                           const float* gM, int64_t ld_gm, float* gH, int64_t ld_gh, void* stream);
int dmpnn_aggregate_bwd(const void* plan, int64_t n_atoms, int64_t n_edges, int64_t d_h,
                        const float* gMv, int64_t ld_gmv, float* gH, int64_t ld_gh, void* stream);
size_t dmpnn_linear_wgrad_ws_bytes(int64_t M, int64_t N, int64_t K, int has_bias);
int dmpnn_linear_wgrad(const dmpnn_gemm_args* g, const float* gZ, int64_t ldgz, float* gW, int64_t ldgw,
                       float* gb, void* ws, size_t ws_bytes, void* stream);

enum dmpnn_molagg_mode { DMPNN_MOLAGG_SUM = 0, DMPNN_MOLAGG_MEAN = 1, DMPNN_MOLAGG_NORM = 2,
                         DMPNN_MOLAGG_ATTENTIVE = 3  };
size_t dmpnn_molagg_ws_bytes(int64_t n_mols);
int dmpnn_molagg_bounds(const int64_t* batch, int64_t n_atoms, int64_t n_mols, void* ws, size_t ws_bytes, void* stream);
int dmpnn_molagg_fwd(const float* H, int64_t ldh, int64_t n_atoms, int64_t d_h, int64_t n_mols, const void* ws, int mode,
                     float norm, float* out, int64_t ldo, void* stream);
int dmpnn_molagg_bwd(const float* gout, int64_t ldg, const int64_t* batch, int64_t n_atoms, int64_t d_h, int64_t n_mols,
                     const void* ws, int mode, float norm, float* gH, int64_t ldgh, void* stream);

typedef struct dmpnn_molagg_attn_args {
    int64_t n_atoms, n_mols, d_h;
    const float* H; int64_t ldh;
    const int64_t* batch;
    const void* bounds;
    const float* W; const float* b;
    float* out; int64_t ldo;
    float* keep_s; float* keep_Z;
    const float* gout; int64_t ldgo;
    float* gH; int64_t ldgh;
    float* gW; float* gb;
    void* ws; size_t ws_bytes;
} dmpnn_molagg_attn_args;
size_t dmpnn_molagg_attn_ws_bytes(const dmpnn_molagg_attn_args* a);
int dmpnn_molagg_attn_fwd(const dmpnn_molagg_attn_args* a, void* stream);
int dmpnn_molagg_attn_bwd(const dmpnn_molagg_attn_args* a, void* stream);

int dmpnn_gather_rows(const float* X, int64_t ldx, int64_t n_src, const int* idx, int64_t n_out, int64_t d,
                      float* out, int64_t ldo, void* stream);

int dmpnn_collate(const int* atom_off, const int* edge_off, int64_t n_mols, const int* src, const int* dst, const int* rev,
                  int64_t n_atoms, int64_t n_edges, int64_t* edge_index, int64_t* rev_edge_index, int64_t* batch,
                  void* stream);

int64_t dmpnn_pack_tiles(const int* atom_off, const int* edge_off, int64_t n_mols, int* tile_row, int* tile_atom, int64_t cap);
int64_t dmpnn_pack_tiles_blocked(const int* atom_off, const int* edge_off, int64_t n_mols, int* tile_row, int* tile_atom, int64_t cap);
int64_t dmpnn_max_tiles(int64_t n_atoms, int64_t n_edges);
int dmpnn_prepare_tiles_from_table(const int* tile_row, const int* tile_atom, int64_t n_tiles, int64_t n_atoms,
                                   int64_t n_edges, void* plan, size_t plan_bytes, void* stream);

// ... 128 lines not shown
```

Baseline: 524.1 M edge-updates/s.

## Add 12-wave and no-spill-path forms of the bond tile kernel for fitting tiles

Adds a specialised tile16 kernel instantiation without the oversize/spill fallback path (GEN=false), used when the caller guarantees all tiles fit. It also adds a 12-wave workgroup form that splits the 20 column tiles as 8x2 + 4x1, with launch bounds allowing 3 blocks. That form is chosen for mid-range tile counts, aiming to cut register pressure and raise occupancy. Oversize tiles now write NaN instead of falling back, which relies on the fit flag being correct. A build-time register cap check is added.

```diff
diff --git a/chemprop_amd/_lib.py b/chemprop_amd/_lib.py
--- a/chemprop_amd/_lib.py
+++ b/chemprop_amd/_lib.py
@@ -12,7 +12,7 @@
 INCLUDE = os.path.join(_ROOT, "include")
 LIB_PATH = os.environ.get("DMPNN_LIB") or os.path.join(_HERE, "libdmpnn_gfx950.so")
 SOURCES = ["dmpnn_abi.hip", "dmpnn_prepare.hip", "dmpnn_segment.hip", "dmpnn_gemm.hip", "dmpnn_gemm_p1.hip",
-           "dmpnn_gemm_p2.hip", "dmpnn_gemm_p3.hip", "dmpnn_gemm_p4.hip", "dmpnn_gemm_s1.hip", "dmpnn_rows16_drop.hip", "dmpnn_mega.hip", "dmpnn_mega16.hip", "dmpnn_mega16_lp.hip", "dmpnn_mega16_bwd.hip", "dmpnn_rows16.hip", "dmpnn_step16.hip", "dmpnn_bstep16.hip", "dmpnn_backward.hip", "dmpnn_molagg.hip", "dmpnn_collate.hip", "dmpnn_tiles_large.hip", "dmpnn_optim.hip", "dmpnn_wgrad16.hip", "dmpnn_head.hip", "dmpnn_vd.hip", "dmpnn_attn.hip", "dmpnn_inputgrad.hip", "dmpnn_predict.hip"]
+           "dmpnn_gemm_p2.hip", "dmpnn_gemm_p3.hip", "dmpnn_gemm_p4.hip", "dmpnn_gemm_s1.hip", "dmpnn_rows16_drop.hip", "dmpnn_mega.hip", "dmpnn_mega16.hip", "dmpnn_mega16_lp.hip", "dmpnn_mega16_fit.hip", "dmpnn_mega16_bwd.hip", "dmpnn_rows16.hip", "dmpnn_step16.hip", "dmpnn_bstep16.hip", "dmpnn_backward.hip", "dmpnn_molagg.hip", "dmpnn_collate.hip", "dmpnn_tiles_large.hip", "dmpnn_optim.hip", "dmpnn_wgrad16.hip", "dmpnn_head.hip", "dmpnn_vd.hip", "dmpnn_attn.hip", "dmpnn_inputgrad.hip", "dmpnn_predict.hip"]
 HEADERS = ["dmpnn_common.hpp", "dmpnn_spill_impl.hpp", "dmpnn_gemm_impl.hpp", "dmpnn_mega_impl.hpp", "dmpnn_mega16_impl.hpp", "dmpnn_mega16_bwd_impl.hpp", "dmpnn_rows16_impl.hpp", "dmpnn_seg16.hpp", "dmpnn_step16_impl.hpp", "dmpnn_head_kernels.hpp"]
 ABI_VERSION = 15
 PLAN_NOFFSETS = 15
@@ -30,6 +30,7 @@
     "dmpnn_molagg_attn_ws_bytes", "dmpnn_molagg_attn_fwd", "dmpnn_molagg_attn_bwd",
     "dmpnn_backward_inputs", "dmpnn_backward_inputs_ws_bytes", "dmpnn_src_sum",
     "dmpnn_predict_head_ws_bytes", "dmpnn_predict_head_wsplit_bytes", "dmpnn_predict_head",
+    "dmpnn_tile_form", "dmpnn_last_tile_form", "dmpnn_debug_tile_form",
 ]
 
 ACT = {"none": 0, "relu": 1, "leakyrelu": 2, "prelu": 3, "tanh": 4, "elu": 5, "selu": 6}
@@ -43,6 +44,8 @@
 F_STORE16 = 128
 F_ATOM = 1024
 F_TILE_PLAN = 2048
+F_TILES_FIT = 8192
+TILE_FORM_WAVES, TILE_FORM_NOGEN = 0xFF, 0x100
 F_UNDIRECTED_MASK = 4096
 F_H0_RESIDUAL = 256
 F_ROW_FINALIZE = 512
@@ -237,13 +240,14 @@
     return any(os.path.getmtime(d) > t for d in deps if os.path.isfile(d))
 
 
-NO_SCRATCH = ("dmpnn_predict.hip",)
+NO_SCRATCH = ("dmpnn_predict.hip", "dmpnn_mega16_fit.hip")
+REGISTER_CAPS = {"k_mpnn_tile16ILi5ELb1ELb0ELi12E": 168, "k_mpnn_tile16ILi5ELb0ELb0ELi12E": 168}
 
 
 def _check_no_scratch(src: str, remarks: str, verbose: bool) -> None:
     import re
 
-    fields = ("Function Name", "VGPRs", "LDS Size [bytes/block]", "ScratchSize [bytes/lane]")
+    fields = ("Function Name", "VGPRs", "LDS Size [bytes/block]", "ScratchSize [bytes/lane]", "AGPRs")
     found = [dict()]
     for key, val in re.findall(r"remark:\s+(%s): (\S+)" % "|".join(re.escape(f) for f in fields), remarks):
         if key == "Function Name":
@@ -257,6 +261,14 @@
             print(f"{os.path.basename(src)}: {k['Function Name']} VGPRs {k.get('VGPRs')} LDS {k.get(fields[2])} B scratch {k.get(fields[3])} B/lane")
         if int(k.get(fields[3], "0")) != 0:
             raise RuntimeError(f"{src}: kernel {k['Function Name']} spills ({k[fields[3]]} bytes of scratch per lane)")
+        for frag, cap in REGISTER_CAPS.items():
+            regs = int(k.get("VGPRs", "0")) + int(k.get("AGPRs", "0"))
+            if frag in k["Function Name"] and regs > cap:
+                raise RuntimeError(f"{src}: kernel {k['Function Name']} takes {regs} registers (VGPRs + AGPRs), more than the {cap} of its form")
+    if os.path.basename(src) == "dmpnn_mega16_fit.hip":
+        for frag in REGISTER_CAPS:
+            if not any(frag in k["Function Name"] for k in kernels):
+                raise RuntimeError(f"{src}: no kernel named *{frag}* in the compiler's resource report (the register cap was not checked)")
 
 
 def build(force: bool = False, verbose: bool = False, defines=(), out: Optional[str] = None) -> str:
@@ -404,6 +416,8 @@
     lib.dmpnn_forward_route.argtypes = [C.POINTER(FwdArgs), C.c_int, C.c_int, C.c_int, C.c_int]
     lib.dmpnn_tile_waves.restype = C.c_int
     lib.dmpnn_tile_waves.argtypes = [C.c_int64, C.c_int64, C.c_int64, C.c_int64]
+    lib.dmpnn_tile_form.argtypes = [C.POINTER(FwdArgs), C.c_int64]
+    lib.dmpnn_debug_tile_form.argtypes = [C.c_int]
     lib.dmpnn_forward_tiles.argtypes = [C.POINTER(FwdArgs), C.c_void_p, C.c_void_p, C.c_void_p, C.c_int64, C.c_size_t, C.c_void_p]
     lib.dmpnn_full_plan_keeps_tiles.argtypes = [C.c_int64, C.c_int64]
     lib.dmpnn_head_ws_bytes.argtypes = [C.POINTER(HeadArgs)]
@@ -426,6 +440,7 @@
     for name in EXPORTS:
         if name != "dmpnn_last_error_string" and name not in size_t_fns and name not in ("dmpnn_pack_tiles", "dmpnn_pack_tiles_blocked", "dmpnn_max_tiles", "dmpnn_split_row_floats"):
             getattr(lib, name).restype = C.c_int
+    lib.dmpnn_debug_tile_form.restype = None
     if lib.dmpnn_version() != ABI_VERSION:
         raise RuntimeError(f"libdmpnn ABI version {lib.dmpnn_version()} != {ABI_VERSION} (stale build?)")
     _lib = lib
diff --git a/chemprop_amd/csrc/dmpnn_abi.hip b/chemprop_amd/csrc/dmpnn_abi.hip
--- a/chemprop_amd/csrc/dmpnn_abi.hip
+++ b/chemprop_amd/csrc/dmpnn_abi.hip
@@ -317,6 +317,13 @@
     t.n_atoms = n_atoms; t.n_edges = n_edges; t.d_h = d_h;
     return tile_waves(t, n_tiles > 0 ? (int)n_tiles : (int)plan_layout(n_atoms, n_edges).max_mtiles);
 }
+
+int dmpnn_tile_form(const dmpnn_fwd_args* a, int64_t n_tiles) {
+    if (!a) return 0;
+    return tile_form(*a, n_tiles > 0 ? (int)n_tiles : (int)plan_layout(a->n_atoms, a->n_edges).max_mtiles);
+}
+int dmpnn_last_tile_form(void) { return g_tile_form_last; }
+void dmpnn_debug_tile_form(int form) { g_tile_form_forced = form; }
 
 int dmpnn_forward_route(const dmpnn_fwd_args* a, int keep, int max_level, int plan_kind, int arith) {
     if (!a || max_level < 0 || plan_kind < 0 || plan_kind > 2 || arith < 0 || arith > 1) return -1;
diff --git a/chemprop_amd/csrc/dmpnn_common.hpp b/chemprop_amd/csrc/dmpnn_common.hpp
--- a/chemprop_amd/csrc/dmpnn_common.hpp
+++ b/chemprop_amd/csrc/dmpnn_common.hpp
@@ -277,6 +277,8 @@
                          const RowsDrop* drop = nullptr);
 int launch_mega16_forward(const dmpnn_fwd_args& a, float* out, int64_t ldout, hipStream_t s);
 int tile_waves(const dmpnn_fwd_args& a, int n_tiles);
+int tile_form(const dmpnn_fwd_args& a, int n_tiles);
+extern thread_local int g_tile_form_forced, g_tile_form_last;
 bool fused16_shapes_ok(const dmpnn_fwd_args& a);
 bool fused16_lean_shapes(const dmpnn_fwd_args& a, bool on_demand = false);
 size_t fused16_lean_bits_bytes(const dmpnn_fwd_args& a);
diff --git a/chemprop_amd/csrc/dmpnn_mega16.hip b/chemprop_amd/csrc/dmpnn_mega16.hip
--- a/chemprop_amd/csrc/dmpnn_mega16.hip
+++ b/chemprop_amd/csrc/dmpnn_mega16.hip
@@ -2,6 +2,11 @@
 #include <cstdlib>
 
 #include "dmpnn_mega16_impl.hpp"
+
+#if !defined(DMPNN_TILE12_MIN_TILES)
+#define DMPNN_TILE12_MIN_TILES 29
+#define DMPNN_TILE12_MAX_TILES 116
+#endif
 
 namespace dmpnn {
 namespace mega16 {
@@ -25,10 +30,15 @@
 DMPNN_DECLARE_MEGA16_LP(1, true, 4) DMPNN_DECLARE_MEGA16_LP(1, false, 4) DMPNN_DECLARE_MEGA16_LP(2, true, 4) DMPNN_DECLARE_MEGA16_LP(2, false, 4)
 DMPNN_DECLARE_MEGA16_LP(5, true, 4) DMPNN_DECLARE_MEGA16_LP(5, false, 4) DMPNN_DECLARE_MEGA16_LP(5, true, 8) DMPNN_DECLARE_MEGA16_LP(5, false, 8)
 #undef DMPNN_DECLARE_MEGA16_LP
+#define DMPNN_DECLARE_MEGA16_FIT(SA, NW) template <> int launch_mega16<5, SA, false, NW, false, false>(const Mega16K& g, int n_tiles, hipStream_t s);
+DMPNN_DECLARE_MEGA16_FIT(true, 8) DMPNN_DECLARE_MEGA16_FIT(false, 8) DMPNN_DECLARE_MEGA16_FIT(true, 12) DMPNN_DECLARE_MEGA16_FIT(false, 12)
+#undef DMPNN_DECLARE_MEGA16_FIT
 }
 
 thread_local long long* g_debug_stamps = nullptr;
 thread_local AggRide g_agg_ride = {nullptr, 0, nullptr, nullptr, 0, 0, 0.f, false};
+thread_local int g_tile_form_forced = 0;
+thread_local int g_tile_form_last = 0;
 
 namespace {
 inline size_t al256(size_t x) { return (x + 255) & ~size_t(255); }
@@ -116,6 +126,23 @@
     return est + est / 16 <= n_cu ? 8 : 4;
 }
 
+static const int kTile12Min = DMPNN_TILE12_MIN_TILES, kTile12Max = DMPNN_TILE12_MAX_TILES;
+static int tile_count_estimate(const dmpnn_fwd_args& a, int n_tiles) {
+    const int64_t est = std::max<int64_t>((a.n_edges + 39) / 40, (a.n_atoms + 19) / 20);
+    return (int)std::min<int64_t>(n_tiles, est + est / 16);
+}
+int tile_form(const dmpnn_fwd_args& a, int n_tiles) {
+    const int w = tile_waves(a, n_tiles);
+    const bool fit = (a.flags & DMPNN_F_TILES_FIT) && !(a.flags & (DMPNN_F_KEEP | DMPNN_F_ATOM | DMPNN_F_STORE16)) && a.d_h > 128 && a.d_h <= 320;
+    if (!fit) return w;
+    static const int env_forced = [] { const char* e = getenv("DMPNN_TILE_FORM"); return e ? (int)strtol(e, nullptr, 0) : 0; }();
+    const int forced = g_tile_form_forced ? g_tile_form_forced : env_forced;
+    if (forced == 4 || forced == 8 || forced == (8 | DMPNN_TILE_FORM_NOGEN) || forced == (12 | DMPNN_TILE_FORM_NOGEN)) return forced;
+    if (w != 8) return w;
+    const int nt = tile_count_estimate(a, n_tiles);
+    return (nt >= kTile12Min && nt <= kTile12Max) ? (12 | DMPNN_TILE_FORM_NOGEN) : w;
+}
+
 int launch_mega16_forward(const dmpnn_fwd_args& a, float* out, int64_t ldout, hipStream_t s) {
     const int64_t nV = a.n_atoms, nE = a.n_edges;
     const WsLayout W = ws_layout(a);
@@ -186,6 +213,13 @@
     const int n_tiles = (a.n_tiles_launch > 0 && a.n_tiles_launch < L.max_mtiles) ? (int)a.n_tiles_launch : (int)L.max_mtiles;
     const bool sa = !act_is_smooth(a.act), kp = (a.flags & DMPNN_F_KEEP) != 0;
     const int wn = a.d_h <= 64 ? 1 : (a.d_h <= 128 ? 2 : 5);
+    const int form = tile_form(a, n_tiles);
+    g_tile_form_last = wn == 5 ? form : 4;
+    if (form & DMPNN_TILE_FORM_NOGEN) {
+        if ((form & DMPNN_TILE_FORM_WAVES) == 12)
+            return sa ? mega16::launch_mega16<5, true, false, 12, false, false>(G, n_tiles, s) : mega16::launch_mega16<5, false, false, 12, false, false>(G, n_tiles, s);
+        return sa ? mega16::launch_mega16<5, true, false, 8, false, false>(G, n_tiles, s) : mega16::launch_mega16<5, false, false, 8, false, false>(G, n_tiles, s);
+    }
     if (a.flags & DMPNN_F_STORE16) {
         if (wn == 1) return sa ? mega16::launch_mega16<1, true, false, 4, true>(G, n_tiles, s) : mega16::launch_mega16<1, false, false, 4, true>(G, n_tiles, s);
         if (wn == 2) return sa ? mega16::launch_mega16<2, true, false, 4, true>(G, n_tiles, s) : mega16::launch_mega16<2, false, false, 4, true>(G, n_tiles, s);
@@ -197,7 +231,7 @@
                            : (kp ? mega16::launch_mega16<WN, false, true>(G, n_tiles, s) : mega16::launch_mega16<WN, false, false>(G, n_tiles, s)))
     if (wn == 1) return DMPNN_PICK(1);
     if (wn == 2) return DMPNN_PICK(2);
-    if (tile_waves(a, n_tiles) == 8)
+    if (form == 8)
         return sa ? (kp ? mega16::launch_mega16<5, true, true, 8>(G, n_tiles, s) : mega16::launch_mega16<5, true, false, 8>(G, n_tiles, s))
                   : (kp ? mega16::launch_mega16<5, false, true, 8>(G, n_tiles, s) : mega16::launch_mega16<5, false, false, 8>(G, n_tiles, s));
     return DMPNN_PICK(5);
diff --git a/chemprop_amd/csrc/dmpnn_mega16_fit.hip b/chemprop_amd/csrc/dmpnn_mega16_fit.hip
--- /dev/null
+++ b/chemprop_amd/csrc/dmpnn_mega16_fit.hip
@@ -0,0 +1,10 @@
+#include "dmpnn_mega16_impl.hpp"
+
+namespace dmpnn {
+namespace mega16 {
+DMPNN_DEFINE_MEGA16_GEN(5, true, false, 8, false, false)
+DMPNN_DEFINE_MEGA16_GEN(5, false, false, 8, false, false)
+DMPNN_DEFINE_MEGA16_GEN(5, true, false, 12, false, false)
+DMPNN_DEFINE_MEGA16_GEN(5, false, false, 12, false, false)
+}
+}
diff --git a/chemprop_amd/csrc/dmpnn_mega16_impl.hpp b/chemprop_amd/csrc/dmpnn_mega16_impl.hpp
--- a/chemprop_amd/csrc/dmpnn_mega16_impl.hpp
+++ b/chemprop_amd/csrc/dmpnn_mega16_impl.hpp
@@ -193,13 +193,15 @@
 template <int WN>
 constexpr size_t lds_bytes_atom() { return lds_bytes<WN>() + kAtomLds; }
 
-template <int WN, bool SA, bool KEEP, int NW = 4, bool LP = false>
-__global__ __launch_bounds__(64 * NW, 2) void k_mpnn_tile16(Mega16K G) {
+template <int WN, bool SA, bool KEEP, int NW = 4, bool LP = false, bool GEN = true>
+__global__ __launch_bounds__(64 * NW, NW == 12 ? 3 : 2) void k_mpnn_tile16(Mega16K G) {
     static_assert(!(LP && KEEP), "the hi-halves-alone form is inference only");
-    static_assert(NW == 4 || (NW == 8 && WN == 5), "the 8-wave form splits 20 column tiles 3+3+3+3+2+2+2+2");
+    static_assert(NW == 4 || (NW == 8 && WN == 5) || (NW == 12 && WN == 5 && !GEN && !KEEP && !LP),
+                  "the 8-wave form splits 20 column tiles 3+3+3+3+2+2+2+2, the 12-wave form 2 x 8 + 1 x 4");
+    static_assert(GEN || (!KEEP && !LP), "the promise form is the inference bond form");
     const mega::MegaK& g = G.m;
     constexpr int KT = 64 * NW;
-    constexpr int JR = 16 / NW;
+#define JROWS(RT) ((16 * (RT) + NW - 1) / NW)
     constexpr int BM = kMegaBM, BA = kMegaBA, BN = 64 * WN, LDC = BN + 4, QN = BN / 4;
     constexpr int TS = BN * 4 + 16;
     constexpr int ITEMS = (BM * QN + KT - 1) / KT;
@@ -256,7 +258,13 @@
         return;
     }
     if (na <= 0 || nrows < 0 || va < 0 || vb > g.nV || rs < 0 || re > g.nE) return;
-    if (nrows > BM || na > BA) {
+    if constexpr (!GEN) {
+        if (nrows > BM || na > BA) {
+            const float nanv = __int_as_float(0x7fc00000);
+            for (int i = tid; i < na * N; i += KT) g.out[(long long)(va + i / N) * g.ldout + (i % N)] = nanv;
+            return;
+        }
+    } else if (nrows > BM || na > BA) {
         if (NW > 4 && threadIdx.x >= kThreads) return;
         const mega::MegaK& gs = spill::fresh_kernargs<Mega16K>()->m;
         if ((KEEP && gs.drop_thr) || G.atom_de) {
@@ -289,9 +297,9 @@
 
     int revl_v = 0, rp_v = 0, aor_v = 0, asrc_v = 0;
     bool row_bad = false;
-    unsigned ro1[JR * RT_E], ro2[JR * RT_E];
+    unsigned ro1[JROWS(RT_E)], ro2[JROWS(RT_E)];
     {
-        int i1[JR * RT_E], i2[JR * RT_E];
+        int i1[JROWS(RT_E)], i2[JROWS(RT_E)];
         if (lean && nrows > 0) {
             const int e = rs + (tid < nrows ? tid : 0);
             const long long es = g.edge_index[e], ed = g.edge_index[(long long)g.nE + e], er = g.rev64[e];
@@ -301,7 +309,7 @@
             aor_v = (tid < nrows && !row_bad) ? (int)d_l : 0;
             asrc_v = (tid < nrows && !row_bad) ? (int)s_l : 0;
 #pragma unroll
-            for (int j = 0; j < JR * RT_E; ++j) {
+            for (int j = 0; j < JROWS(RT_E); ++j) {
                 const int r = wave + NW * j;
                 const long long sj = g.edge_index[r < nrows ? rs + r : rs];
                 i1[j] = (sj >= 0 && sj < g.nV) ? (int)sj : 0;
@@ -309,32 +317,32 @@
             }
         } else if (lean) {
 #pragma unroll
-            for (int j = 0; j < JR * RT_E; ++j) { i1[j] = 0; i2[j] = 0; }
+            for (int j = 0; j < JROWS(RT_E); ++j) { i1[j] = 0; i2[j] = 0; }
         } else {
             revl_v = tid < nrows ? g.revp[rs + tid] - rs : 0;
             rp_v = g.row_ptr[va + (tid <= na ? tid : na)] - rs;
 #pragma unroll
-            for (int j = 0; j < JR * RT_E; ++j) {
+            for (int j = 0; j < JROWS(RT_E); ++j) {
                 const int r = wave + NW * j;
                 i1[j] = g.srcp[r < nrows ? rs + r : 0];
                 i2[j] = g.perm[r < nrows ? rs + r : 0];
             }
         }
 #pragma unroll
-        for (int j = 0; j < JR * RT_E; ++j) {
+        for (int j = 0; j < JROWS(RT_E); ++j) {
             const bool ok = wave + NW * j < nrows;
             ro1[j] = ok ? (unsigned)i1[j] * (unsigned)g.ldv * 4u : kOOB;
             ro2[j] = ok ? (unsigned)i2[j] * (unsigned)g.lde * 4u : kOOB;
         }
     }
     const rsrc_t rVg = gemm::make_rsrc(g.V, g.v_bytes), rEg = gemm::make_rsrc(g.E, g.e_bytes);
-    u32x2 a_grp[JR * RT_E];
+    u32x2 a_grp[JROWS(RT_E)];
     {
         const int k = lane * 2;
         const unsigned k1o = k < g.d_v ? (unsigned)k * 4u : kOOB;
         const unsigned k2o = (k >= g.d_v && k < g.d_v + g.d_e) ? (unsigned)(k - g.d_v) * 4u : kOOB;
 #pragma unroll
-        for (int j = 0; j < JR * RT_E; ++j)
+        for (int j = 0; j < JROWS(RT_E); ++j)
             a_grp[j] = __builtin_amdgcn_raw_buffer_load_b64(rVg, gemm::join_off(ro1[j], k1o), 0, 0) |
                        __builtin_amdgcn_raw_buffer_load_b64(rEg, gemm::join_off(ro2[j], k2o), 0, 0);
     }
@@ -415,7 +423,7 @@
 
     auto body = [&](auto wl_c) __attribute__((always_inline)) {
     constexpr int WL = decltype(wl_c)::value;
-    auto ct0 = [&]() -> int { return (NW == 8 && WL == 2) ? 2 * wave + 4 : WL * wave; };
+    auto ct0 = [&]() -> int { return (NW == 8 && WL == 2) ? 2 * wave + 4 : ((NW == 12 && WL == 1) ? wave + 8 : WL * wave); };
     auto load_bfrags = [&](rsrc_t rW, const unsigned (&offB)[WL], int c, h8 (&bh)[WL], h8 (&bl)[WL]) {
 #pragma unroll
         for (int ct = 0; ct < WL; ++ct) {
@@ -544,9 +552,9 @@
     constexpr int TSG = 4 * 128 + 16;
     unsigned char* Ag = lds;
     auto ga_load = [&](auto rt_c, auto has_a2_c, int grp, int K1, int K2, rsrc_t rA1, rsrc_t rA2,
-                       const unsigned (&ro1)[JR * decltype(rt_c)::value], const unsigned (&ro2)[JR * decltype(rt_c)::value],
-                       u32x2 (&v)[JR * decltype(rt_c)::value]) {
-        constexpr int J = JR * decltype(rt_c)::value;
+                       const unsigned (&ro1)[JROWS(decltype(rt_c)::value)], const unsigned (&ro2)[JROWS(decltype(rt_c)::value)],
+                       u32x2 (&v)[JROWS(decltype(rt_c)::value)]) {
+        constexpr int J = JROWS(decltype(rt_c)::value);
         constexpr bool HAS_A2 = decltype(has_a2_c)::value;
         const int k = grp * 128 + lane * 2;
         const unsigned k1o = k < K1 ? (unsigned)k * 4u : kOOB;
@@ -557,8 +565,8 @@
             if constexpr (HAS_A2) v[j] = v[j] | __builtin_amdgcn_raw_buffer_load_b64(rA2, gemm::join_off(ro2[j], k2o), 0, 0);
         }
     };
-    auto ga_stage = [&](auto rt_c, f32x4 (&acc)[decltype(rt_c)::value][WL], const u32x2 (&v)[JR * decltype(rt_c)::value], float s_prev) -> float {
-        constexpr int RT = decltype(rt_c)::value, J = JR * RT;
+    auto ga_stage = [&](auto rt_c, f32x4 (&acc)[decltype(rt_c)::value][WL], const u32x2 (&v)[JROWS(decltype(rt_c)::value)], float s_prev) -> float {
+        constexpr int RT = decltype(rt_c)::value, J = JROWS(RT);
         float mx = 0.f;
 #pragma unroll
         for (int j = 0; j < J; ++j) mx = fmaxf(mx, fmaxf(fabsf(__uint_as_float(v[j].x)), fabsf(__uint_as_float(v[j].y))));
@@ -985,10 +993,10 @@
         const ColConst cc = col_consts(G.WoM.inv_scale, g.b_o);
         const rsrc_t rV = gemm::make_rsrc(g.V + (long long)va * g.ldv, (unsigned)(na * g.ldv) * 4u);
         const rsrc_t rnull = gemm::make_rsrc(g.W_o, 0);
-        unsigned rov[JR * RT_A];
-#pragma unroll
-        for (int j = 0; j < JR * RT_A; ++j) rov[j] = wave + NW * j < na ? (unsigned)(wave + NW * j) * (unsigned)g.ldv * 4u : kOOB;
-        u32x2 v_grp[JR * RT_A];
+        unsigned rov[JROWS(RT_A)];
+#pragma unroll
+        for (int j = 0; j < JROWS(RT_A); ++j) rov[j] = wave + NW * j < na ? (unsigned)(wave + NW * j) * (unsigned)g.ldv * 4u : kOOB;
+        u32x2 v_grp[JROWS(RT_A)];
         ga_load(RA{}, F_{}, 0, g.d_v, 0, rV, rnull, rov, rov, v_grp);
         contract(RA{}, acc, T16, TS, (N + BK - 1) / BK, 0, G.WoM);
         stamp();
@@ -1044,24 +1052,29 @@
     };
     if constexpr (NW == 4) {
         body(std::integral_constant<int, WN>{});
+    } else if constexpr (NW == 12) {
+        if (__builtin_amdgcn_readfirstlane((int)(threadIdx.x >> 6)) < 8) body(std::integral_constant<int, 2>{});
+        else body(std::integral_constant<int, 1>{});
     } else {
         if (__builtin_amdgcn_readfirstlane((int)(threadIdx.x >> 6)) < 4) body(std::integral_constant<int, 3>{});
         else body(std::integral_constant<int, 2>{});
     }
-}
-
-template <int WN, bool SA, bool KEEP, int NW = 4, bool LP = false>
+#undef JROWS
+}
+
+template <int WN, bool SA, bool KEEP, int NW = 4, bool LP = false, bool GEN = true>
 int launch_mega16(const Mega16K& g, int n_tiles, hipStream_t s);
 
 #define DMPNN_DEFINE_MEGA16(WN, SA, KEEP) DMPNN_DEFINE_MEGA16_NW(WN, SA, KEEP, 4)
 #define DMPNN_DEFINE_MEGA16_NW(WN, SA, KEEP, NW) DMPNN_DEFINE_MEGA16_LP(WN, SA, KEEP, NW, false)
-#define DMPNN_DEFINE_MEGA16_LP(WN, SA, KEEP, NW, LP)                                                       \
+#define DMPNN_DEFINE_MEGA16_LP(WN, SA, KEEP, NW, LP) DMPNN_DEFINE_MEGA16_GEN(WN, SA, KEEP, NW, LP, true)
+#define DMPNN_DEFINE_MEGA16_GEN(WN, SA, KEEP, NW, LP, GEN)                                                 \
     template <>                                                                                            \
-    int launch_mega16<WN, SA, KEEP, NW, LP>(const Mega16K& g, int n_tiles, hipStream_t s) {                \
+    int launch_mega16<WN, SA, KEEP, NW, LP, GEN>(const Mega16K& g, int n_tiles, hipStream_t s) {                \
         const size_t lds = g.atom_de ? lds_bytes_atom<WN>() : lds_bytes<WN>();                             \
         static bool attr_set = false;                                                                      \
         if (!attr_set) {                                                                                   \
-            hipError_t e = hipFuncSetAttribute(reinterpret_cast<const void*>(&k_mpnn_tile16<WN, SA, KEEP, NW, LP>),      \
+            hipError_t e = hipFuncSetAttribute(reinterpret_cast<const void*>(&k_mpnn_tile16<WN, SA, KEEP, NW, LP, GEN>),      \
                                                hipFuncAttributeMaxDynamicSharedMemorySize, (int)lds_bytes_atom<WN>()); \
             if (e != hipSuccess) {                                                                         \
                 set_error("hipFuncSetAttribute(k_mpnn_tile16<%d>, %zu B LDS): %s", WN, lds, hipGetErrorString(e)); \
@@ -1069,7 +1082,7 @@
             }                                                                                              \
             attr_set = true;                                                                               \
         }                                                                                                  \
-        hipLaunchKernelGGL((k_mpnn_tile16<WN, SA, KEEP, NW, LP>), dim3((unsigned)n_tiles), dim3(64 * NW), lds, s, g);   \
+        hipLaunchKernelGGL((k_mpnn_tile16<WN, SA, KEEP, NW, LP, GEN>), dim3((unsigned)n_tiles), dim3(64 * NW), lds, s, g);   \
         DMPNN_CHECK_LAUNCH("k_mpnn_tile16");                                                               \
         return DMPNN_OK;                                                                                   \
     }
diff --git a/chemprop_amd/engine.py b/chemprop_amd/engine.py
--- a/chemprop_amd/engine.py
+++ b/chemprop_amd/engine.py
@@ -8,7 +8,7 @@
 from torch import Tensor
 
 from . import _lib
-from ._lib import (ACT, F_FUSED, F_H0_RESIDUAL, F_KEEP, F_LOADER_TILES, F_MEGA, F_ROW_FINALIZE, F_SPLIT16, F_STORE16, F_TILE_PLAN, F_UNDIRECTED, F_WSPLIT_READY,
+from ._lib import (ACT, F_FUSED, F_H0_RESIDUAL, F_KEEP, F_LOADER_TILES, F_MEGA, F_ROW_FINALIZE, F_SPLIT16, F_STORE16, F_TILE_PLAN, F_TILES_FIT, F_UNDIRECTED, F_WSPLIT_READY,
                    PLAN_NOFUSE_MASK, PLAN_NOMEGA_MASK, FwdArgs, GemmArgs)
 
 
@@ -93,7 +93,7 @@
 class GraphPlan:
 
     __slots__ = ("buf", "n_atoms", "n_edges", "device", "light", "tiles_only", "edge_index", "rev_edge_index", "loader_tiles",
-                 "any_size", "oversize", "pending", "_job", "host_tiles")
+                 "any_size", "oversize", "tiles_fit", "pending", "_job", "host_tiles")
 
     def __init__(self, edge_index: Tensor, rev_edge_index: Tensor, n_atoms: int, light=False, batch: Optional[Tensor] = None,
                  tiles: Optional[tuple] = None, launch: bool = True):
@@ -109,6 +109,7 @@
         self.buf = torch.empty(nbytes // 4, dtype=torch.int32, device=dev)
         self.n_atoms, self.n_edges, self.device = int(n_atoms), n_edges, dev
         self.oversize = None
+        self.tiles_fit = False
         small = small_plan_fits(n_atoms, n_edges)
         self.loader_tiles = 0
         if light == "tiles" and tiles is not None:
@@ -502,6 +503,8 @@
     if getattr(plan, "loader_tiles", 0) or getattr(plan, "any_size", False):
         a.flags |= F_LOADER_TILES
         a.n_tiles_launch = plan.loader_tiles
+    if getattr(plan, "tiles_fit", False):
+        a.flags |= F_TILES_FIT
     a.act, a.act_slope, a.act_slope_ptr = act_code(act), float(slope), _ptr(slope_t)
     a.V, a.ldv = V.data_ptr(), V.stride(0)
     a.E, a.lde = E.data_ptr(), E.stride(0)
diff --git a/chemprop_amd/nn.py b/chemprop_amd/nn.py
--- a/chemprop_amd/nn.py
+++ b/chemprop_amd/nn.py
@@ -167,7 +167,7 @@
         return
     blk = r.block = _lib.FwdArgs.from_buffer_copy(r.args)
     blk.ldv, blk.lde, blk.ldout = r.d_v, r.d_e, r.d_h
-    r.flags = int(blk.flags) & ~_lib.F_WSPLIT_READY & ~_lib.F_LOADER_TILES
+    r.flags = int(blk.flags) & ~_lib.F_WSPLIT_READY & ~_lib.F_LOADER_TILES & ~_lib.F_TILES_FIT
     r.ldh, r.spill = int(blk.ldh), None
     mp.__dict__["_dmpnn_replay"] = r
 
@@ -234,18 +234,19 @@
     ctx = None if dev.index is None or dev.index == cur else torch.cuda.device(dev)
     if ctx is not None:
         ctx.__enter__()
+    flags = (r.flags | _lib.F_TILES_FIT) if oversize is False else r.flags
     try:
         stream = engine._raw_stream(dev.index if dev.index is not None else cur) if engine._raw_stream is not None else engine._stream_ptr(dev)
         if tiles is not None:
-            a.flags = r.flags | _lib.F_LOADER_TILES
+            a.flags = flags | _lib.F_LOADER_TILES
             a.n_tiles_launch = tiles[2]
             rc = lib.dmpnn_forward_tiles(_ctypes.byref(a), None, tiles[0].data_ptr(), tiles[1].data_ptr(), tiles[2], nbytes, stream)
         elif own is not None:
-            a.flags = r.flags if small else (r.flags | _lib.F_LOADER_TILES)
+            a.flags = flags if small else (flags | _lib.F_LOADER_TILES)
             a.n_tiles_launch = own[2]
             rc = lib.dmpnn_forward_tiles(_ctypes.byref(a), batch.data_ptr(), own[0].data_ptr(), own[1].data_ptr(), own[2], nbytes, stream)
         else:
-            a.flags = r.flags if small else (r.flags | _lib.F_LOADER_TILES)
+            a.flags = flags if small else (flags | _lib.F_LOADER_TILES)
             a.n_tiles_launch = n_mols
             rc = lib.dmpnn_forward_tiles(_ctypes.byref(a), batch.data_ptr(), None, None, 0, nbytes, stream)
     finally:
@@ -340,6 +341,7 @@
         note_batch(bmg.batch, n_mols)
     mp.__dict__.pop("_dmpnn_last", None)
     plan.oversize = oversize
+    plan.tiles_fit = getattr(bmg, "oversize", None) is False
     level = _route(mp, plan, n_mols, getattr(bmg, "batch", None))
     if oversize is True:
         level = min(level, 1)
diff --git a/include/dmpnn.h b/include/dmpnn.h
--- a/include/dmpnn.h
+++ b/include/dmpnn.h
@@ -40,6 +40,7 @@
     DMPNN_F_ROW_FINALIZE = 1u << 9,
     DMPNN_F_ATOM = 1u << 10,
     DMPNN_F_TILE_PLAN = 1u << 11,
+    DMPNN_F_TILES_FIT = 1u << 13,
     DMPNN_F_STORE16 = 1u << 7
 };
 
@@ -147,6 +148,11 @@
                    DMPNN_ROUTE_MEGA = 4, DMPNN_ROUTE_MEGA16 = 5 };
 int dmpnn_forward_route(const dmpnn_fwd_args* a, int keep, int max_level, int plan_kind, int arith);
 int dmpnn_tile_waves(int64_t n_atoms, int64_t n_edges, int64_t d_h, int64_t n_tiles);
+#define DMPNN_TILE_FORM_WAVES 0xFF
+#define DMPNN_TILE_FORM_NOGEN 0x100
+int dmpnn_tile_form(const dmpnn_fwd_args* a, int64_t n_tiles);
+int dmpnn_last_tile_form(void);
+void dmpnn_debug_tile_form(int form);
 
 #define DMPNN_KEEP_ROWS_MIN 4096
 typedef struct dmpnn_train_route_info {
```

Result: no change. 522.4 M edge-updates/s (-0.3%).
